# pujariaditya/WaveVerify

Measured on AMD Instinct MI355X. Metric: clips/sec embed+detect, 1s@16kHz bs=256, higher is better.
Workload: dtype f32; 1 GPU; embed_detect: 256 clips x 1 s @ 16 kHz per GPU (BASELINE.json configs[1]), seeded random weights; batch_per_gpu=256, global_batch=256, clip_samples=16000, parallelism=dp1 (independent clip shards, no data-path collective)

## Files before the change

### waveverify_amd/csrc/wv_k1.hip

```cpp
#include <algorithm>
#include <atomic>
#include <cstdlib>
#include <string>
#include <type_traits>

#include "wv_dev.h"

namespace wv {

typedef const __attribute__((address_space(1))) void* gptr_t;
typedef __attribute__((address_space(3))) void* lptr_t;

__device__ __attribute__((aligned(16))) float g_zero16[4] = {0.f, 0.f, 0.f, 0.f};

__device__ __forceinline__ float dpp_next(float v) {
    return __builtin_bit_cast(float, __builtin_amdgcn_update_dpp(0, __builtin_bit_cast(int, v), 0x130, 0xf, 0xf, true));
}

template <int NT_, int BKC_, int BM_ = 128>
struct K1 {
    static constexpr int NT = NT_, BN = 32 * NT_, BKC = BKC_, KQ = BKC_ / 4, BM = BM_, WM = BM_ / 32, NTHREADS = 64 * WM;
    static constexpr int A4 = KQ * BM;
    static constexpr int B4 = BKC * BN / 4;
    static constexpr int STAGE4 = A4 + B4;
    static constexpr int A_PIECES = A4 / 64, B_PIECES = B4 / 64;
    static constexpr int A_PER = (A_PIECES + WM - 1) / WM, B_PER_DMA = (B_PIECES + WM - 1) / WM;
    static constexpr int CG = BN / 4;
    static constexpr int HLD = BN + 4;
    static constexpr int NBT = (BKC / 2) * CG;
    static constexpr int B_PER = (NBT + NTHREADS - 1) / NTHREADS;
    static_assert(A4 % 64 == 0 && B4 % 64 == 0 && NTHREADS % CG == 0 && 64 % CG == 0, "staging maps");
};

template <int NT> struct NVec;
template <> struct NVec<4> { typedef f32x4 type; };
template <> struct NVec<2> { typedef f32x2 type; };

constexpr int OOB_VOFF = 0x40000000;

template <class C>
struct DmaRows {
    const float* src; size_t ld; int K; int rbase;
    __device__ __forceinline__ void init(const float* Xb, int K_, int Tin, int ti0, int wave, int lane) {
        const int col = ti0 + 4 * (lane % C::CG);
        rbase = lane / C::CG;
        const bool inr = col >= 0 && col + 3 < Tin;
        src = inr ? Xb + col : g_zero16;
        ld = inr ? (size_t)Tin : 0;
        K = K_;
        (void)wave;
    }
    __device__ __forceinline__ void init_flat(const float* X, int K_, int Tin, int B, int Tv, int pad, long long g0, int lane) {
        const long long g = g0 + 4 * (lane % C::CG);
        const int b = (int)(g / Tv), t = (int)(g - (long long)b * Tv) - pad;
        rbase = lane / C::CG;
        const bool inr = b < B && t >= 0;
        src = inr ? X + (size_t)b * K_ * Tin + t : g_zero16;
        ld = inr ? (size_t)Tin : 0;
        K = K_;
    }
    __device__ __forceinline__ void issue(int c, f32x4* Bst, int wave) const {
#pragma unroll
        for (int i = 0; i < C::B_PER_DMA; ++i) {
            const int pi = wave + i * C::WM;
            if (C::B_PIECES % C::WM == 0 || pi < C::B_PIECES) {
                const int k = min(c * C::BKC + pi * (64 / C::CG) + rbase, K - 1);
                __builtin_amdgcn_global_load_lds((gptr_t)(src + (size_t)k * ld), (lptr_t)(Bst + pi * 64), 16, 0, 0);
            }
        }
    }
};

template <class C>
struct DmaA {
    __amdgpu_buffer_rsrc_t rsrc;
    int voff[C::A_PER];
    int chunk_bytes;
    __device__ __forceinline__ void init(const f32x4* wq, int Mp, int m0, int nchunks, int wave, int lane) {
        rsrc = __builtin_amdgcn_make_buffer_rsrc(const_cast<f32x4*>(wq + m0), 0, (nchunks * C::KQ * Mp - m0) * 16, 0x00020000);
        chunk_bytes = C::KQ * Mp * 16;
#pragma unroll
        for (int i = 0; i < C::A_PER; ++i) {
            const int idx = (wave + i * C::WM) * 64 + lane;
            voff[i] = ((idx / C::BM) * Mp + idx % C::BM) * 16;
        }
    }
    __device__ __forceinline__ void issue(int c, f32x4* Ast, int wave) const {
        const int soff = c * chunk_bytes;
#pragma unroll
        for (int i = 0; i < C::A_PER; ++i) {
            const int pi = wave + i * C::WM;
            if (C::A_PIECES % C::WM == 0 || pi < C::A_PIECES) {
                const int vo = voff[i];
                __builtin_amdgcn_raw_ptr_buffer_load_lds(rsrc, (lptr_t)(Ast + pi * 64), 16, vo, soff, 0, 0);
            }
        }
    }
};

template <class C, int EPI, int RES>
struct K1Epi {
    static constexpr int NT = C::NT, HLD = C::HLD;
    static constexpr int NTAP = EPI == 0 ? 5 : (EPI == 2 ? 4 : (EPI == 4 ? 8 : 16));
    static constexpr int WLD = EPI == 0 ? 8 : NTAP + 4;
    static constexpr int TABLE_FLOATS = C::BM * WLD;
    static constexpr bool HASR = RES == 1 || RES == 2 || RES == 5;
    static constexpr bool RAWH = RES == 4 || RES == 5;
    static constexpr int RP = HASR ? 4 : 0;
    typedef typename NVec<NT>::type ovec;
    int M, m0, b, to0, lane, wave, half, q, o, to;
    bool act_lane, vec;
    const float* Rb; float* Yb; float* Ab; float* Wl;
    const float* Rb2; float* Hb; float* Sb;
    int voff0, nrec;
    float fgam, fbet;

    __device__ __forceinline__ int row_of(int r) const { return 32 * wave + (r & 3) + 8 * (r >> 2) + 4 * half; }
    __device__ __forceinline__ ovec load_res(const PwDwArgs& p, int r) const {
        ovec v;
#pragma unroll
        for (int e = 0; e < NT; ++e) v[e] = 0.f;
        const int gm = m0 + row_of(r);
        if (act_lane && gm < M) {
            const float* rp = Rb + (size_t)gm * p.Tout + to;
            if (vec) v = *reinterpret_cast<const ovec*>(rp);
            else {
#pragma unroll
                for (int e = 0; e < NT; ++e)
                    if (o + e < p.tto && to + e < p.Tout) v[e] = rp[e];
            }
        }
        return v;
    }
    __device__ __forceinline__ void store(const PwDwArgs& p, int gm, const float (&y)[NT]) const {
        const size_t yo = (size_t)gm * p.Tout + to;
        if (Yb) {
            if (vec) { ovec v; _Pragma("unroll") for (int e = 0; e < NT; ++e) v[e] = y[e]; *reinterpret_cast<ovec*>(Yb + yo) = v; }
            else {
#pragma unroll
                for (int e = 0; e < NT; ++e)
                    if (o + e < p.tto && to + e < p.Tout) Yb[yo + e] = y[e];
            }
        }
        if (Ab) {
            float a[NT];
#pragma unroll
            for (int e = 0; e < NT; ++e) a[e] = elu1(y[e] * p.act_scale);
            if (vec) { ovec v; _Pragma("unroll") for (int e = 0; e < NT; ++e) v[e] = a[e]; *reinterpret_cast<ovec*>(Ab + yo) = v; }
            else {
#pragma unroll
                for (int e = 0; e < NT; ++e)
                    if (o + e < p.tto && to + e < p.Tout) Ab[yo + e] = a[e];
            }
        }
    }
    __device__ __forceinline__ void begin(const PwDwArgs& p, float* table, int m0_, int b_, int to0_, long long gflat = 0) {
        M = p.pw.M; m0 = m0_; b = b_; to0 = to0_;
        const int tid = threadIdx.x;
        lane = tid & 63;
        wave = __builtin_amdgcn_readfirstlane(tid >> 6);
        half = lane >> 5; q = lane & 31;
        Wl = table;
        const size_t bo = (size_t)b * M * p.Tout;
        Yb = p.Y ? p.Y + bo : nullptr;
        Ab = p.Yact ? p.Yact + bo : nullptr;
        Rb = (HASR && p.resid) ? p.resid + bo : nullptr;
        Rb2 = (RES == 2 && p.resid2) ? p.resid2 + bo : nullptr;
        Hb = (RAWH && p.Yraw) ? p.Yraw + bo : nullptr;
        Sb = (RES == 5 && p.Ysum) ? p.Ysum + bo : nullptr;
        o = NT * q; to = to0 + o;
        act_lane = o < p.tto && to < p.Tout;
        vec = act_lane && to + NT - 1 < p.Tout && o + NT - 1 < p.tto && (p.Tout % NT) == 0;
        nrec = M * p.Tout * 4;
        voff0 = act_lane ? ((m0 + 32 * wave + 4 * half) * p.Tout + to) * 4 : 0x7f000000;
        if (EPI == 0 && p.flat) {
            const long long gc = gflat + p.pad + o;
            const int bo2 = (int)(gc / p.Tv), t = (int)(gc - (long long)bo2 * p.Tv) - p.pad;
            const bool ok = o < p.tto && bo2 < p.B && t >= 0;
            Yb = p.Y; Ab = p.Yact; Rb = HASR ? p.resid : nullptr; Rb2 = RES == 2 ? p.resid2 : nullptr; Hb = RAWH ? p.Yraw : nullptr; Sb = RES == 5 ? p.Ysum : nullptr;
            nrec = (int)((long long)p.B * M * p.Tout * 4);
            voff0 = ok ? (int)((((long long)bo2 * M + m0 + 32 * wave + 4 * half) * p.Tout + t) * 4) : (int)0x80000000u;
        }
        if (EPI == 8 && p.flat) {
            const int TvO = p.Tv >> 3;
            const long long go = gflat / 8 + (q >> 1);
            const int bo2 = (int)(go / TvO), n = (int)(go - (long long)bo2 * TvO);
            const bool ok = (q & 1) == 0 && (q >> 1) < p.tto && bo2 < p.B && n < p.Tout;
            Yb = p.Y; Ab = p.Yact;
            nrec = (int)((long long)p.B * M * p.Tout * 4);
            voff0 = ok ? (int)((((long long)bo2 * M + m0 + 32 * wave + 4 * half) * p.Tout + n) * 4) : (int)0x80000000u;
            fgam = 1.f; fbet = 0.f;
            if (p.film) {
                const float* fl = p.film + (size_t)min(bo2, p.B - 1) * p.film_stride + 2 * (m0 / (M / p.bands));
                fgam = fl[0]; fbet = fl[1];
            }
        }
        const bool lane_film = EPI == 8 && p.flat;
        const int bw = p.film ? (M / p.bands) : 1;
        const float* filmb = (p.film && !lane_film) ? p.film + (size_t)b * p.film_stride : nullptr;
        for (int m = tid; m < C::BM; m += C::NTHREADS) {
            const int gm = m0 + m;
            float* row = Wl + m * WLD;
#pragma unroll
            for (int i = 0; i < NTAP; ++i) row[i] = (gm < M && i < p.ks) ? p.dw_w[(size_t)gm * p.ks + i] : 0.f;
            float gam = 1.f, bet = 0.f;
            if (filmb && gm < M) { const int band = gm / bw; gam = filmb[2 * band]; bet = filmb[2 * band + 1]; }
            row[NTAP] = (gm < M && p.dw_b) ? p.dw_b[gm] : 0.f;
            row[NTAP + 1] = gam; row[NTAP + 2] = bet;
            if (EPI != 0) row[WLD - 1] = 0.f;
        }
    }

    typedef unsigned uvec __attribute__((ext_vector_type(NT)));
    __device__ __forceinline__ ovec buf_load(__amdgpu_buffer_rsrc_t r, int off) const {
        if constexpr (NT == 4) return __builtin_bit_cast(ovec, __builtin_amdgcn_raw_buffer_load_b128(r, off, 0, 0));
        else return __builtin_bit_cast(ovec, __builtin_amdgcn_raw_buffer_load_b64(r, off, 0, 0));
    }
    __device__ __forceinline__ void buf_store(__amdgpu_buffer_rsrc_t r, int off, ovec v) const {
        if constexpr (NT == 4) __builtin_amdgcn_raw_buffer_store_b128(__builtin_bit_cast(uvec, v), r, off, 0, 0);
        else __builtin_amdgcn_raw_buffer_store_b64(__builtin_bit_cast(uvec, v), r, off, 0, 0);
    }

    __device__ __forceinline__ void finish(f32x16 (&acc)[NT], const PwDwArgs& p, float* strips) {
        if constexpr (EPI == 0) {
            constexpr int NSH = 4 / NT;
            const int clip_bytes = nrec;
            const __amdgpu_buffer_rsrc_t rY = uniform_rsrc(Yb ? Yb : p.Yact, Yb ? clip_bytes : 0);
            const __amdgpu_buffer_rsrc_t rA = uniform_rsrc(Ab ? Ab : p.Yact, Ab ? clip_bytes : 0);
            const __amdgpu_buffer_rsrc_t rR = uniform_rsrc(Rb ? Rb : p.X, Rb ? clip_bytes : 0);
            const int row_bytes = p.Tout * 4;
            const int voff = voff0;
            const float* Wrow = Wl + (32 * wave + 4 * half) * 8;
            ovec res4[HASR ? 4 : 1];
            ovec add4[RES == 2 ? 4 : 1];
            const __amdgpu_buffer_rsrc_t rR2 = uniform_rsrc(Rb2 ? Rb2 : p.X, Rb2 ? clip_bytes : 0);
            const __amdgpu_buffer_rsrc_t rH = uniform_rsrc(Hb ? Hb : p.Y, Hb ? clip_bytes : 0);
            const __amdgpu_buffer_rsrc_t rS = uniform_rsrc(Sb ? Sb : p.Y, Sb ? clip_bytes : 0);
            const float sres = (RES == 5 && p.scale_ptr) ? p.out_scale * p.scale_ptr[0] : p.out_scale;
            if constexpr (HASR) {
#pragma unroll
                for (int r = 0; r < 4; ++r) res4[r] = buf_load(rR, voff + ((r & 3) + 8 * (r >> 2)) * row_bytes);
            }
            if constexpr (RES == 2) {
#pragma unroll
                for (int r = 0; r < 4; ++r) add4[r] = buf_load(rR2, voff + ((r & 3) + 8 * (r >> 2)) * row_bytes);
            }
            f32x4 w0n = *reinterpret_cast<const f32x4*>(Wrow), w1n = *reinterpret_cast<const f32x4*>(Wrow + 4);
#pragma unroll
            for (int r = 0; r < 16; ++r) {
                const int cr = (r & 3) + 8 * (r >> 2);
                const f32x4 w0 = w0n, w1 = w1n;
                if (r + 1 < 16) {
                    const int cn = ((r + 1) & 3) + 8 * ((r + 1) >> 2);
                    w0n = *reinterpret_cast<const f32x4*>(Wrow + cn * 8);
                    w1n = *reinterpret_cast<const f32x4*>(Wrow + cn * 8 + 4);
                }
                float hh[NT + 4], cur[NT];
#pragma unroll
                for (int e = 0; e < NT; ++e) { cur[e] = acc[e][r]; hh[e] = cur[e]; }
#pragma unroll
                for (int s2 = 1; s2 <= NSH; ++s2) {
#pragma unroll
                    for (int e = 0; e < NT; ++e) { cur[e] = dpp_next(cur[e]); hh[s2 * NT + e] = cur[e]; }
                }
                const int off = voff + cr * row_bytes;
                ovec y;
#pragma unroll
                for (int e = 0; e < NT; ++e) {
                    float v = fmaf(w0.x, hh[e], w1.y);
                    v = fmaf(w0.y, hh[e + 1], v); v = fmaf(w0.z, hh[e + 2], v);
                    v = fmaf(w0.w, hh[e + 3], v); v = fmaf(w1.x, hh[e + 4], v);
                    y[e] = v;
                }
                if constexpr (HASR) {
                    const ovec rr = res4[r & 3];
                    ovec rsum;
                    (void)rsum;
                    if (r + 4 < 16) res4[r & 3] = buf_load(rR, voff + (((r + 4) & 3) + 8 * ((r + 4) >> 2)) * row_bytes);
#pragma unroll
                    for (int e = 0; e < NT; ++e) {
                        if constexpr (RES == 2) {
                            const float z = p.out_scale * rr[e];
                            y[e] = y[e] * (z > 0.f ? 1.f : __expf(z)) * p.out_scale;
                        } else if constexpr (RES == 5) {
                            rsum[e] = fmaf(y[e], sres, rr[e]);
                        } else y[e] = fmaf(y[e], p.out_scale, rr[e]);
                    }
                    if constexpr (RES == 5) buf_store(rS, off, rsum);
                }
                if constexpr (RES == 2) {
                    const ovec ad = add4[r & 3];
                    if (r + 4 < 16) add4[r & 3] = buf_load(rR2, voff + (((r + 4) & 3) + 8 * ((r + 4) >> 2)) * row_bytes);
#pragma unroll
                    for (int e = 0; e < NT; ++e) y[e] += ad[e];
                }
                if constexpr (RAWH) {
                    ovec hraw;
#pragma unroll
                    for (int e = 0; e < NT; ++e) hraw[e] = hh[e + 4];
                    buf_store(rH, off, hraw);
                }
                if (Yb) buf_store(rY, off, y);
                if (Ab) {
                    ovec a;
#pragma unroll
                    for (int e = 0; e < NT; ++e) a[e] = elu1(y[e] * p.act_scale);
                    buf_store(rA, off, a);
                }
                __builtin_amdgcn_sched_barrier(0);
            }
        } else if constexpr (EPI == 5) {
            float* Hw = strips + wave * (4 * HLD);
#pragma unroll
            for (int r = 0; r < 16; ++r) {
                float* strip = Hw + (r & 1) * 2 * HLD;
                ovec hv;
#pragma unroll
                for (int e = 0; e < NT; ++e) hv[e] = acc[e][r];
                *reinterpret_cast<ovec*>(strip + half * HLD + NT * q) = hv;
                const int row = row_of(r), gm = m0 + row;
                const float* wt = Wl + row * WLD;
                const f32x4 ta = *reinterpret_cast<const f32x4*>(wt), tb = *reinterpret_cast<const f32x4*>(wt + 4);
                const f32x4 tc = *reinterpret_cast<const f32x4*>(wt + 8), td = *reinterpret_cast<const f32x4*>(wt + 16);
                if (gm < M && q < p.tto && to0 + q < p.Tout) {
                    const float* hp = strip + half * HLD + p.off + q * 5;
                    float y = td.x;
                    y = fmaf(ta.x, hp[0], y); y = fmaf(ta.y, hp[1], y); y = fmaf(ta.z, hp[2], y); y = fmaf(ta.w, hp[3], y);
                    y = fmaf(tb.x, hp[4], y); y = fmaf(tb.y, hp[5], y); y = fmaf(tb.z, hp[6], y); y = fmaf(tb.w, hp[7], y);
                    y = fmaf(tc.x, hp[8], y); y = fmaf(tc.y, hp[9], y);
                    y = fmaf(y, td.y, td.z);
                    const size_t ro = (size_t)gm * p.Tout + to0 + q;
                    if (Yb) Yb[ro] = y;
                    if (Ab) Ab[ro] = elu1(y * p.act_scale);
                }
            }
        } else if constexpr (EPI >= 2) {
            static_assert(NT == 4 && RES == 0, "strided DPP epilogue: 128-column windows, no residual");
            constexpr int R = EPI;
            const bool flat = R == 8 && p.flat;
            const int clip_bytes = flat ? nrec : M * p.Tout * 4;
            const __amdgpu_buffer_rsrc_t rY = uniform_rsrc(Yb ? Yb : p.Yact, Yb ? clip_bytes : 0);
            const __amdgpu_buffer_rsrc_t rA = uniform_rsrc(Ab ? Ab : p.Yact, Ab ? clip_bytes : 0);
            const int row_bytes = p.Tout * 4;
            const int o0 = R == 2 ? 2 * q : (R == 4 ? q : q >> 1);
            const bool lane_ok = (R != 8 || (q & 1) == 0) && o0 + (R == 2 ? 1 : 0) < p.tto && to0 + o0 + (R == 2 ? 1 : 0) < p.Tout;
            const int voff = flat ? voff0 : (lane_ok ? ((m0 + 32 * wave + 4 * half) * p.Tout + to0 + o0) * 4 : 0x7f000000);
            const float* Wrow = Wl + (32 * wave + 4 * half) * WLD;
#pragma unroll
            for (int r = 0; r < 16; ++r) {
                const int cr = (r & 3) + 8 * (r >> 2);
                constexpr int NL = R == 8 ? 4 : 2;
                float hh[4 * NL], cur[4];
#pragma unroll
                for (int e = 0; e < 4; ++e) { cur[e] = acc[e][r]; hh[e] = cur[e]; }
#pragma unroll
                for (int l = 1; l < NL; ++l) {
#pragma unroll
                    for (int e = 0; e < 4; ++e) { cur[e] = dpp_next(cur[e]); hh[4 * l + e] = cur[e]; }
                }
                const float* wt = Wrow + cr * WLD;
                float w[2 * R];
#pragma unroll
                for (int i = 0; i < 2 * R; i += 4) {
                    const f32x4 v = *reinterpret_cast<const f32x4*>(wt + i);
                    w[i] = v.x; w[i + 1] = v.y; w[i + 2] = v.z; w[i + 3] = v.w;
                }
                const f32x4 bgb = *reinterpret_cast<const f32x4*>(wt + NTAP);
                const int off = voff + cr * row_bytes;
                constexpr int NO = R == 2 ? 2 : 1;
                float y[NO];
#pragma unroll
                for (int j = 0; j < NO; ++j) {
                    const int base = R == 2 ? 2 + 2 * j : 0;
                    float v = bgb.x;
#pragma unroll
                    for (int i = 0; i < 2 * R; ++i) v = fmaf(w[i], hh[base + i], v);
                    y[j] = fmaf(v, bgb.y, bgb.z);
                    if (R == 8 && flat) y[j] = fmaf(y[j], fgam, fbet);
                }
                if constexpr (R == 2) {
                    typedef unsigned u2 __attribute__((ext_vector_type(2)));
                    if (Yb) __builtin_amdgcn_raw_buffer_store_b64(u2{__builtin_bit_cast(unsigned, y[0]), __builtin_bit_cast(unsigned, y[1])}, rY, off, 0, 0);
                    if (Ab) __builtin_amdgcn_raw_buffer_store_b64(u2{__builtin_bit_cast(unsigned, elu1(y[0] * p.act_scale)),
                                                                        __builtin_bit_cast(unsigned, elu1(y[1] * p.act_scale))}, rA, off, 0, 0);
                } else {
                    if (Yb) __builtin_amdgcn_raw_buffer_store_b32(__builtin_bit_cast(unsigned, y[0]), rY, off, 0, 0);
                    if (Ab) __builtin_amdgcn_raw_buffer_store_b32(__builtin_bit_cast(unsigned, elu1(y[0] * p.act_scale)), rA, off, 0, 0);
                }
                __builtin_amdgcn_sched_barrier(0);
            }
        } else {
            float* Hw = strips + wave * (4 * HLD);
            const int ks = p.ks;
            const int no = (p.tto + 31) / 32;
#pragma unroll
            for (int r = 0; r < 16; ++r) {
                float* strip = Hw + (r & 1) * 2 * HLD;
                ovec hv;
#pragma unroll
                for (int e = 0; e < NT; ++e) hv[e] = acc[e][r];
                *reinterpret_cast<ovec*>(strip + half * HLD + NT * q) = hv;
                const int row = row_of(r), gm = m0 + row;
                if (gm >= M) continue;
                const float* wt = Wl + row * WLD;
                const float bias = wt[16], gam = wt[17], bet = wt[18];
                const float* hrow = strip + half * HLD + p.off;
                const size_t ro = (size_t)gm * p.Tout + to0;
                for (int e = 0; e < no; ++e) {
                    const int oo = q * no + e;
                    if (oo >= p.tto || to0 + oo >= p.Tout) break;
                    const float* hp = hrow + oo * p.stride;
                    float y = bias;
                    for (int i = 0; i < ks; ++i) y = fmaf(wt[i], hp[i * p.dil], y);
                    y = fmaf(y, gam, bet);
                    if (RES == 1 && Rb) y = fmaf(y, p.out_scale, Rb[ro + oo]);
                    if (Yb) Yb[ro + oo] = y;
                    if (Ab) Ab[ro + oo] = elu1(y * p.act_scale);
                }
            }
        }
    }
};

template <int LDR> struct LdrSel { typedef RowPairLoader type; };
template <> struct LdrSel<2> { typedef ConvTrPair<4> type; };
template <> struct LdrSel<3> { typedef ConvTrPair<2> type; };
template <> struct LdrSel<4> { typedef ConvTrPair<1> type; };
template <> struct LdrSel<5> { typedef ConvTrPair<0> type; };
template <> struct LdrSel<6> { typedef ConvTrLds<4> type; };
template <> struct LdrSel<7> { typedef ConvTrLds<2> type; };
template <class C> constexpr int k1_lwp(int ldr) { return ldr == 7 ? (C::BN / 2 + 6 + 3) / 4 * 4 : (C::BN / 4 + 6 + 3) / 4 * 4; }

template <class C, int EPI, int LDR, int RES, int NS>
__global__ __launch_bounds__(C::NTHREADS, LDR >= 2 ? (C::B_PER > 1 ? 2 : 3) : 4) void k1_kernel(PwDwArgs p) {
    extern __shared__ __attribute__((aligned(16))) float smem[];
    constexpr bool REG = LDR != 0;
    typedef K1Epi<C, EPI, RES> Epi;
    typedef typename LdrSel<LDR>::type LB;
    typedef typename NVec<C::NT>::type bvec;
    constexpr bool FLAT_OK = EPI == 0 || EPI == 8;
    TileId tile = decode_tile(p);
    if (FLAT_OK && p.flat) {
        const unsigned L = blockIdx.x, j = L >> 3;
        tile.m_tile = j % p.num_m; tile.t_tile = (j / p.num_m) * 8 + (L & 7); tile.b = 0;
        tile.valid = tile.t_tile < p.num_t;
    }
    if (!tile.valid) return;
    const long long gflat = (long long)tile.t_tile * p.tto * p.stride;
    f32x4* S4 = reinterpret_cast<f32x4*>(smem);
    float* table = smem + NS * C::STAGE4 * 4;
    static_assert(NS == 2 || (NS == 3 && LDR == 0), "three stages: DMA path only");
    const int tid = threadIdx.x, lane = tid & 63;
    const int wave = __builtin_amdgcn_readfirstlane(tid >> 6);
    const int h = lane >> 5, i31 = lane & 31;
    const int cg = tid % C::CG;
    const int K = p.pw.K, Mp = p.pw.Mp;
    const int nchunks = (K + C::BKC - 1) / C::BKC;
    const f32x4* wq = reinterpret_cast<const f32x4*>(p.pw.wq);
    const int m0 = tile.m_tile * C::BM, b = tile.b;
    const int to0 = tile.t_tile * p.tto;
    const int ti0 = to0 * p.stride - p.pad - p.off;
    const float* Xb = p.X + (size_t)b * K * p.Tin;

    constexpr int LWP = LDR >= 6 ? k1_lwp<C>(LDR) : 4;
    Epi epi;
    epi.begin(p, table, m0, b, to0, gflat);
    DmaRows<C> db{};
    DmaA<C> da;
    da.init(wq, Mp, m0, nchunks, wave, lane);
    LB lb{};
    float raw[REG ? C::B_PER : 1][REG ? LB::NRAW : 1];
    if constexpr (LDR == 0) {
        if (FLAT_OK && p.flat) db.init_flat(p.X, K, p.Tin, p.B, p.Tv, p.pad, gflat, lane);
        else db.init(Xb, K, p.Tin, ti0, wave, lane);
    }
    else {
        const float* Xt = Xb;
        int c0 = ti0, ncols = p.Tin, tout = p.Tout;
        if (EPI == 0 && p.flat) {
            const long long g = gflat + 4 * cg;
            const int bb = (int)(g / p.Tv), t = (int)(g - (long long)bb * p.Tv) - p.pad;
            const bool inb = bb < p.B;
            Xt = p.X + (size_t)(inb ? bb : 0) * K * p.Tin;
            c0 = t - 4 * cg; ncols = inb ? p.Tin : 0; tout = inb ? p.Tout : 0;
        }
        if constexpr (LDR == 1) lb = LB{Xt, K, p.Tin, ncols, c0, p.pre_scale, p.pre_elu, nullptr, 0, false, false};
        else if constexpr (LDR >= 6) {
            const int lfirst = max(c0, 0) / p.ratio;
            lb = LB{p.ct_w, K, p.ratio, c0, LWP, ((lfirst - 1) & ~3), C::BKC - 1, nullptr, 0, 0};
        }
        else lb = LB{Xt, p.ct_w, p.ct_wt, K, p.pw.Kp, p.Tin, tout, c0, p.ratio, p.pre_scale, p.pre_elu, 0, 0, {}, {}};
    }
    float* Rbuf = table + Epi::TABLE_FLOATS;
    auto issue_rows = [&](int c, int buf) {
        if constexpr (LDR >= 6) {
            constexpr int PPR = LWP / 4, NPIECE = C::BKC * PPR, NINST = (NPIECE + 63) / 64, PER = (NINST + C::WM - 1) / C::WM;
#pragma unroll
            for (int i = 0; i < PER; ++i) {
                const int inst = wave + i * C::WM;
                const int q = inst * 64 + lane;
                const int row = q / PPR, f = lb.ls + 4 * (q - row * PPR);
                const bool inr = f >= 0 && f < p.Tin;
                const float* src = inr ? Xb + (size_t)(c * C::BKC + min(row, C::BKC - 1)) * p.Tin + f : g_zero16;
                if (inst < NINST && q < NPIECE)
                    __builtin_amdgcn_global_load_lds((gptr_t)src, (lptr_t)(Rbuf + (size_t)buf * C::BKC * LWP + inst * 256), 16, 0, 0);
            }
        }
    };

    auto issue = [&](int c, int st) {
        f32x4* S = S4 + st * C::STAGE4;
        da.issue(c, S, wave);
        if constexpr (!REG) db.issue(c, S + C::A4, wave);
    };
    auto fetch = [&](int c) {
        if constexpr (LDR >= 6) { if (c + 1 < nchunks) issue_rows(c + 1, (c + 1) & 1); }
        if constexpr (REG) {
#pragma unroll
            for (int r = 0; r < C::B_PER; ++r) {
                const int idx = tid + r * C::NTHREADS;
                if (C::NBT % C::NTHREADS == 0 || idx < C::NBT) lb.fetch2(c * C::BKC + 2 * (idx / C::CG), raw[r]);
            }
        }
    };
    auto commit = [&](int c, int st) {
        if constexpr (LDR >= 6) lb.Rcur = Rbuf + (size_t)(c & 1) * C::BKC * LWP;
        if constexpr (REG) {
            f32x4* Bq = S4 + st * C::STAGE4 + C::A4;
#pragma unroll
            for (int r = 0; r < C::B_PER; ++r) {
                const int idx = tid + r * C::NTHREADS;
                if (!(C::NBT % C::NTHREADS == 0 || idx < C::NBT)) continue;
                const int kp = idx / C::CG;
                float o[8];
                lb.finish2(c * C::BKC + 2 * kp, raw[r], o);
                Bq[(2 * kp) * C::CG + cg] = f32x4{o[0], o[1], o[2], o[3]};
                Bq[(2 * kp + 1) * C::CG + cg] = f32x4{o[4], o[5], o[6], o[7]};
            }
        }
    };
    constexpr int PIECES_MIN = C::A_PIECES / C::WM + C::B_PIECES / C::WM;
    f32x16 acc[C::NT];
#pragma unroll
    for (int e = 0; e < C::NT; ++e)
#pragma unroll
        for (int r = 0; r < 16; ++r) acc[e][r] = 0.f;
    issue(0, 0);
    if constexpr (NS == 2) {
        if constexpr (LDR >= 6) {
            issue_rows(0, 0);
            __syncthreads();
        }
        if constexpr (REG) { lb.init(cg); fetch(0); commit(0, 0); }
        __syncthreads();
    } else {
        if (nchunks > 1) { issue(1, 1); asm volatile("s_waitcnt vmcnt(%0)" :: "n"(PIECES_MIN) : "memory"); }
        else asm volatile("s_waitcnt vmcnt(0)" ::: "memory");
        asm volatile("s_waitcnt lgkmcnt(0)" ::: "memory");
        __builtin_amdgcn_s_barrier();
    }
    int st = 0;
    for (int c = 0; c < nchunks; ++c) {
        const f32x4* S = S4 + st * C::STAGE4;
        const int stn = st + 1 == NS ? 0 : st + 1;
        if constexpr (NS == 2) {
            if (c + 1 < nchunks) { issue(c + 1, stn); fetch(c + 1); }
        } else {
            if (c + 2 < nchunks) issue(c + 2, stn + 1 == NS ? 0 : stn + 1);
        }
        const float* Bf = reinterpret_cast<const float*>(S + C::A4) + C::NT * i31;
#pragma unroll
        for (int g = 0; g < C::BKC / 16; ++g) {
            const f32x4 a0 = S[(4 * g + h) * C::BM + 32 * wave + i31];
            const f32x4 a1 = S[(4 * g + h + 2) * C::BM + 32 * wave + i31];
#define WV_K1_STEP(AV, ROW)                                                                        \
    { const bvec bv = *reinterpret_cast<const bvec*>(Bf + (ROW) * C::BN);                          \
      _Pragma("unroll") for (int e = 0; e < C::NT; ++e)                                            \
          acc[e] = __builtin_amdgcn_mfma_f32_32x32x2f32(AV, bv[e], acc[e], 0, 0, 0); }
            WV_K1_STEP(a0.x, 16 * g + 4 * h + 0) WV_K1_STEP(a0.y, 16 * g + 4 * h + 1)
            WV_K1_STEP(a0.z, 16 * g + 4 * h + 2) WV_K1_STEP(a0.w, 16 * g + 4 * h + 3)
            WV_K1_STEP(a1.x, 16 * g + 8 + 4 * h + 0) WV_K1_STEP(a1.y, 16 * g + 8 + 4 * h + 1)
            WV_K1_STEP(a1.z, 16 * g + 8 + 4 * h + 2) WV_K1_STEP(a1.w, 16 * g + 8 + 4 * h + 3)
#undef WV_K1_STEP
        }
        if constexpr (NS == 2) {
            if (c + 1 < nchunks) commit(c + 1, stn);
            __syncthreads();
        } else {
            if (c + 2 < nchunks) asm volatile("s_waitcnt vmcnt(%0)" :: "n"(PIECES_MIN) : "memory");
            else asm volatile("s_waitcnt vmcnt(0)" ::: "memory");
            __builtin_amdgcn_s_barrier();
        }
        st = stn;
    }
    epi.finish(acc, p, smem);
}

static bool aligned16(const void* p) { return (reinterpret_cast<uintptr_t>(p) & 15) == 0; }

bool k1_supported(const PwDwArgs& a) {
    if (!a.pw.wq || a.pw.Mp % 128) return false;
    if (a.pw.M < 33) return false;
    if (((a.ct_w ? a.Tout : a.Tin) & 3) || !aligned16(a.X) || a.pw.K < 1) return false;
    if ((long long)a.pw.K * a.Tin * 4 >= OOB_VOFF || (long long)a.pw.M * a.Tout * 4 >= OOB_VOFF) return false;
    if (a.Y && !aligned16(a.Y)) return false;
    if (a.Yact && !aligned16(a.Yact)) return false;
    if (a.resid && !aligned16(a.resid)) return false;
    if ((a.resid2 && !aligned16(a.resid2)) || (a.Yraw && !aligned16(a.Yraw)) || (a.Ysum && !aligned16(a.Ysum))) return false;
    if (a.ks < 1 || a.ks > 16 || (a.ks - 1) * a.dil + 1 + 3 > 64) return false;
    if (a.ct_w && a.ratio == 1) return false;
    return true;
}

template <class C, int EPI, int LDR, int RES, int NS = 2>
static hipError_t k1_run(PwDwArgs a, hipStream_t s, const char* base) {
    const size_t smem = NS * (size_t)C::STAGE4 * 16 + (size_t)K1Epi<C, EPI, RES>::TABLE_FLOATS * sizeof(float) +
                        (LDR >= 6 ? (size_t)2 * C::BKC * k1_lwp<C>(LDR) * sizeof(float) : 0);
    static_assert(C::WM * 4 * C::HLD <= 2 * C::STAGE4 * 4, "strips alias the stages");
    a.num_m = (a.pw.M + C::BM - 1) / C::BM;
    a.num_t = (a.Tout + a.tto - 1) / a.tto;
    a.stagger = 0; a.first_gen = 0;
    long long n_act = (long long)a.num_t * a.B;
    if (a.flat) {
        if (!(C::NT == 4 && (EPI == 0 || (EPI == 8 && LDR == 0)))) return hipErrorInvalidValue;
        n_act = EPI == 8 ? ((long long)a.B * (a.Tv / 8) + a.tto - 1) / a.tto : ((long long)a.B * a.Tv - a.pad + a.tto - 1) / a.tto;
        if (n_act > 0x7fffffffLL) return hipErrorInvalidValue;
        a.num_t = (int)n_act;
    }
    const long long nblk = ((n_act + 7) / 8) * 8 * a.num_m;
    if (nblk > 0x7fffffffLL) return hipErrorInvalidValue;
    std::string name;
    if (prof::enabled())
        name = std::string(base) + "<" + std::to_string(C::BM) + "," + std::to_string(C::BN) + (LDR == 0 ? (NS == 3 ? ",dma3" : ",dma") : (LDR >= 6 ? ",win" : ",reg")) + (a.flat ? ",flat>" : ">");
    const double M = a.pw.M, K = a.pw.K, Bd = a.B;
    const double outs = (a.Y ? 1.0 : 0.0) + (a.Yact ? 1.0 : 0.0) + (a.resid ? 1.0 : 0.0);
    const double flops = a.ct_w ? 2.0 * Bd * a.Tout * K * (M + 2.0) : 2.0 * Bd * M * (K * a.Tin + (double)a.ks * a.Tout);
    prof::Scope ps(s, name.c_str(), flops, 4.0 * Bd * (K * a.Tin + M * a.Tout * outs));
    hipLaunchKernelGGL((k1_kernel<C, EPI, LDR, RES, NS>), dim3((unsigned)nblk), dim3(C::NTHREADS), smem, s, a);
    return hipGetLastError();
}

bool pw_dw_geometry(PwDwArgs& a, int BN);

template <class C, int EPI, int RES>
static hipError_t k1_pick_ldr(const PwDwArgs& a, hipStream_t s) {
    if (a.ct_w) {
        if constexpr (EPI == 0 && RES == 0) {
#ifndef K1_NO_LDS_UPSAMPLE
            if (!a.flat && a.pre_scale == 1.f && !a.pre_elu && a.pw.K % C::BKC == 0 && a.Tin % 4 == 0 && a.Tout == a.Tin * a.ratio && C::BM <= 128) {
                if (a.ratio % 4 == 0) return k1_run<C, 0, 6, false>(a, s, "convtr_pw_lds");
                if (a.ratio == 2) return k1_run<C, 0, 7, false>(a, s, "convtr_pw_lds");
            }
#endif
            if (a.ratio % 4 == 0) return k1_run<C, 0, 2, false>(a, s, "convtr_pw");
            if (a.ratio == 2) return k1_run<C, 0, 3, false>(a, s, "convtr_pw");
            return k1_run<C, 0, 5, false>(a, s, "convtr_pw");
        }
        return hipErrorInvalidValue;
    }
    const char* base = a.spec_add ? "spec_add" : (EPI == 0 ? (RES == 2 ? "pw_dw_k5_dact" : RES == 4 ? "pw_dw_k5_h" : RES == 5 ? "pw_dw_k5_hres" : RES ? "pw_dw_k5" : "pw_dw_k5_nr") : (EPI == 1 ? "pw_dw" : "pw_dw_s"));
    if (a.pre_elu || a.pre_scale != 1.f) return k1_run<C, EPI, 1, RES>(a, s, base);
    if constexpr (C::NT == 4 && C::BM == 128) {
        if (EPI == 0 && a.pw.K >= 256) return k1_run<C, EPI, 0, RES, 3>(a, s, base);
    }
    return k1_run<C, EPI, 0, RES>(a, s, base);
}

template <class C>
static hipError_t k1_pick_epi(const PwDwArgs& a, hipStream_t s, bool k5) {
    const bool res = a.resid != nullptr;
    if (a.res_mode == 2) {
        if (!k5 || !res) return hipErrorNotSupported;
        return k1_pick_ldr<C, 0, 2>(a, s);
    }
    if (a.Yraw) {
        if (!k5 || a.ct_w || (res != (a.Ysum != nullptr))) return hipErrorNotSupported;
        return res ? k1_pick_ldr<C, 0, 5>(a, s) : k1_pick_ldr<C, 0, 4>(a, s);
    }
    if (k5) return res ? k1_pick_ldr<C, 0, true>(a, s) : k1_pick_ldr<C, 0, false>(a, s);
    if constexpr (C::NT == 4) {
        if (!res && !a.ct_w && a.dil == 1 && a.ks == 2 * a.stride && a.pad == a.stride &&
            a.off == (a.stride == 2 ? 2 : 0)) {
            if (a.stride == 2) return k1_pick_ldr<C, 2, false>(a, s);
            if (a.stride == 4) return k1_pick_ldr<C, 4, false>(a, s);
            if (a.stride == 8) return k1_pick_ldr<C, 8, false>(a, s);
        }
        if (!res && !a.ct_w && a.dil == 1 && a.ks == 10 && a.stride == 5 && a.tto <= 32) return k1_pick_ldr<C, 5, false>(a, s);
    }
    return res ? k1_pick_ldr<C, 1, true>(a, s) : k1_pick_ldr<C, 1, false>(a, s);
}

hipError_t launch_k1(const PwDwArgs& a0, hipStream_t s) {
    PwDwArgs a = a0;
    const bool k5 = a.ks == 5 && a.stride == 1 && a.dil == 1 && a.pad == 4 && !a.film;
    const int need = (a.ks - 1) * a.dil + 1;
    bool narrow = (a.ct_w ? a.Tout : a.Tin) + a.pad + 3 <= 64;
    if (!narrow) {
        PwDwArgs g128 = a, g64 = a;
        if (pw_dw_geometry(g128, 128) && pw_dw_geometry(g64, 64)) {
            const long long c128 = (long long)((a.Tout + g128.tto - 1) / g128.tto) * 128;
            const long long c64 = (long long)((a.Tout + g64.tto - 1) / g64.tto) * 64;
            if (c64 * 100 < c128 * 95) narrow = true;
        }
    }
    (void)need;
    a.flat = 0;
    if (k5 && a.B > 1 && (a.Tout & 3) == 0) {
        int bm = 128, best = (a.pw.M + 127) / 128 * 128;
        for (int cand : {96, 64}) { const int pd = (a.pw.M + cand - 1) / cand * cand; if (pd < best) { best = pd; bm = cand; } }
        const long long Tv = a.Tout + 4;
        const long long flat_cols = ((long long)a.B * Tv - 4 + 123) / 124 * 128;
        PwDwArgs g = a;
        const int bn = narrow ? 64 : 128;
        long long clip_cols = -1;
        if (pw_dw_geometry(g, bn)) clip_cols = (long long)a.B * ((a.Tout + g.tto - 1) / g.tto) * bn;
        if (a.pw.M % bm == 0 && (long long)a.B * a.pw.M * a.Tout * 4 < 0x7fffffffLL && clip_cols > 0 &&
            flat_cols * 100 < clip_cols * 98) {
            a.flat = 1; a.Tv = (int)Tv; narrow = false;
        }
    }
    if (!pw_dw_geometry(a, narrow ? 64 : 128)) return hipErrorNotSupported;
    if (!narrow && !a.flat && !a.resid && !a.ct_w && a.ks == 16 && a.stride == 8 && a.dil == 1 && a.pad == 8 && a.off == 0 && a.B > 1 &&
        a.Tin % 8 == 0 && a.Tout * 8 == a.Tin && a.pw.M % 128 == 0 && (!a.film || (a.pw.M / a.bands) % 128 == 0) && !a.pre_elu && a.pre_scale == 1.f &&
        (long long)a.B * a.pw.M * a.Tout * 4 < 0x7fffffffLL && (long long)a.B * a.pw.K * a.Tin * 4 < 0x7fffffffLL) {
        const long long flat_tiles = ((long long)a.B * ((a.Tin + 8) / 8) + a.tto - 1) / a.tto;
        const long long clip_tiles = (long long)a.B * ((a.Tout + a.tto - 1) / a.tto);
        if (flat_tiles * 100 < clip_tiles * 98) { a.flat = 1; a.Tv = a.Tin + 8; }
    }
    if ((a.tto * a.stride) % 4 != 0 || (a.pad + a.off) % 4 != 0) return hipErrorNotSupported;
    int bm = 128, best = (a.pw.M + 127) / 128 * 128;
    for (int cand : {96, 64}) {
        const int padded = (a.pw.M + cand - 1) / cand * cand;
        if (padded < best) { best = padded; bm = cand; }
    }
    if (narrow) {
        if (bm == 128) return k1_pick_epi<K1<2, 32, 128>>(a, s, k5);
        if (bm == 96) return k1_pick_epi<K1<2, 32, 96>>(a, s, k5);
        return k1_pick_epi<K1<2, 32, 64>>(a, s, k5);
    }
    if (a.ct_w && k5 && !narrow && !a.resid && !a.Yraw && a.res_mode != 2 && a.pw.M % 256 == 0) return k1_pick_ldr<K1<4, 16, 256>, 0, false>(a, s);
    if (bm == 128) return k1_pick_epi<K1<4, 16, 128>>(a, s, k5);
    if (bm == 96) return k1_pick_epi<K1<4, 16, 96>>(a, s, k5);
    return k1_pick_epi<K1<4, 16, 64>>(a, s, k5);
}


template <class C, bool FUSE>
__global__ __launch_bounds__(C::NTHREADS, (FUSE && C::BM == 64) ? 2 : ((FUSE || C::B_PER > 1) ? 3 : 4)) void stft_k1_kernel(StftArgs p, SpecAddArgs q) {
    constexpr bool PRE_RES = FUSE && C::BM == 64;
    extern __shared__ __attribute__((aligned(16))) float smem[];
    typedef typename NVec<C::NT>::type bvec;
    typedef unsigned uvec __attribute__((ext_vector_type(C::NT)));
    const unsigned L = blockIdx.x, j = L >> 3;
    const int m_tile = j % p.num_m;
    const unsigned n_idx = (j / p.num_m) * 8 + (L & 7);
    if (n_idx >= (unsigned)p.num_t * p.B) return;
    const int t_tile = n_idx % p.num_t, b = n_idx / p.num_t;
    f32x4* S4 = reinterpret_cast<f32x4*>(smem);
    const int tid = threadIdx.x, lane = tid & 63;
    const int wave = __builtin_amdgcn_readfirstlane(tid >> 6);
    const int h = lane >> 5, i31 = lane & 31, cg = tid % C::CG;
    const int K = p.n_fft, m0 = m_tile * C::BM, t0 = t_tile * C::BN;
    const int nchunks = (K + C::BKC - 1) / C::BKC;
    const float* wb = p.wav + (size_t)b * p.T;
    DmaA<C> da;
    da.init(reinterpret_cast<const f32x4*>(p.basis_q), p.Mp, m0, nchunks, wave, lane);

    int sbase[4]; bool fv[4];
#pragma unroll
    for (int e = 0; e < 4; ++e) {
        const int t = t0 + 4 * cg + e;
        fv[e] = t < p.Tf;
        sbase[e] = t * p.hop - (p.n_fft - 1);
    }
    const bool interior = (K % C::BKC) == 0 && t0 + C::BN <= p.Tf && (long long)t0 * p.hop - (p.n_fft - 1) >= 0 &&
                          (long long)(t0 + C::BN - 1) * p.hop < p.T;
    float raw[C::B_PER][8];
    const bool side_on = m_tile == 0;
    float d0[4] = {0.f, 0.f, 0.f, 0.f}, d1[4] = {0.f, 0.f, 0.f, 0.f};
    auto fetch = [&](int c, auto FAST) {
#pragma unroll
        for (int r = 0; r < C::B_PER; ++r) {
            const int idx = tid + r * C::NTHREADS;
            if (!(C::NBT % C::NTHREADS == 0 || idx < C::NBT)) continue;
            const int k0 = c * C::BKC + 2 * (idx / C::CG);
            if constexpr (decltype(FAST)::value) {
#pragma unroll
                for (int e = 0; e < 4; ++e) {
                    const f32x2u v = *reinterpret_cast<const f32x2u*>(wb + (sbase[e] + k0));
                    raw[r][e] = v.x; raw[r][4 + e] = v.y;
                }
            } else {
#pragma unroll
                for (int i = 0; i < 2; ++i)
#pragma unroll
                    for (int e = 0; e < 4; ++e) raw[r][4 * i + e] = wb[min(max(sbase[e] + k0 + i, 0), p.T - 1)];
            }
        }
    };
    auto commit = [&](int c, int st, auto FAST) {
        f32x4* Bq = S4 + st * C::STAGE4 + C::A4;
#pragma unroll
        for (int r = 0; r < C::B_PER; ++r) {
            const int idx = tid + r * C::NTHREADS;
            if (!(C::NBT % C::NTHREADS == 0 || idx < C::NBT)) continue;
            const int kp = idx / C::CG, k0 = c * C::BKC + 2 * kp;
            float o[8];
#pragma unroll
            for (int i = 0; i < 2; ++i)
#pragma unroll
                for (int e = 0; e < 4; ++e) {
                    if constexpr (decltype(FAST)::value) o[4 * i + e] = raw[r][4 * i + e];
                    else {
                        const int sidx = sbase[e] + k0 + i;
                        o[4 * i + e] = (fv[e] && k0 + i < K && sidx >= 0 && sidx < p.T) ? raw[r][4 * i + e] : 0.f;
                    }
                }
            Bq[(2 * kp) * C::CG + cg] = f32x4{o[0], o[1], o[2], o[3]};
            Bq[(2 * kp + 1) * C::CG + cg] = f32x4{o[4], o[5], o[6], o[7]};
            if (side_on) {
#pragma unroll
                for (int i = 0; i < 2; ++i) {
                    const int k = min(k0 + i, K - 1);
                    const float s0 = p.side[k], s1 = p.side[K + k];
#pragma unroll
                    for (int e = 0; e < 4; ++e) { d0[e] = fmaf(s0, o[4 * i + e], d0[e]); d1[e] = fmaf(s1, o[4 * i + e], d1[e]); }
                }
            }
        }
    };
    f32x16 acc[C::NT];
#pragma unroll
    for (int e = 0; e < C::NT; ++e)
#pragma unroll
        for (int r = 0; r < 16; ++r) acc[e][r] = 0.f;
    auto gemm = [&](auto FAST) {
        da.issue(0, S4, wave);
        fetch(0, FAST); commit(0, 0, FAST);
        __syncthreads();
        for (int c = 0; c < nchunks; ++c) {
            const int st = c & 1;
            const f32x4* S = S4 + st * C::STAGE4;
            if (c + 1 < nchunks) { da.issue(c + 1, S4 + (st ^ 1) * C::STAGE4, wave); fetch(c + 1, FAST); }
            const float* Bf = reinterpret_cast<const float*>(S + C::A4) + C::NT * i31;
#pragma unroll
            for (int g = 0; g < C::BKC / 16; ++g) {
                const f32x4 a0 = S[(4 * g + h) * C::BM + 32 * wave + i31];
                const f32x4 a1 = S[(4 * g + h + 2) * C::BM + 32 * wave + i31];
#define WV_ST_STEP(AV, ROW)                                                                        \
    { const bvec bv = *reinterpret_cast<const bvec*>(Bf + (ROW) * C::BN);                          \
      _Pragma("unroll") for (int e = 0; e < C::NT; ++e)                                            \
          acc[e] = __builtin_amdgcn_mfma_f32_32x32x2f32(AV, bv[e], acc[e], 0, 0, 0); }
                WV_ST_STEP(a0.x, 16 * g + 4 * h + 0) WV_ST_STEP(a0.y, 16 * g + 4 * h + 1)
                WV_ST_STEP(a0.z, 16 * g + 4 * h + 2) WV_ST_STEP(a0.w, 16 * g + 4 * h + 3)
                WV_ST_STEP(a1.x, 16 * g + 8 + 4 * h + 0) WV_ST_STEP(a1.y, 16 * g + 8 + 4 * h + 1)
                WV_ST_STEP(a1.z, 16 * g + 8 + 4 * h + 2) WV_ST_STEP(a1.w, 16 * g + 8 + 4 * h + 3)
#undef WV_ST_STEP
            }
            if (c + 1 < nchunks) commit(c + 1, st ^ 1, FAST);
            __syncthreads();
        }
    };
    if (interior) gemm(std::true_type{});
    else gemm(std::false_type{});
    float* sd = smem;
    if (side_on) {
        const int slot = tid / C::CG;
#pragma unroll
        for (int e = 0; e < 4; ++e) {
            sd[(slot * C::BN + 4 * cg + e) * 2] = d0[e];
            sd[(slot * C::BN + 4 * cg + e) * 2 + 1] = d1[e];
        }
        __syncthreads();
    }
    constexpr int NSLOT = C::NTHREADS / C::CG;
    const int clip_bytes = p.F * p.Tf * 4;
    const __amdgpu_buffer_rsrc_t rP = uniform_rsrc(FUSE ? p.wav : p.P + (size_t)b * p.F * p.Tf, FUSE ? 0 : clip_bytes);
    const int tq = t0 + C::NT * i31;
    const bool lane_ok = tq < p.Tf;
    auto logmag = [&](float re, float im) { return stft_logmag(re, im, p.c1, p.c0); };
    constexpr int F16 = FUSE ? (C::BM / 2 + 1 + 15) / 16 * 16 : 0, NC2 = F16 / 16;
    float* Pl = smem + NSLOT * C::BN * 2;
    f32x4 a2[FUSE ? NC2 : 1][2];
    if constexpr (FUSE) {
        const __amdgpu_buffer_rsrc_t rW = uniform_rsrc(q.pw.wq, NC2 * 4 * q.pw.Mp * 16);
        const int avoff = (h * q.pw.Mp + 32 * wave + i31) * 16;
#pragma unroll
        for (int c = 0; c < NC2; ++c) {
            a2[c][0] = __builtin_bit_cast(f32x4, __builtin_amdgcn_raw_buffer_load_b128(rW, avoff, c * 4 * q.pw.Mp * 16, 0));
            a2[c][1] = __builtin_bit_cast(f32x4, __builtin_amdgcn_raw_buffer_load_b128(rW, avoff, (c * 4 + 2) * q.pw.Mp * 16, 0));
        }
        for (int i = tid; i < (F16 - (C::BM / 2 + 1)) * C::BN; i += C::NTHREADS) Pl[(C::BM / 2 + 1) * C::BN + i] = 0.f;
    }
#pragma unroll
    for (int r = 0; r < 16; r += 2) {
        const int row = m0 + 32 * wave + (r & 3) + 8 * (r >> 2) + 4 * h;
// ... 159 lines not shown
```

### waveverify_amd/csrc/wv_kernels.h

```cpp
#pragma once
#include <hip/hip_runtime.h>
#include <stdint.h>

#include <cstring>
#include <vector>

namespace wv {

constexpr int BK = 16;
constexpr int M_ALIGN = 128;

inline int round_up(int x, int a) { return (x + a - 1) / a * a; }

struct PwWeight {
    const float* wt = nullptr;
    int K = 0, M = 0, Kp = 0, Mp = 0;
    const float* wq = nullptr;
};
struct PwDwArgs {
    const float* X;
    PwWeight pw;
    const float* dw_w;
    const float* dw_b;
    const float* film;
    const float* resid;
    const float* resid2;
    float* Yraw;
    float* Ysum;
    const float* scale_ptr;
    int res_mode;
    float* Y;
    int B, Tin, Tout, ks, stride, dil, pad;
    float pre_scale;
    int pre_elu;
    float out_scale;
    int bands, film_stride;
    float* Yact;
    float act_scale;
    int num_m, num_t;
    int stagger, first_gen;
    int tto, off;
    int spec_add;
    int flat, Tv;
    const float* ct_w;
    int ratio;
    const float* ct_wt;
};
hipError_t launch_pw_dw(const PwDwArgs& a, hipStream_t s);
bool k1_supported(const PwDwArgs& a);
hipError_t launch_k1(const PwDwArgs& a, hipStream_t s);
bool pw_dw_geometry(PwDwArgs& a, int BN);
struct RbArgs {
    const float* X;
    float pre_scale;
    PwWeight pw1, pw2;
    const float* tab1;
    const float* tab2;
    float* Y;
    float* Yact;
    float out_scale, act_scale;
    int B, C, T;
    int num_t, ntiles;
    const float* out_scale_ptr = nullptr;
    float *sv_h0 = nullptr, *sv_u = nullptr, *sv_h1 = nullptr, *sv_v = nullptr;
};
bool rb_supported(const RbArgs& a);
hipError_t launch_resblock(const RbArgs& a, hipStream_t s);
inline std::vector<float> pack_rb_table(const float* dw_w, const float* dw_b, int C) {
    std::vector<float> t((size_t)C * 8, 0.f);
    for (int m = 0; m < C; ++m) {
        for (int i = 0; i < 5; ++i) t[(size_t)m * 8 + i] = dw_w[(size_t)m * 5 + i];
        t[(size_t)m * 8 + 5] = dw_b ? dw_b[m] : 0.f;
        t[(size_t)m * 8 + 6] = 1.f;
    }
    return t;
}
inline std::vector<float> pack_ct_wt(const float* w, int K, int Kp, int ratio) {
    std::vector<float> t((size_t)2 * ratio * Kp, 0.f);
    for (int k = 0; k < K; ++k)
        for (int i = 0; i < 2 * ratio; ++i) t[(size_t)i * Kp + k] = w[(size_t)k * 2 * ratio + i];
    return t;
}

struct H16Weight { const void* wq = nullptr; int K = 0, M = 0, Kp = 0, Mp = 0, nchunks = 0; };
inline uint16_t f32_to_f16_bits(float f) {
    uint32_t x; std::memcpy(&x, &f, 4);
    const uint32_t sign = (x >> 16) & 0x8000u;
    x &= 0x7fffffffu;
    if (x >= 0x7f800000u) return (uint16_t)(sign | 0x7c00u | (x > 0x7f800000u ? 0x200u : 0u));
    if (x >= 0x477ff000u) return (uint16_t)(sign | 0x7c00u);
    if (x < 0x38800000u) {
        if (x < 0x33000000u) return (uint16_t)sign;
        const int e = (int)(x >> 23);
        uint32_t m = (x & 0x7fffffu) | 0x800000u;
        const int shift = 126 - e;
        const uint32_t half = m >> shift, rem = m & ((1u << shift) - 1), mid = 1u << (shift - 1);
        return (uint16_t)(sign | (half + ((rem > mid || (rem == mid && (half & 1))) ? 1u : 0u)));
    }
    const uint32_t mant = x & 0x7fffffu, e = (x >> 23) - 112;
    uint32_t hv = (e << 10) | (mant >> 13);
    const uint32_t rem = mant & 0x1fffu;
    if (rem > 0x1000u || (rem == 0x1000u && (hv & 1))) ++hv;
    return (uint16_t)(sign | hv);
}
inline std::vector<uint16_t> pack_h16(const float* pw, const float* dw, int M, int K, int ks, H16Weight* out, bool dw_by_k = false) {
    H16Weight w; w.K = K; w.M = M; w.Kp = round_up(K, 16); w.Mp = round_up(M, 32);
    const int nkc = w.Kp / 16;
    w.nchunks = round_up(ks * nkc, 8);
    std::vector<uint16_t> q((size_t)w.nchunks * w.Mp * 16, 0);
    for (int i = 0; i < ks; ++i)
        for (int m = 0; m < M; ++m) {
            const float t = (dw && !dw_by_k) ? dw[(size_t)m * ks + i] : 1.f;
            for (int k = 0; k < K; ++k) {
                const float tk = (dw && dw_by_k) ? dw[(size_t)k * ks + i] : t;
                q[(((size_t)((k / 16) * ks + i) * w.Mp + m) * 2 + ((k >> 3) & 1)) * 8 + (k & 7)] = f32_to_f16_bits(pw[(size_t)m * K + k] * tk);
            }
        }
    *out = w;
    return q;
}
inline std::vector<uint16_t> pack_head16(const float* wc, int D, int nb, int hop, H16Weight* out) {
    const int rows = nb * hop;
    std::vector<float> wt((size_t)rows * D);
    for (int d = 0; d < D; ++d)
        for (int r = 0; r < rows; ++r) wt[(size_t)r * D + d] = wc[(size_t)d * rows + r];
    return pack_h16(wt.data(), nullptr, rows, D, 1, out);
}
struct RhArgs {
    const void* X; float pre_scale; H16Weight w1, w2; const float* tab1; const float* tab2;
    void* Y; void* Yact; float out_scale, act_scale; int B, C, T; int num_t, ntiles;
};
constexpr double RH_LOG2E = 1.4426950408889634;
inline std::vector<uint16_t> pack_rh_pw(const float* pw, int C, H16Weight* out) {
    std::vector<float> t((size_t)C * C);
    for (size_t i = 0; i < t.size(); ++i) t[i] = (float)((double)pw[i] / RH_LOG2E);
    return pack_h16(t.data(), nullptr, C, C, 1, out);
}
inline std::vector<float> pack_rh_table(const float* dw_w, const float* dw_b, int C, double scale) {
    std::vector<float> t((size_t)(C / 2) * 12, 0.f);
    for (int m = 0; m < C; ++m) {
        float* row = t.data() + (size_t)(m / 2) * 12 + (m & 1);
        for (int i = 0; i < 5; ++i) row[2 * i] = (float)((double)dw_w[(size_t)m * 5 + i] * scale);
        row[10] = dw_b ? (float)((double)dw_b[m] * scale) : 0.f;
    }
    return t;
}
bool rh_supported(const RhArgs& a);
hipError_t launch_resblock16(const RhArgs& a, hipStream_t s);
struct Conv16Args {
    const void* X; H16Weight w; const float* bias; const void* resid; void* Y; void* Yact; float* Yf32;
    float out_scale, act_scale; int B, M, Tin, Tout, ks, stride, pad;
    const float* film = nullptr; int bands = 1, film_stride = 0;
    int up = 0, up_mb = 0;
};
inline int up16_block(int Mo, int r) {
    for (int mb = (256 / r) / 8 * 8; mb >= 8; mb -= 8)
        if (Mo % mb == 0) return mb;
    return 0;
}
inline std::vector<uint16_t> pack_up16(const float* pw, const float* ct, int Mo, int K, int r, int mb, H16Weight* out) {
    H16Weight w; w.K = K; w.M = Mo * r; w.Kp = round_up(K, 16); w.Mp = round_up(w.M, 32);
    const int nkc = w.Kp / 16;
    w.nchunks = round_up(2 * nkc, 8);
    std::vector<uint16_t> q((size_t)w.nchunks * w.Mp * 16, 0);
    for (int i = 0; i < 2; ++i)
        for (int p = 0; p < r; ++p)
            for (int m = 0; m < Mo; ++m) {
                const size_t row = (size_t)(m / mb) * r * mb + (size_t)p * mb + m % mb;
                for (int k = 0; k < K; ++k)
                    q[(((size_t)((k / 16) * 2 + i) * w.Mp + row) * 2 + ((k >> 3) & 1)) * 8 + (k & 7)] =
                        f32_to_f16_bits(pw[(size_t)m * K + k] * ct[(size_t)k * 2 * r + (i == 0 ? p + r : p)]);
            }
    *out = w;
    return q;
}
hipError_t launch_conv16(const Conv16Args& a, hipStream_t s);
struct Spec16Args {
    const float* wav; H16Weight cosw, sinw, cosl, sinl, pw; const void* resid; void* Y; void* Yact;
    const float* side;
    float* Yf32;
    float out_scale, act_scale, c1, c0; int B, T, Tf, n_fft, hop;
};
hipError_t launch_spec16(const Spec16Args& a, hipStream_t s);
inline float f16_bits_to_f32(uint16_t hb) {
    const uint32_t sign = (uint32_t)(hb & 0x8000u) << 16, e = (hb >> 10) & 31u, m = hb & 0x3ffu;
    uint32_t x;
    if (e == 0) {
        if (m == 0) x = sign;
        else { int sh = 0; uint32_t mm = m; while (!(mm & 0x400u)) { mm <<= 1; ++sh; } x = sign | ((uint32_t)(113 - sh) << 23) | ((mm & 0x3ffu) << 13); }
    } else if (e == 31) x = sign | 0x7f800000u | (m << 13);
    else x = sign | ((e + 112) << 23) | (m << 13);
    float f; std::memcpy(&f, &x, 4);
    return f;
}
inline void pack_stft16(const float* basis, int n_fft, std::vector<uint16_t> (&q)[4], H16Weight (&w)[4]) {
    const int F = n_fft / 2 + 1, R = n_fft / 2;
    std::vector<float> m[4];
    for (auto& v : m) v.resize((size_t)R * n_fft);
    for (int f = 0; f < R; ++f)
        for (int n = 0; n < n_fft; ++n) {
            const float c = basis[(size_t)f * n_fft + n];
            const float s = f == 0 ? basis[(size_t)(F - 1) * n_fft + n] : basis[(size_t)(F + f) * n_fft + n];
// ... 128 lines not shown
```

### waveverify_amd/csrc/wv_kernels.hip

```cpp
#include "wv_kernels.h"
#include "wv_dev.h"

namespace wv {


template <int BM_, int BN_, int WM_, int WN_>
struct Tile {
    static constexpr int BM = BM_, BN = BN_, WM = WM_, WN = WN_;
    static constexpr int NTHREADS = 64 * WM * WN;
    static constexpr int MT = BM / (32 * WM);
    static constexpr int NT = BN / (32 * WN);
    static constexpr int A_VEC = BK * BM / 4;
    static constexpr int A_PER = (A_VEC + NTHREADS - 1) / NTHREADS;
    static constexpr int B_TPR = BN / 4;
    static constexpr int BKSTEP = NTHREADS / B_TPR;
    static constexpr int B_PER = (BK + BKSTEP - 1) / BKSTEP;
    static constexpr int STAGE = BK * (BM + BN);
    static_assert(MT >= 1 && NT >= 1, "tile too small for the wave grid");
    static_assert(BM % 4 == 0 && NTHREADS % B_TPR == 0 && BKSTEP >= 1, "staging map");
};

template <class T>
__device__ __forceinline__ void zero_acc(f32x16 (&acc)[T::MT][T::NT]) {
#pragma unroll
// ... 103 lines not shown
    const float* base; int K, ld, ncols, c0; float scale; int elu;
    const float* p; int c; bool full, vec;
    __device__ __forceinline__ void init(int col4) {
        c = c0 + col4;
        full = c >= 0 && c + 3 < ncols;
        vec = full && ((ld & 3) == 0) && ((c & 3) == 0) && ((reinterpret_cast<uintptr_t>(base) & 15) == 0);
        p = base + c;
    }
    __device__ __forceinline__ void fetch(int k, float (&raw)[4]) const {
        if (k < K && vec) {
            const float4 v = *reinterpret_cast<const float4*>(p + (size_t)k * ld);
            raw[0] = v.x; raw[1] = v.y; raw[2] = v.z; raw[3] = v.w;
        } else {
#pragma unroll
            for (int i = 0; i < 4; ++i)
                raw[i] = (k < K && c + i >= 0 && c + i < ncols) ? p[(size_t)k * ld + i] : 0.f;
        }
    }
    __device__ __forceinline__ void finish(int, const float (&raw)[4], float (&o)[4]) const {
#pragma unroll
        for (int i = 0; i < 4; ++i) o[i] = act(raw[i], scale, elu);
    }
};

template <class T>
struct QT {
    static constexpr int KQ = BK / 4;
    static constexpr int NB = KQ * T::BN;
    static constexpr int CG = T::BN / 4;
    static constexpr int NBT = (BK / 2) * CG;
    static constexpr int B_PER = (NBT + T::NTHREADS - 1) / T::NTHREADS;
    static_assert(T::NTHREADS % CG == 0, "a thread keeps its column group");
};

template <class T, class LB>
__device__ __forceinline__ void gemm_mainloop_q(f32x16 (&acc)[1][T::NT], const f32x4* __restrict__ wq,
                                                int Mp, int m0, LB& lb, int nchunks, f32x4* smem) {
    using Q = QT<T>;
    static_assert(T::WN == 1 && T::MT == 1, "row-strip tile");
    const int tid = threadIdx.x, lane = tid & 63, wave = tid >> 6;
    const int cg = tid % Q::CG;
    const int h = lane >> 5, i31 = lane & 31;
    const f32x4* wa = wq + m0 + 32 * wave + i31;
    f32x4 an0, an1;
    float rb[Q::B_PER][LB::NRAW];
    lb.init(cg);

    auto fetch = [&](int c) {
        an0 = wa[(size_t)(c * Q::KQ + h) * Mp];
        an1 = wa[(size_t)(c * Q::KQ + h + 2) * Mp];
#pragma unroll
        for (int r = 0; r < Q::B_PER; ++r) {
            const int idx = tid + r * T::NTHREADS;
            if (Q::NBT % T::NTHREADS == 0 || idx < Q::NBT) lb.fetch2(c * BK + (idx / Q::CG) * 2, rb[r]);
        }
    };
    auto commit = [&](int c, f32x4* buf) {
        float* Bf = reinterpret_cast<float*>(buf);
#pragma unroll
        for (int r = 0; r < Q::B_PER; ++r) {
            const int idx = tid + r * T::NTHREADS;
            if (!(Q::NBT % T::NTHREADS == 0 || idx < Q::NBT)) continue;
            const int kp = idx / Q::CG;
            const int kq = kp >> 1, kh = kp & 1;
            float o[8];
            lb.finish2(c * BK + 2 * kp, rb[r], o);
#pragma unroll
            for (int j = 0; j < 4; ++j) {
                const int slot = q_slot(4 * cg + j);
                f32x2 v{o[j], o[4 + j]};
                *reinterpret_cast<f32x2*>(Bf + ((size_t)(kq * T::BN + slot) * 4 + 2 * kh)) = v;
            }
        }
    };
    int bslot[T::NT];
#pragma unroll
    for (int j = 0; j < T::NT; ++j) bslot[j] = q_slot(32 * j + i31);
    fetch(0);
    commit(0, smem);
    f32x4 a0 = an0, a1 = an1;
    __syncthreads();
    for (int c = 0; c < nchunks; ++c) {
        const f32x4* Bs = smem + (c & 1) * Q::NB;
        if (c + 1 < nchunks) fetch(c + 1);
        {
            f32x4 b0[T::NT], b1[T::NT];
#pragma unroll
            for (int j = 0; j < T::NT; ++j) {
                b0[j] = Bs[h * T::BN + bslot[j]];
                b1[j] = Bs[(h + 2) * T::BN + bslot[j]];
            }
#define WV_QSTEP(AV, BQ, COMP)                                                                     \
    _Pragma("unroll") for (int j = 0; j < T::NT; ++j)                                              \
        acc[0][j] = __builtin_amdgcn_mfma_f32_32x32x2f32(AV, BQ[j].COMP, acc[0][j], 0, 0, 0);
            WV_QSTEP(a0.x, b0, x) WV_QSTEP(a0.y, b0, y) WV_QSTEP(a0.z, b0, z) WV_QSTEP(a0.w, b0, w)
            WV_QSTEP(a1.x, b1, x) WV_QSTEP(a1.y, b1, y) WV_QSTEP(a1.z, b1, z) WV_QSTEP(a1.w, b1, w)
#undef WV_QSTEP
        }
        if (c + 1 < nchunks) commit(c + 1, smem + ((c + 1) & 1) * Q::NB);
        a0 = an0; a1 = an1;
        __syncthreads();
    }
}

template <class T, int KS, int RP_ = 8>
struct PwDwEpi {
    static constexpr int HLD = T::BN + 4;
    static constexpr int RP = RP_;
    static constexpr int WLD = KS ? 8 : 20;
    static constexpr int FLOATS = T::BM * WLD;
    static constexpr int STRIP_FLOATS = T::WM * 4 * HLD;
    int M, m0, b, to0, lane, wave, half, q, o, to;
    bool act_lane, vec;
    const float* Rb; float* Yb; float* Wl; float* Hw;
    float4 res[RP ? RP : 1];

    __device__ __forceinline__ int row_of(int r) const { return 32 * wave + (r & 3) + 8 * (r >> 2) + 4 * half; }
    __device__ __forceinline__ float4 load_res(const PwDwArgs& p, int r) const {
        float4 v = make_float4(0.f, 0.f, 0.f, 0.f);
        const int gm = m0 + row_of(r);
        if (Rb && act_lane && gm < M) {
            const float* rp = Rb + (size_t)gm * p.Tout + to;
            if (vec) v = *reinterpret_cast<const float4*>(rp);
            else {
                v.x = rp[0];
                if (to + 1 < p.Tout) v.y = rp[1];
                if (to + 2 < p.Tout) v.z = rp[2];
                if (to + 3 < p.Tout) v.w = rp[3];
            }
        }
        return v;
    }
    __device__ __forceinline__ void begin(const PwDwArgs& p, float* epi_smem, float* strip_smem, int m0_, int b_, int to0_) {
        M = p.pw.M; m0 = m0_; b = b_; to0 = to0_;
        const int tid = threadIdx.x;
        lane = tid & 63;
        wave = __builtin_amdgcn_readfirstlane(tid >> 6);
        half = lane >> 5; q = lane & 31;
        Wl = epi_smem;
        Hw = strip_smem + wave * (4 * HLD);
        Yb = p.Y + (size_t)b * M * p.Tout;
        Rb = p.resid ? p.resid + (size_t)b * M * p.Tout : nullptr;
        o = 4 * q; to = to0 + o;
        act_lane = o < p.tto && to < p.Tout;
        vec = act_lane && to + 3 < p.Tout && o + 3 < p.tto && (p.Tout & 3) == 0;
        if (KS) {
            const int bw = p.film ? (M / p.bands) : 1;
            const float* filmb = p.film ? p.film + (size_t)b * p.film_stride : nullptr;
            for (int m = tid; m < T::BM; m += T::NTHREADS) {
                const int gm = m0 + m;
                float v[8] = {0, 0, 0, 0, 0, 0, 1.f, 0};
                if (gm < M) {
#pragma unroll
                    for (int i = 0; i < KS; ++i) v[i] = p.dw_w[(size_t)gm * KS + i];
                    v[5] = p.dw_b ? p.dw_b[gm] : 0.f;
                    if (filmb) { const int band = gm / bw; v[6] = filmb[2 * band]; v[7] = filmb[2 * band + 1]; }
                }
                *reinterpret_cast<float4*>(Wl + m * 8) = make_float4(v[0], v[1], v[2], v[3]);
                *reinterpret_cast<float4*>(Wl + m * 8 + 4) = make_float4(v[4], v[5], v[6], v[7]);
            }
            if constexpr (RP > 0) {
#pragma unroll
                for (int r = 0; r < RP; ++r) res[r] = load_res(p, r);
            }
        } else {
            const int bw = p.film ? (M / p.bands) : 1;
            const float* filmb = p.film ? p.film + (size_t)b * p.film_stride : nullptr;
            for (int m = tid; m < T::BM; m += T::NTHREADS) {
                const int gm = m0 + m;
                float* row = Wl + m * WLD;
                for (int i = 0; i < 16; ++i) row[i] = (gm < M && i < p.ks) ? p.dw_w[(size_t)gm * p.ks + i] : 0.f;
                row[16] = (gm < M && p.dw_b) ? p.dw_b[gm] : 0.f;
                float gam = 1.f, bet = 0.f;
                if (filmb && gm < M) { const int band = gm / bw; gam = filmb[2 * band]; bet = filmb[2 * band + 1]; }
                row[17] = gam; row[18] = bet; row[19] = 0.f;
            }
        }
    }

    __device__ __forceinline__ void finish(f32x16 (&acc)[1][T::NT], const PwDwArgs& p) {
        if (KS) {
#pragma unroll
            for (int r = 0; r < 16; ++r) {
                float* strip = Hw + (r & 1) * 2 * HLD;
#pragma unroll
                for (int j = 0; j < T::NT; ++j) strip[half * HLD + 32 * j + q] = acc[0][j][r];
                const int row = row_of(r), gm = m0 + row;
                float4 rr = make_float4(0.f, 0.f, 0.f, 0.f);
                if constexpr (RP > 0) {
                    rr = res[r % RP];
                    if (r + RP < 16) res[r % RP] = load_res(p, r + RP);
                }
                if (act_lane && gm < M) {
                    const float4 h0 = *reinterpret_cast<const float4*>(strip + half * HLD + o);
                    const float4 h1 = *reinterpret_cast<const float4*>(strip + half * HLD + o + 4);
                    const float4 w0 = *reinterpret_cast<const float4*>(Wl + row * 8);
                    const float4 w1 = *reinterpret_cast<const float4*>(Wl + row * 8 + 4);
                    const float h[8] = {h0.x, h0.y, h0.z, h0.w, h1.x, h1.y, h1.z, h1.w};
                    const float rv[4] = {rr.x, rr.y, rr.z, rr.w};
                    float y[4];
#pragma unroll
                    for (int e = 0; e < 4; ++e) {
                        float v = w1.y;
                        v = fmaf(w0.x, h[e], v); v = fmaf(w0.y, h[e + 1], v); v = fmaf(w0.z, h[e + 2], v);
                        v = fmaf(w0.w, h[e + 3], v); v = fmaf(w1.x, h[e + 4], v);
                        v = fmaf(v, w1.z, w1.w);
                        if (RP > 0 && Rb) v = fmaf(v, p.out_scale, rv[e]);
                        y[e] = v;
                    }
                    const size_t yo = (size_t)gm * p.Tout + to;
                    if (p.Y) {
                        float* yp = Yb + yo;
                        if (vec) *reinterpret_cast<float4*>(yp) = make_float4(y[0], y[1], y[2], y[3]);
                        else {
#pragma unroll
                            for (int e = 0; e < 4; ++e)
                                if (o + e < p.tto && to + e < p.Tout) yp[e] = y[e];
                        }
                    }
                    if (p.Yact) {
                        float* ya = p.Yact + (size_t)b * M * p.Tout + yo;
#pragma unroll
                        for (int e = 0; e < 4; ++e) y[e] = elu1(y[e] * p.act_scale);
                        if (vec) *reinterpret_cast<float4*>(ya) = make_float4(y[0], y[1], y[2], y[3]);
                        else {
#pragma unroll
                            for (int e = 0; e < 4; ++e)
                                if (o + e < p.tto && to + e < p.Tout) ya[e] = y[e];
                        }
                    }
                }
            }
        } else {
            const int ks = p.ks;
            const int no = (p.tto + 31) / 32;
            const bool pair2 = no == 2 && p.stride == 2 && ks == 4 && p.dil == 1 && (p.off & 1) == 0 &&
                               (p.Tout & 1) == 0 && (to0 & 1) == 0;
#pragma unroll
            for (int r = 0; r < 16; ++r) {
                float* strip = Hw + (r & 1) * 2 * HLD;
#pragma unroll
                for (int j = 0; j < T::NT; ++j) strip[half * HLD + 32 * j + q] = acc[0][j][r];
                const int row = row_of(r), gm = m0 + row;
                if (gm >= M) continue;
                const float* wt = Wl + row * WLD;
                const float bias = wt[16], gam = wt[17], bet = wt[18];
                const float* hrow = strip + half * HLD + p.off;
                float* yrow = Yb + (size_t)gm * p.Tout + to0;
                float* arow = p.Yact ? p.Yact + ((size_t)b * M + gm) * p.Tout + to0 : nullptr;
                const float* rrow = Rb ? Rb + (size_t)gm * p.Tout + to0 : nullptr;
                if (pair2) {
                    const int o0 = 2 * q;
                    if (o0 + 1 < p.tto && to0 + o0 + 1 < p.Tout) {
                        const f32x2 ha = *reinterpret_cast<const f32x2*>(hrow + 2 * o0);
                        const f32x2 hb = *reinterpret_cast<const f32x2*>(hrow + 2 * o0 + 2);
                        const f32x2 hc = *reinterpret_cast<const f32x2*>(hrow + 2 * o0 + 4);
                        float y0 = fmaf(wt[3], hb.y, fmaf(wt[2], hb.x, fmaf(wt[1], ha.y, fmaf(wt[0], ha.x, bias))));
                        float y1 = fmaf(wt[3], hc.y, fmaf(wt[2], hc.x, fmaf(wt[1], hb.y, fmaf(wt[0], hb.x, bias))));
                        y0 = fmaf(y0, gam, bet); y1 = fmaf(y1, gam, bet);
                        if (rrow) { y0 = fmaf(y0, p.out_scale, rrow[o0]); y1 = fmaf(y1, p.out_scale, rrow[o0 + 1]); }
                        if (p.Y) *reinterpret_cast<f32x2*>(yrow + o0) = f32x2{y0, y1};
                        if (arow) *reinterpret_cast<f32x2*>(arow + o0) = f32x2{elu1(y0 * p.act_scale), elu1(y1 * p.act_scale)};
                        continue;
                    }
                }
                for (int e = 0; e < no; ++e) {
                    const int oo = q * no + e;
                    if (oo >= p.tto || to0 + oo >= p.Tout) break;
                    const float* h = hrow + oo * p.stride;
                    float y = bias;
                    for (int i = 0; i < ks; ++i) y = fmaf(wt[i], h[i * p.dil], y);
                    y = fmaf(y, gam, bet);
                    if (rrow) y = fmaf(y, p.out_scale, rrow[oo]);
                    if (p.Y) yrow[oo] = y;
                    if (arow) arow[oo] = elu1(y * p.act_scale);
                }
            }
        }
    }
};

template <class T, int KS, int RM = -1, bool RES = true>
__global__ __launch_bounds__(T::NTHREADS, (T::NTHREADS >= 192 && T::BN == 128) ? 3 : 2) void pw_dw_kernel(PwDwArgs p) {
    static_assert(T::WN == 1 && T::MT == 1, "row-strip tile");
    extern __shared__ __attribute__((aligned(16))) float smem[];
    constexpr int HLD = T::BN + 4;
    const TileId tile = decode_tile(p);
    if (!tile.valid) return;
    const int m0 = tile.m_tile * T::BM;
    const int b = tile.b;
    const int K = p.pw.K;
    const int to0 = tile.t_tile * p.tto;
    const int ti0 = to0 * p.stride - p.pad - p.off;

    if (p.stagger > 0) {
        const unsigned lin = blockIdx.x;
        if (lin < (unsigned)p.first_gen) {
            const int slot = lin / 256;
            for (int i = 0; i < slot * p.stagger; ++i) __builtin_amdgcn_s_sleep(127);
        }
    }
    PwDwEpi<T, KS, (RM < 0 && RES) ? ((T::BN == 64 || T::BM <= 96) ? 4 : 8) : 0> epi;
    constexpr int STAGES_F = 2 * QT<T>::NB * 4;
    epi.begin(p, smem + STAGES_F, smem, m0, b, to0);
    static_assert(PwDwEpi<T, KS>::STRIP_FLOATS <= STAGES_F, "strips alias the stages");
    f32x16 acc[1][T::NT];
    zero_acc<T>(acc);
// ... 490 lines not shown
}
Scope::Scope(hipStream_t st, const char* kernel, double flops, double bytes) : s(st) {
    if (!g_on.load(std::memory_order_relaxed)) return;
    hipStreamCaptureStatus cs = hipStreamCaptureStatusNone;
    if (hipStreamIsCapturing(st, &cs) != hipSuccess || cs != hipStreamCaptureStatusNone) return;
    std::lock_guard<std::mutex> lk(g_mu);
    if (g_recs.size() >= MAX_RECS) drain_locked();
    std::string key = std::string(kernel) + "|" + g_role;
    auto it = g_index.find(key);
    int k;
    if (it == g_index.end()) { k = (int)g_agg.size(); g_index[key] = k; Agg a; a.name = key; g_agg.push_back(a); }
    else k = it->second;
    g_agg[k].launches += 1; g_agg[k].flops += flops; g_agg[k].bytes += bytes;
    ev_a = get_event(); ev_b = get_event(); key_ = k;
    (void)hipEventRecord((hipEvent_t)ev_a, s);
    armed = true;
}
Scope::~Scope() {
    if (!armed) return;
    (void)hipEventRecord((hipEvent_t)ev_b, s);
    std::lock_guard<std::mutex> lk(g_mu);
    g_recs.push_back(Rec{(hipEvent_t)ev_a, (hipEvent_t)ev_b, key_});
}
}

template <class T>
static std::string tile_name(const char* base) {
    return std::string(base) + "<" + std::to_string(T::BM) + "," + std::to_string(T::BN) + "," +
           std::to_string(T::WM) + "," + std::to_string(T::WN) + ">";
}

template <class T>
static constexpr size_t stage_bytes() { return 2 * (size_t)T::STAGE * sizeof(float); }

static int cur_dev() { int d = 0; (void)hipGetDevice(&d); return d & 31; }
template <class K>
static hipError_t set_smem(K kernel, size_t bytes, std::atomic<unsigned>& done) {
    if (bytes <= 64 * 1024) return hipSuccess;
    const unsigned bit = 1u << cur_dev();
    if (done.load(std::memory_order_relaxed) & bit) return hipSuccess;
    hipError_t e = hipFuncSetAttribute(reinterpret_cast<const void*>(kernel),
                                       hipFuncAttributeMaxDynamicSharedMemorySize, (int)bytes);
    if (e == hipSuccess) done.fetch_or(bit, std::memory_order_relaxed);
    return e;
}

static int gcd_(int a, int b) { while (b) { int t = a % b; a = b; b = t; } return a; }

bool pw_dw_geometry(PwDwArgs& a, int BN) {
    const int span = (a.ks - 1) * a.dil + 1;
    a.off = (4 - (a.pad % 4)) % 4;
    int tto = (BN - a.off - span) / a.stride + 1;
    const int q = 4 / gcd_(a.stride, 4);
    tto -= tto % q;
    if (tto < 1) {
        a.off = 0;
        tto = (BN - span) / a.stride + 1;
    }
    a.tto = tto;
    return tto >= 1;
}

template <class T, int KS>
static hipError_t run_pw_dw_ks(PwDwArgs a, hipStream_t s) {
    if (!pw_dw_geometry(a, T::BN)) return hipErrorInvalidValue;
    const size_t eb = (size_t)PwDwEpi<T, KS>::FLOATS * sizeof(float);
    const size_t smem = 2 * (size_t)QT<T>::NB * 16 + eb;
    static std::atomic<unsigned> attr_f32{0};
    {
        hipError_t e = set_smem(pw_dw_kernel<T, KS>, smem, attr_f32);
        if (e != hipSuccess) return e;
    }
    static std::atomic<int> per_cu_dev[32];
    int per_cu = per_cu_dev[cur_dev()].load(std::memory_order_relaxed);
    if (per_cu < 1) {
        int n = 0;
        if (hipOccupancyMaxActiveBlocksPerMultiprocessor(&n, pw_dw_kernel<T, KS>, T::NTHREADS, smem) != hipSuccess || n < 1)
            n = 1;
        per_cu = n;
        per_cu_dev[cur_dev()].store(n, std::memory_order_relaxed);
    }
    a.stagger = 2;
    a.first_gen = 256 * per_cu;
    a.num_m = (a.pw.M + T::BM - 1) / T::BM;
    a.num_t = (a.Tout + a.tto - 1) / a.tto;
    const long long n_act = (long long)a.num_t * a.B;
    const long long nblk = ((n_act + 7) / 8) * 8 * a.num_m;
    if (nblk > 0x7fffffffLL) return hipErrorInvalidValue;
    dim3 grid((unsigned)nblk);
    if (nblk < 4LL * a.first_gen) a.stagger = 0;
    static const std::string name = tile_name<T>(KS ? "pw_dw_k5" : "pw_dw");
    const double M = a.pw.M, K = a.pw.K, Bd = a.B;
    if constexpr (KS == 5) if (a.ct_w) {
        static const std::string cname = tile_name<T>("convtr_pw");
        prof::Scope pc(s, cname.c_str(), 2.0 * Bd * a.Tout * K * (M + 2.0), 4.0 * Bd * (K * a.Tin + M * a.Tout));
        static std::atomic<unsigned> attr_ct4{0}, attr_ct2{0}, attr_ct1{0}, attr_ct0{0};
        {
            hipError_t e = set_smem(pw_dw_kernel<T, 5, 4>, smem, attr_ct4);
            if (e == hipSuccess) e = set_smem(pw_dw_kernel<T, 5, 2>, smem, attr_ct2);
            if (e == hipSuccess) e = set_smem(pw_dw_kernel<T, 5, 1>, smem, attr_ct1);
            if (e == hipSuccess) e = set_smem(pw_dw_kernel<T, 5, 0>, smem, attr_ct0);
            if (e != hipSuccess) return e;
        }
        if (a.ratio % 4 == 0) hipLaunchKernelGGL((pw_dw_kernel<T, 5, 4>), grid, dim3(T::NTHREADS), smem, s, a);
        else if (a.ratio == 2) hipLaunchKernelGGL((pw_dw_kernel<T, 5, 2>), grid, dim3(T::NTHREADS), smem, s, a);
        else if (a.ratio == 1) hipLaunchKernelGGL((pw_dw_kernel<T, 5, 1>), grid, dim3(T::NTHREADS), smem, s, a);
        else hipLaunchKernelGGL((pw_dw_kernel<T, 5, 0>), grid, dim3(T::NTHREADS), smem, s, a);
        return hipGetLastError();
    }
    if constexpr (KS == 5) if (a.spec_add && a.resid) {
        static const std::string sname = tile_name<T>("spec_add");
        prof::Scope pa(s, sname.c_str(), 2.0 * Bd * M * K * a.Tin, 4.0 * Bd * (K * a.Tin + 2.0 * M * a.Tout));
        static std::atomic<unsigned> attr_sa{0};
        {
            hipError_t e = set_smem(pw_dw_kernel<T, 5, -2>, smem, attr_sa);
            if (e != hipSuccess) return e;
        }
        hipLaunchKernelGGL((pw_dw_kernel<T, 5, -2>), grid, dim3(T::NTHREADS), smem, s, a);
        return hipGetLastError();
    }
    static const std::string name_nr = tile_name<T>("pw_dw_k5_nr");
    const bool nores = KS == 5 && !a.resid;
    prof::Scope ps(s, nores ? name_nr.c_str() : name.c_str(), 2.0 * Bd * M * (K * a.Tin + (double)a.ks * a.Tout),
                   4.0 * Bd * (K * a.Tin + M * a.Tout * (a.resid ? 2.0 : 1.0)));
    if constexpr (KS == 5) if (nores) {
        static std::atomic<unsigned> attr_nr{0};
        {
            hipError_t e = set_smem(pw_dw_kernel<T, 5, -1, false>, smem, attr_nr);
            if (e != hipSuccess) return e;
        }
        hipLaunchKernelGGL((pw_dw_kernel<T, 5, -1, false>), grid, dim3(T::NTHREADS), smem, s, a);
        return hipGetLastError();
    }
    hipLaunchKernelGGL((pw_dw_kernel<T, KS>), grid, dim3(T::NTHREADS), smem, s, a);
    return hipGetLastError();
}

template <class T>
static hipError_t run_pw_dw(const PwDwArgs& a, hipStream_t s) {
    if (a.ks == 5 && a.stride == 1 && a.dil == 1 && a.pad == 4) return run_pw_dw_ks<T, 5>(a, s);
    return run_pw_dw_ks<T, 0>(a, s);
}

static int pick_bm(int M) {
    if (M <= 32) return 32;
    if (M <= 64) return 64;
    if (M <= 96) return 96;
    if (M % 128 == 0) return 128;
    if (M == 192) return 64;
    if (M % 96 == 0) return 96;
    return 128;
}

hipError_t launch_pw_dw(const PwDwArgs& a, hipStream_t s) {
    if (a.ct_w && (!a.ct_wt || (reinterpret_cast<uintptr_t>(a.ct_wt) & 7) || a.ratio < 1 || a.Tout != a.Tin * a.ratio || a.ks != 5 || a.stride != 1 || a.dil != 1 || a.pad != 4 ||
                   (reinterpret_cast<uintptr_t>(a.ct_w) & 15)))
        return hipErrorInvalidValue;
    if (a.ks < 1 || a.ks > 16 || a.stride < 1 || a.dil < 1 || a.pad < 0 || a.pw.Mp % M_ALIGN || a.pw.Kp % BK || !a.pw.wq)
        return hipErrorInvalidValue;
    if (k1_supported(a)) {
        const hipError_t e = launch_k1(a, s);
        if (e != hipErrorNotSupported) return e;
    }
    if (a.res_mode || a.Yraw || a.Ysum) return hipErrorNotSupported;
    const int need = (a.ks - 1) * a.dil + 1;
    bool narrow = a.Tin + a.pad + 3 <= 64 && need + 3 <= 64;
    if (!narrow && need + 3 <= 64) {
        PwDwArgs g128 = a, g64 = a;
        if (pw_dw_geometry(g128, 128) && pw_dw_geometry(g64, 64)) {
            const long long c128 = (long long)((a.Tout + g128.tto - 1) / g128.tto) * 128;
            const long long c64 = (long long)((a.Tout + g64.tto - 1) / g64.tto) * 64;
            if (c64 * 100 < c128 * 95) narrow = true;
        }
    }
    const int bm = pick_bm(a.pw.M);
    if (narrow) {
        switch (bm) {
            case 32: return run_pw_dw<Tile<32, 64, 1, 1>>(a, s);
            case 64: return run_pw_dw<Tile<64, 64, 2, 1>>(a, s);
            case 96: return run_pw_dw<Tile<96, 64, 3, 1>>(a, s);
            default: return run_pw_dw<Tile<128, 64, 4, 1>>(a, s);
        }
    }
    switch (bm) {
        case 32: return run_pw_dw<Tile<32, 128, 1, 1>>(a, s);
        case 64: return run_pw_dw<Tile<64, 128, 2, 1>>(a, s);
        case 96: return run_pw_dw<Tile<96, 128, 3, 1>>(a, s);
        default: return run_pw_dw<Tile<128, 128, 4, 1>>(a, s);
    }
}

template <class T, int MODE>
static hipError_t run_dw_pw_mode(const DwPwArgs& a, hipStream_t s) {
    size_t smem = stage_bytes<T>();
    const size_t hb = ((size_t)T::BM * (T::BN + 4) + T::BN) * sizeof(float);
    if (hb > smem) smem = hb;
    static std::atomic<unsigned> attr_done{0};
    {
        hipError_t e = set_smem(dw_pw_kernel<T, MODE>, smem, attr_done);
        if (e != hipSuccess) return e;
    }
    if (a.l2norm && a.pw.M > T::BM) return hipErrorInvalidValue;
    dim3 grid((a.pw.M + T::BM - 1) / T::BM, (a.Tout + T::BN - 1) / T::BN, a.B);
    static const std::string name = tile_name<T>(MODE == 0 ? "pw" : "dwconv_pw");
    const double M = a.pw.M, K = a.pw.K, Bd = a.B;
    const double stencil = a.mode == 1 ? 2.0 * a.ks : 0.0;
    prof::Scope ps(s, name.c_str(), Bd * a.Tout * (2.0 * M * K + stencil * K),
                   4.0 * Bd * (K * a.Tin + M * a.Tout * (a.accumulate ? 2.0 : 1.0)));
    hipLaunchKernelGGL((dw_pw_kernel<T, MODE>), grid, dim3(NT_), smem, s, a);
    return hipGetLastError();
}

template <class T>
static hipError_t run_dw_pw(const DwPwArgs& a, hipStream_t s) {
    if (a.mode == 0) return run_dw_pw_mode<T, 0>(a, s);
    return run_dw_pw_mode<T, 1>(a, s);
}

hipError_t launch_dw_pw(const DwPwArgs& a, hipStream_t s) {
    if (a.pw.Mp % M_ALIGN || a.pw.Kp % BK || a.mode < 0 || a.mode > 1 || a.Tout != a.Tin) return hipErrorInvalidValue;
    int bm = pick_bm(a.pw.M);
    if (a.l2norm) bm = a.pw.M <= 64 ? 64 : 128;
    if (a.Tout <= 64) {
        if (bm <= 64) return run_dw_pw<Tile<64, 64, 2, 2>>(a, s);
        return run_dw_pw<Tile<128, 64, 2, 2>>(a, s);
    }
    switch (bm) {
        case 32: return run_dw_pw<Tile<32, 128, 1, 4>>(a, s);
        case 64: return run_dw_pw<Tile<64, 128, 1, 4>>(a, s);
        case 96: return run_dw_pw<Tile<96, 128, 1, 4>>(a, s);
        default: return run_dw_pw<Tile<128, 128, 1, 4>>(a, s);
    }
}

template <class T>
static hipError_t run_stft(const StftArgs& a, hipStream_t s) {
    dim3 grid((a.n_fft + T::BM - 1) / T::BM, (a.Tf + T::BN - 1) / T::BN, a.B);
    static const std::string name = tile_name<T>("stft_logmag");
    prof::Scope ps(s, name.c_str(), 2.0 * a.B * (2.0 * a.F) * a.n_fft * a.Tf,
                   4.0 * a.B * ((double)a.T + (double)a.F * a.Tf));
    hipLaunchKernelGGL(stft_logmag_kernel<T>, grid, dim3(NT_), stage_bytes<T>(), s, a);
    return hipGetLastError();
}

hipError_t launch_stft_logmag(const StftArgs& a_in, hipStream_t s) {
    StftArgs a = a_in;
    a.c1 = 0.5f * 0.69314718055994531f * a.inv_std;
    a.c0 = -a.mean * a.inv_std;
    if (a.Mp % M_ALIGN || a.Mp < a.n_fft || a.n_fft < 4 || (a.n_fft & 1) || a.F != a.n_fft / 2 + 1 || !a.side)
        return hipErrorInvalidValue;
    {
        const hipError_t e = launch_stft_k1(a, s);
        if (e != hipErrorNotSupported) return e;
    }
    if (a.Tf <= 64) return run_stft<Tile<128, 64, 2, 2>>(a, s);
    if (a.n_fft <= 64) return run_stft<Tile<64, 128, 1, 4>>(a, s);
    if (round_up(a.n_fft, 96) < round_up(a.n_fft, 128)) return run_stft<Tile<96, 128, 1, 4>>(a, s);
    return run_stft<Tile<128, 128, 1, 4>>(a, s);
}

hipError_t launch_conv_pre(const float* x, const float* w, const float* bias, float* Y, float* Yact, float act_scale,
                           int B, int C, int T, int ks, float in_scale, hipStream_t s) {
    if (ks < 1 || ks > MAX_KS) return hipErrorInvalidValue;
    dim3 grid((T + 4 * NT_ - 1) / (4 * NT_), B);
    prof::Scope ps(s, "conv_pre", 2.0 * B * C * ks * (double)T, 4.0 * B * (double)T * (1.0 + C * (Yact ? 2.0 : 1.0)));
    hipLaunchKernelGGL(conv_pre_kernel, grid, dim3(NT_), 0, s, x, w, bias, Y, Yact, act_scale, C, T, ks, in_scale);
    return hipGetLastError();
}

hipError_t launch_tail(const float* H, const float* w, const float* bias, const float* x,
                       float* out, int B, int C, int Tin, int T, int ks, float pre_scale,
                       float out_scale, hipStream_t s) {
    if (ks < 1 || ks > 32 || T > Tin) return hipErrorInvalidValue;
    if (ks == 5 && (Tin & 3) == 0 && (reinterpret_cast<uintptr_t>(H) & 15) == 0) {
        prof::Scope ps(s, "tail", 2.0 * B * C * ks * (double)T, 4.0 * B * ((double)C * Tin + 2.0 * T));
        hipLaunchKernelGGL(tail5_vec_kernel, dim3((T + 1007) / 1008, B), dim3(NT_), 0, s, H, w, bias, x, out, C, Tin, T, pre_scale, out_scale);
        return hipGetLastError();
    }
    const int per_block = 4 * (64 - (ks - 1));
    dim3 grid((T + per_block - 1) / per_block, B);
    prof::Scope ps(s, "tail", 2.0 * B * C * ks * (double)T, 4.0 * B * ((double)C * Tin + 2.0 * T));
    hipLaunchKernelGGL(tail_kernel, grid, dim3(NT_), 0, s, H, w, bias, x, out, C, Tin, T, ks,
                       pre_scale, out_scale);
    return hipGetLastError();
}

hipError_t launch_head(const HeadArgs& a, hipStream_t s) {
    using T = Tile<64, 64, 2, 2>;
    dim3 grid(a.nb, a.B);
    static const std::string name = tile_name<T>("head");
    prof::Scope ps(s, name.c_str(), 2.0 * a.B * a.D * (double)a.nb * a.hop * a.Fr,
                   4.0 * a.B * ((double)a.D * a.Fr + (a.logits ? (double)a.nb * a.T : 0.0)));
    if (a.keep_lo || a.keep_hi || a.psum) {
        if (!a.keep_lo || !a.keep_hi || a.mean_prob) return hipErrorInvalidValue;
        hipLaunchKernelGGL((head_kernel<T, true>), grid, dim3(NT_), stage_bytes<T>(), s, a);
    } else {
        hipLaunchKernelGGL((head_kernel<T, false>), grid, dim3(NT_), stage_bytes<T>(), s, a);
    }
    return hipGetLastError();
}

hipError_t launch_film(const FilmArgs& a, hipStream_t s) {
    if (a.E > NT_ || a.E < 1) return hipErrorInvalidValue;
    prof::Scope ps(s, "film", 2.0 * a.B * a.E * (a.msg_dim + a.n_layers * a.E + a.n_out), 4.0 * a.B * (a.msg_dim + a.n_out));
    hipLaunchKernelGGL(film_kernel, dim3(a.B), dim3(NT_), 0, s, a);
    return hipGetLastError();
}

}
```

### waveverify_amd/csrc/wv_model.hip

```cpp
#include <hip/hip_runtime.h>

#include <cmath>
#include <cstdio>
#include <cstdlib>
#include <cstring>
#include <string>
#include <unordered_map>
#include <vector>

#include "wv_host.h"
#include "wv_kernels.h"

namespace {

thread_local std::string g_err;
using wv::fail;

struct Param {
    std::string name;
    std::vector<int64_t> shape;
    bool wn = false;
    bool optional = false;
    std::vector<float> data;
    bool set = false;
    int64_t numel() const { int64_t n = 1; for (auto d : shape) n *= d; return n; }
};

using wv::PwWeight;

struct ResBlock {
    PwWeight pw1, pw2;
    const float *dw1_w, *dw1_b, *dw2_w, *dw2_b;
    const float *tab1 = nullptr, *tab2 = nullptr;
    float pre_scale, out_scale;
    int ks, dil1, dil2;
};
struct SpecLayer {
    const float* basis_t; const float* basis_q; const float* side; int n_fft, hop, F, Mp; float mean, inv_std;
    PwWeight pw; float scale;
    const float* id_taps;
};
struct DownLayer { PwWeight pw; const float *dw_w, *dw_b; int ratio; float pre_scale; };
struct UpLayer {
    const float* ct_w; int ratio; PwWeight pw; const float* pw_b; float pre_scale;
    const float* id_taps;
    const float* ct_wt;
    std::vector<ResBlock> res;
};

}

int wv::fail(int code, std::string msg) { g_err = std::move(msg); return code; }

struct wv_model {
    wv_config cfg{};
    std::vector<Param> params;
    std::unordered_map<std::string, int> index;
    std::unordered_map<std::string, std::vector<float>> stft_override;
    bool finalized = false;
    std::vector<void*> dev;

    const float *pre_w = nullptr, *pre_b = nullptr;
    std::vector<std::vector<ResBlock>> enc_blocks;
    std::vector<SpecLayer> specs;
    std::vector<DownLayer> downs;
    const float* post_dw_w = nullptr; PwWeight post_pw; const float* post_b = nullptr;
    bool has_film = false;
    const float *f_w0 = nullptr, *f_b0 = nullptr, *f_wl = nullptr, *f_bl = nullptr,
                *f_wf = nullptr, *f_bf = nullptr;
    PwWeight dec_pw0; const float *dec_dw0_w = nullptr, *dec_dw0_b = nullptr;
    std::vector<UpLayer> ups;
    const float *last_w = nullptr, *last_b = nullptr;
    float dec_post = 1.f;
    const float *head_wc = nullptr, *head_bc = nullptr;
    int head_nb = 0;
    struct H16Block { wv::H16Weight w1, w2; const float *tab1 = nullptr, *tab2 = nullptr; };
    struct H16Stage { std::vector<H16Block> blocks; wv::H16Weight spec, down, cosw, sinw, cosl, sinl, post, head; };
    struct H16Up { wv::H16Weight up; int mb = 0; std::vector<H16Block> blocks; };
    std::vector<H16Stage> h16;
    wv::H16Weight h16_dec_head;
    std::vector<H16Up> h16_ups;

    ~wv_model() { for (void* p : dev) (void)hipFree(p); }
};

namespace {

int hop_of(const wv_config& c) { int h = 1; for (int i = 0; i < c.n_strides; ++i) h *= c.strides[i]; return h; }
int ratio_enc(const wv_config& c, int s) { return c.strides[c.n_strides - 1 - s]; }

void add(wv_model* m, const std::string& name, std::vector<int64_t> shape, bool wn, bool optional = false) {
    Param p; p.name = name; p.shape = std::move(shape); p.wn = wn; p.optional = optional;
    m->index[name] = (int)m->params.size();
    m->params.push_back(std::move(p));
}

void add_resblock(wv_model* m, const std::string& pre, int dim, int k, bool zero_init) {
    if (zero_init) add(m, pre + ".res_scale_param", {1}, false);
    const int idx[2][2] = {{1, 2}, {4, 5}};
    for (auto& pd : idx) {
        add(m, pre + ".block." + std::to_string(pd[0]) + ".conv.conv.weight", {dim, dim, 1}, true);
        add(m, pre + ".block." + std::to_string(pd[1]) + ".conv.conv.bias", {dim}, false);
        add(m, pre + ".block." + std::to_string(pd[1]) + ".conv.conv.weight", {dim, 1, k}, true);
    }
}

void build_param_table(wv_model* m) {
    const wv_config& c = m->cfg;
    const int C0 = c.channels_enc, S = c.n_strides;
    const bool zi = c.zero_init != 0;
    add(m, "encoder.conv_pre.1.conv.conv.bias", {C0}, false);
    add(m, "encoder.conv_pre.1.conv.conv.weight", {C0, 1, c.kernel_size}, true);
    int mult = 1;
    for (int s = 0; s < S; ++s) {
        for (int j = 0; j < c.n_residual_enc; ++j)
            add_resblock(m, "encoder.blocks." + std::to_string(s) + "." + std::to_string(j),
                         mult * C0, c.residual_kernel_size, zi);
        mult *= 2;
    }
    mult = 1;
    for (int s = 0; s < S; ++s) {
        const std::string pre = "encoder.spec_blocks." + std::to_string(s);
        if (zi) add(m, pre + ".scale_param", {1}, false);
        add(m, pre + ".layer.conv.conv.weight", {mult * C0, mult * c.n_fft_base / 2 + 1, 1}, true);
        mult *= 2;
    }
    mult = 1;
    for (int s = 0; s < S; ++s) {
        const int C = mult * C0, r = ratio_enc(c, s);
        const std::string pre = "encoder.downsample." + std::to_string(s);
        add(m, pre + ".2.conv.conv.weight", {2 * C, C, 1}, true);
        add(m, pre + ".3.conv.conv.bias", {2 * C}, false);
        add(m, pre + ".3.conv.conv.weight", {2 * C, 1, 2 * r}, true);
        mult *= 2;
    }
    const int Ctop = mult * C0;
    if (zi) add(m, "encoder.spec_post.scale_param", {1}, false);
    add(m, "encoder.spec_post.layer.conv.conv.weight", {Ctop, mult * c.n_fft_base / 2 + 1, 1}, true);
    add(m, "encoder.conv_post.1.conv.conv.weight", {Ctop, 1, c.last_kernel_size}, true);
    add(m, "encoder.conv_post.2.conv.conv.bias", {c.dimension}, false);
    add(m, "encoder.conv_post.2.conv.conv.weight", {c.dimension, Ctop, 1}, true);
    const bool opt = c.kind != WV_KIND_GENERATOR;
    const int E = c.embedding_dim;
    add(m, "encoder.msg_embedding.0.weight", {E, c.msg_dimension}, false, opt);
    add(m, "encoder.msg_embedding.0.bias", {E}, false, opt);
    for (int l = 0; l < c.embedding_layers; ++l) {
        const std::string pre = "encoder.msg_embedding." + std::to_string(1 + 2 * l);
        add(m, pre + ".weight", {E, E}, false, opt);
        add(m, pre + ".bias", {E}, false, opt);
    }
    for (int s = 0; s < S; ++s)
        for (int b = 0; b < c.freq_bands; ++b)
            for (const char* nm : {"gamma", "beta"}) {
                const std::string pre = "encoder.film_layers." + std::to_string(s) + "." +
                                        std::to_string(b) + "." + nm + "_layer";
                add(m, pre + ".weight", {1, E}, false, opt);
                add(m, pre + ".bias", {1}, false, opt);
            }
    if (c.kind == WV_KIND_GENERATOR) {
        const int Cd = c.channels_dec;
        int dm = 1 << S;
        add(m, "decoder.model.0.conv.conv.weight", {dm * Cd, c.dimension, 1}, true);
        add(m, "decoder.model.1.conv.conv.bias", {dm * Cd}, false);
        add(m, "decoder.model.1.conv.conv.weight", {dm * Cd, 1, c.kernel_size}, true);
        int n = 2;
        for (int i = 0; i < S; ++i) {
            const int C = dm * Cd, r = c.strides[i];
            add(m, "decoder.model." + std::to_string(n + 2) + ".convtr.convtr.weight", {C, 1, 2 * r}, true);
            add(m, "decoder.model." + std::to_string(n + 3) + ".conv.conv.bias", {C / 2}, false);
            add(m, "decoder.model." + std::to_string(n + 3) + ".conv.conv.weight", {C / 2, C, 1}, true);
            for (int j = 0; j < c.n_residual_dec; ++j)
                add_resblock(m, "decoder.model." + std::to_string(n + 4 + j), C / 2,
                             c.residual_kernel_size, zi);
            n += 4 + c.n_residual_dec;
            dm /= 2;
        }
        add(m, "decoder.model." + std::to_string(n + 2) + ".conv.conv.bias", {1}, false);
        add(m, "decoder.model." + std::to_string(n + 2) + ".conv.conv.weight", {1, Cd, c.last_kernel_size}, true);
    } else {
        const int nb = c.kind == WV_KIND_DETECTOR ? c.nbits : 1;
        add(m, "reverse_convolution.weight", {c.dimension, c.output_dim, hop_of(c)}, false);
        add(m, "reverse_convolution.bias", {c.output_dim}, false);
        add(m, "last_layer.weight", {nb, c.output_dim, 1}, false);
        add(m, "last_layer.bias", {nb}, false);
    }
}

struct Uploader {
    wv_model* m;
    int err = WV_OK;
    const float* up(const std::vector<float>& h) {
        if (err != WV_OK) return nullptr;
        void* d = nullptr;
        const size_t bytes = std::max<size_t>(h.size(), 1) * sizeof(float);
        if (hipMalloc(&d, bytes) != hipSuccess) { err = fail(WV_EHIP, "hipMalloc failed while packing weights"); return nullptr; }
        m->dev.push_back(d);
        if (!h.empty() && hipMemcpy(d, h.data(), h.size() * sizeof(float), hipMemcpyHostToDevice) != hipSuccess) {
            err = fail(WV_EHIP, "hipMemcpy failed while packing weights");
            return nullptr;
        }
        return static_cast<const float*>(d);
    }
    wv::H16Weight h16(const std::vector<float>& pw, const float* dw, int M, int K, int ks) {
        wv::H16Weight w;
        const std::vector<uint16_t> q = wv::pack_h16(pw.data(), dw, M, K, ks, &w);
        return h16_up(q, w);
    }
    wv_model::H16Block h16_block(const std::string& pre, int C) {
        wv_model::H16Block b;
        wv::H16Weight w;
        { const std::vector<uint16_t> q = wv::pack_rh_pw(host(pre + ".block.1.conv.conv.weight").data(), C, &w); b.w1 = h16_up(q, w); }
        { const std::vector<uint16_t> q = wv::pack_rh_pw(host(pre + ".block.4.conv.conv.weight").data(), C, &w); b.w2 = h16_up(q, w); }
        b.tab1 = up(wv::pack_rh_table(host(pre + ".block.2.conv.conv.weight").data(), host(pre + ".block.2.conv.conv.bias").data(), C, wv::RH_LOG2E));
        b.tab2 = up(wv::pack_rh_table(host(pre + ".block.5.conv.conv.weight").data(), host(pre + ".block.5.conv.conv.bias").data(), C, 1.0));
        return b;
    }
    wv::H16Weight h16_up(const std::vector<uint16_t>& q, wv::H16Weight w) {
        if (err != WV_OK) return w;
        void* d = nullptr;
        if (hipMalloc(&d, q.size() * sizeof(uint16_t)) != hipSuccess) { err = fail(WV_EHIP, "hipMalloc failed while packing f16 weights"); return w; }
        m->dev.push_back(d);
        if (hipMemcpy(d, q.data(), q.size() * sizeof(uint16_t), hipMemcpyHostToDevice) != hipSuccess) {
            err = fail(WV_EHIP, "hipMemcpy failed while packing f16 weights");
            return w;
        }
        w.wq = d;
        return w;
    }
    const std::vector<float>& host(const std::string& name) {
        static const std::vector<float> empty;
        auto it = m->index.find(name);
        if (it == m->index.end()) { err = fail(WV_ENOKEY, "internal: unknown key " + name); return empty; }
        return m->params[it->second].data;
    }
    const float* plain(const std::string& name) { return up(host(name)); }
    float scalar_or(const std::string& name, float dflt) {
        auto it = m->index.find(name);
        return it == m->index.end() ? dflt : m->params[it->second].data[0];
    }
    PwWeight pw_from(const std::vector<float>& w, int M, int K) {
        PwWeight p; p.M = M; p.K = K; p.Kp = wv::round_up(K, wv::BK); p.Mp = wv::round_up(M, wv::M_ALIGN);
        std::vector<float> t((size_t)p.Kp * p.Mp, 0.f);
        for (int mm = 0; mm < M; ++mm)
            for (int k = 0; k < K; ++k) t[(size_t)k * p.Mp + mm] = w[(size_t)mm * K + k];
        p.wt = up(t);
        std::vector<float> q((size_t)wv::round_up(K, 32) * p.Mp, 0.f);
        for (int mm = 0; mm < M; ++mm)
            for (int k = 0; k < K; ++k) q[((size_t)(k / 4) * p.Mp + mm) * 4 + (k & 3)] = w[(size_t)mm * K + k];
        p.wq = up(q);
        return p;
    }
    PwWeight pw(const std::string& name) {
        auto it = m->index.find(name);
        const Param& P = m->params[it->second];
        return pw_from(P.data, (int)P.shape[0], (int)P.shape[1]);
    }
};

std::vector<float> make_basis(int n_fft) {
    const int F = n_fft / 2 + 1;
    std::vector<float> w((size_t)2 * F * n_fft);
    const float c = (float)(-2.0 * M_PI / n_fft);
    const float wc = (float)(2.0 * M_PI / n_fft);
    for (int k = 0; k < F; ++k) {
        volatile float ck = c * (float)k;
        for (int n = 0; n < n_fft; ++n) {
            volatile float ang = ck * (float)n;
            volatile float wa = (float)n * wc;
            const float win = 0.5f - 0.5f * (float)std::cos((double)wa);
            w[(size_t)k * n_fft + n] = (float)std::cos((double)ang) * win;
            w[(size_t)(F + k) * n_fft + n] = (float)std::sin((double)ang) * win;
        }
    }
    return w;
}

const float* pack_basis(Uploader& U, const std::vector<float>& basis, int n_fft, int* Mp_out, const float** side_out,
                        const float** q_out) {
    std::vector<float> bt, side;
    wv::pack_stft_basis(basis.data(), n_fft, bt, side, Mp_out);
    *side_out = U.up(side);
    *q_out = U.up(wv::pack_stft_q(bt, n_fft, *Mp_out));
    return U.up(bt);
}

ResBlock pack_resblock(Uploader& U, const std::string& pre, int idx, float rs, int ks, int dil1) {
    ResBlock r{};
    r.pw1 = U.pw(pre + ".block.1.conv.conv.weight");
    r.dw1_w = U.plain(pre + ".block.2.conv.conv.weight");
    r.dw1_b = U.plain(pre + ".block.2.conv.conv.bias");
    r.pw2 = U.pw(pre + ".block.4.conv.conv.weight");
    r.dw2_w = U.plain(pre + ".block.5.conv.conv.weight");
    r.dw2_b = U.plain(pre + ".block.5.conv.conv.bias");
    r.pre_scale = (float)std::pow(1.0 + idx * (double)rs * rs, -0.5);
    r.out_scale = rs * U.scalar_or(pre + ".res_scale_param", 1.f);
    r.ks = ks; r.dil1 = dil1; r.dil2 = 1;
    if (ks == 5 && U.err == WV_OK) {
        const int C = r.pw1.M;
        r.tab1 = U.up(wv::pack_rb_table(U.host(pre + ".block.2.conv.conv.weight").data(), U.host(pre + ".block.2.conv.conv.bias").data(), C));
        r.tab2 = U.up(wv::pack_rb_table(U.host(pre + ".block.5.conv.conv.weight").data(), U.host(pre + ".block.5.conv.conv.bias").data(), C));
    }
    return r;
}

int ipow(int b, int e) { int r = 1; while (e-- > 0) r *= b; return r; }
int round_up_int(int x, int a) { return (x + a - 1) / a * a; }

int pack_model(wv_model* m) {
    const wv_config& c = m->cfg;
    Uploader U{m};
    std::vector<float> head_wc_host;
    const int S = c.n_strides, C0 = c.channels_enc;
    const float rs = c.res_scale_enc;
    m->pre_w = U.plain("encoder.conv_pre.1.conv.conv.weight");
    m->pre_b = U.plain("encoder.conv_pre.1.conv.conv.bias");
    int mult = 1, stride = 1;
    for (int s = 0; s <= S; ++s) {
        const bool post = s == S;
        const std::string pre = post ? "encoder.spec_post" : "encoder.spec_blocks." + std::to_string(s);
        if (!post) {
            std::vector<ResBlock> blocks;
            for (int j = 1; j <= c.n_residual_enc; ++j)
                blocks.push_back(pack_resblock(U, "encoder.blocks." + std::to_string(s) + "." + std::to_string(j - 1),
                                               j, rs, c.residual_kernel_size, ipow(c.dilation_base, j)));
            m->enc_blocks.push_back(std::move(blocks));
        }
        SpecLayer sp{};
        sp.n_fft = mult * c.n_fft_base; sp.hop = stride; sp.F = sp.n_fft / 2 + 1;
        auto ov = m->stft_override.find(pre + ".spec.weight");
        sp.basis_t = pack_basis(U, ov != m->stft_override.end() ? ov->second : make_basis(sp.n_fft),
                                sp.n_fft, &sp.Mp, &sp.side, &sp.basis_q);
        const int mi = post ? WV_MAX_STRIDES : s;
        sp.mean = post ? c.spec_means[WV_MAX_STRIDES] : c.spec_means[s];
        sp.inv_std = 1.f / (post ? c.spec_stds[WV_MAX_STRIDES] : c.spec_stds[s]);
        (void)mi;
        sp.pw = U.pw(pre + ".layer.conv.conv.weight");
        sp.scale = U.scalar_or(pre + ".scale_param", 1.f) * rs;
        {
            std::vector<float> taps((size_t)sp.pw.M * 5, 0.f);
            for (int mm = 0; mm < sp.pw.M; ++mm) taps[(size_t)mm * 5 + 4] = 1.f;
            sp.id_taps = U.up(taps);
        }
        m->specs.push_back(sp);
        if (!post) {
            DownLayer d{};
            const std::string dp = "encoder.downsample." + std::to_string(s);
            d.pw = U.pw(dp + ".2.conv.conv.weight");
            d.dw_w = U.plain(dp + ".3.conv.conv.weight");
            d.dw_b = U.plain(dp + ".3.conv.conv.bias");
            d.ratio = ratio_enc(c, s);
            d.pre_scale = (float)std::pow(1.0 + c.n_residual_enc * (double)rs * rs, -0.5);
            m->downs.push_back(d);
            stride *= d.ratio;
            mult *= 2;
        }
    }
    m->post_dw_w = U.plain("encoder.conv_post.1.conv.conv.weight");
    m->post_pw = U.pw("encoder.conv_post.2.conv.conv.weight");
    m->post_b = U.plain("encoder.conv_post.2.conv.conv.bias");
    (void)C0;

    m->has_film = m->params[m->index["encoder.msg_embedding.0.weight"]].set;
    if (m->has_film) {
        const int E = c.embedding_dim;
        m->f_w0 = U.plain("encoder.msg_embedding.0.weight");
        m->f_b0 = U.plain("encoder.msg_embedding.0.bias");
        std::vector<float> wl, bl, wf, bf;
        for (int l = 0; l < c.embedding_layers; ++l) {
            const std::string pre = "encoder.msg_embedding." + std::to_string(1 + 2 * l);
            const auto& w = U.host(pre + ".weight"); const auto& b = U.host(pre + ".bias");
            wl.insert(wl.end(), w.begin(), w.end()); bl.insert(bl.end(), b.begin(), b.end());
        }
        for (int s = 0; s < S; ++s)
            for (int b = 0; b < c.freq_bands; ++b)
                for (const char* nm : {"gamma", "beta"}) {
                    const std::string pre = "encoder.film_layers." + std::to_string(s) + "." +
                                            std::to_string(b) + "." + nm + "_layer";
                    const auto& w = U.host(pre + ".weight"); const auto& bb = U.host(pre + ".bias");
                    wf.insert(wf.end(), w.begin(), w.end()); bf.push_back(bb[0]);
                }
        m->f_wl = U.up(wl); m->f_bl = U.up(bl); m->f_wf = U.up(wf); m->f_bf = U.up(bf);
        (void)E;
    }

    if (c.kind == WV_KIND_GENERATOR) {
        const float rd = c.res_scale_dec;
        m->dec_pw0 = U.pw("decoder.model.0.conv.conv.weight");
        m->dec_dw0_w = U.plain("decoder.model.1.conv.conv.weight");
        m->dec_dw0_b = U.plain("decoder.model.1.conv.conv.bias");
        m->dec_post = (float)std::pow(1.0 + c.n_residual_dec * (double)rd * rd, -0.5);
        int n = 2;
        for (int i = 0; i < S; ++i) {
            UpLayer u{};
            u.ratio = c.strides[i];
            u.ct_w = U.plain("decoder.model." + std::to_string(n + 2) + ".convtr.convtr.weight");
            u.pw = U.pw("decoder.model." + std::to_string(n + 3) + ".conv.conv.weight");
            u.pw_b = U.plain("decoder.model." + std::to_string(n + 3) + ".conv.conv.bias");
            {
                std::vector<float> taps((size_t)u.pw.M * 5, 0.f);
                for (int mm = 0; mm < u.pw.M; ++mm) taps[(size_t)mm * 5 + 4] = 1.f;
                u.id_taps = U.up(taps);
                const std::vector<float>& cw = U.host("decoder.model." + std::to_string(n + 2) + ".convtr.convtr.weight");
                u.ct_wt = U.up(wv::pack_ct_wt(cw.data(), u.pw.K, u.pw.Kp, u.ratio));
            }
            u.pre_scale = i > 0 ? m->dec_post : 1.f;
            for (int j = 0; j < c.n_residual_dec; ++j)
                u.res.push_back(pack_resblock(U, "decoder.model." + std::to_string(n + 4 + j), j, rd,
                                              c.residual_kernel_size, ipow(c.dilation_base, j)));
            m->ups.push_back(std::move(u));
            n += 4 + c.n_residual_dec;
        }
        m->last_w = U.plain("decoder.model." + std::to_string(n + 2) + ".conv.conv.weight");
        m->last_b = U.plain("decoder.model." + std::to_string(n + 2) + ".conv.conv.bias");
    } else {
        const int D = c.dimension, O = c.output_dim, hop = hop_of(c);
        const int nb = c.kind == WV_KIND_DETECTOR ? c.nbits : 1;
        const auto& w1 = U.host("reverse_convolution.weight");
        const auto& b1 = U.host("reverse_convolution.bias");
        const auto& w2 = U.host("last_layer.weight");
        const auto& b2 = U.host("last_layer.bias");
        std::vector<float> wc((size_t)D * nb * hop), bc(nb);
        for (int d = 0; d < D; ++d)
            for (int nn = 0; nn < nb; ++nn)
                for (int j = 0; j < hop; ++j) {
                    double acc = 0;
                    for (int o = 0; o < O; ++o) acc += (double)w2[(size_t)nn * O + o] * w1[((size_t)d * O + o) * hop + j];
                    wc[((size_t)d * nb + nn) * hop + j] = (float)acc;
                }
        for (int nn = 0; nn < nb; ++nn) {
            double acc = b2[nn];
            for (int o = 0; o < O; ++o) acc += (double)w2[(size_t)nn * O + o] * b1[o];
            bc[nn] = (float)acc;
        }
        m->head_wc = U.up(wc); m->head_bc = U.up(bc); m->head_nb = nb;
        head_wc_host = wc;
    }
    auto rh_c = [](int C) { return C == 32 || C == 64 || C == 96 || C == 128 || C == 192 || C == 256 || C == 384 || C == 512 || C == 768; };
    bool h16_ok = c.residual_kernel_size == 5 && c.dilation_base == 1 && c.kernel_size <= 16 && c.last_kernel_size <= 16;
    for (int s = 0, C = C0; s < S && h16_ok; ++s, C *= 2) {
        h16_ok = rh_c(C) || m->enc_blocks[s].empty();
        if (C != m->specs[s].n_fft && round_up_int(m->specs[s].F, 16) > 2 * C) h16_ok = false;
        if (C % 8) h16_ok = false;
    }
    if (h16_ok) {
        int C = C0;
        for (int s = 0; s < S && U.err == WV_OK; ++s, C *= 2) {
            wv_model::H16Stage st;
            for (int j = 0; j < c.n_residual_enc; ++j)
                st.blocks.push_back(U.h16_block("encoder.blocks." + std::to_string(s) + "." + std::to_string(j), C));
            const int F = m->specs[s].F, r = ratio_enc(c, s);
            st.spec = U.h16(U.host("encoder.spec_blocks." + std::to_string(s) + ".layer.conv.conv.weight"), nullptr, C, F, 1);
            const std::string dp = "encoder.downsample." + std::to_string(s);
            st.down = U.h16(U.host(dp + ".2.conv.conv.weight"), U.host(dp + ".3.conv.conv.weight").data(), 2 * C, C, 2 * r);
            {
                const int n_fft = m->specs[s].n_fft;
                auto ov = m->stft_override.find("encoder.spec_blocks." + std::to_string(s) + ".spec.weight");
                const std::vector<float> basis = ov != m->stft_override.end() ? ov->second : make_basis(n_fft);
                std::vector<uint16_t> q4[4];
                wv::H16Weight w4[4];
                wv::pack_stft16(basis.data(), n_fft, q4, w4);
                st.cosw = U.h16_up(q4[0], w4[0]); st.sinw = U.h16_up(q4[1], w4[1]); st.cosl = U.h16_up(q4[2], w4[2]); st.sinl = U.h16_up(q4[3], w4[3]);
            }
            m->h16.push_back(std::move(st));
        }
        if (U.err == WV_OK && C % 16 == 0) {
            wv_model::H16Stage st;
            const int n_fft = m->specs[S].n_fft;
            st.spec = U.h16(U.host("encoder.spec_post.layer.conv.conv.weight"), nullptr, C, m->specs[S].F, 1);
            if ((C == n_fft && C == 1024 && m->specs[S].hop == 320) || (2 * C == n_fft && C == 128 && m->specs[S].hop == 32)) {
                auto ov = m->stft_override.find("encoder.spec_post.spec.weight");
                const std::vector<float> basis = ov != m->stft_override.end() ? ov->second : make_basis(n_fft);
                std::vector<uint16_t> q4[4];
                wv::H16Weight w4[4];
                wv::pack_stft16(basis.data(), n_fft, q4, w4);
                st.cosw = U.h16_up(q4[0], w4[0]); st.sinw = U.h16_up(q4[1], w4[1]); st.cosl = U.h16_up(q4[2], w4[2]); st.sinl = U.h16_up(q4[3], w4[3]);
            }
            {
                wv::H16Weight w;
                const std::vector<uint16_t> q = wv::pack_h16(U.host("encoder.conv_post.2.conv.conv.weight").data(), U.host("encoder.conv_post.1.conv.conv.weight").data(),
                                                             c.dimension, C, c.last_kernel_size, &w, true);
                st.post = U.h16_up(q, w);
                if (c.kind != WV_KIND_GENERATOR) {
                    wv::H16Weight wh;
                    const std::vector<uint16_t> qh = wv::pack_head16(head_wc_host.data(), c.dimension, m->head_nb, hop_of(c), &wh);
                    st.head = U.h16_up(qh, wh);
                }
            }
            m->h16.push_back(std::move(st));
        }
        bool dec_ok = c.kind == WV_KIND_GENERATOR && (int)m->h16.size() > S && c.dimension % 16 == 0 && (c.last_kernel_size == 3 || c.last_kernel_size == 5 || c.last_kernel_size == 7);
        for (size_t i = 0; i < m->ups.size() && dec_ok; ++i) dec_ok = (m->ups[i].res.empty() || rh_c(m->ups[i].pw.M)) && m->ups[i].pw.M % 16 == 0 && m->ups[i].pw.K % 16 == 0;
        if (dec_ok && U.err == WV_OK) {
            m->h16_dec_head = U.h16(U.host("decoder.model.0.conv.conv.weight"), U.host("decoder.model.1.conv.conv.weight").data(), m->dec_pw0.M, c.dimension, c.kernel_size);
            int n = 2;
            for (size_t i = 0; i < m->ups.size() && U.err == WV_OK; ++i) {
                wv_model::H16Up hu;
                const UpLayer& u = m->ups[i];
                wv::H16Weight w;
                hu.mb = wv::up16_block(u.pw.M, u.ratio) ? wv::up16_block(u.pw.M, u.ratio) : u.pw.M;
                const std::vector<uint16_t> q = wv::pack_up16(U.host("decoder.model." + std::to_string(n + 3) + ".conv.conv.weight").data(),
                                                              U.host("decoder.model." + std::to_string(n + 2) + ".convtr.convtr.weight").data(), u.pw.M, u.pw.K, u.ratio, hu.mb, &w);
                hu.up = U.h16_up(q, w);
                for (int j = 0; j < c.n_residual_dec; ++j) hu.blocks.push_back(U.h16_block("decoder.model." + std::to_string(n + 4 + j), u.pw.M));
                m->h16_ups.push_back(std::move(hu));
                n += 4 + c.n_residual_dec;
            }
        }
    }
    return U.err;
}

size_t align_up(size_t x) { return (x + 255) & ~(size_t)255; }

struct WsLayout {
    size_t act = 0;
    size_t spec = 0;
    size_t film = 0, latent = 0;
    size_t off_r0 = 0, off_r1 = 0, off_a0 = 0, off_a1 = 0, off_u = 0, off_p = 0, off_film = 0, off_lat = 0, total = 0;
};

WsLayout layout(const wv_model* m, int B, int T) {
    const wv_config& c = m->cfg;
    WsLayout L;
    size_t Tl = (size_t)T, C = (size_t)c.channels_enc, mx = C * Tl, sp = 0;
    int mult = 1;
    size_t stride = 1;
    for (int s = 0; s <= c.n_strides; ++s) {
        const size_t F = (size_t)mult * c.n_fft_base / 2 + 1;
        const size_t Tf = ((size_t)T + stride - 1) / stride;
        sp = std::max(sp, F * Tf);
        if (s < c.n_strides) {
            const int r = ratio_enc(c, s);
            Tl = (Tl + r - 1) / r; C *= 2; mx = std::max(mx, C * Tl);
            stride *= r; mult *= 2;
        }
    }
    const size_t Fr = Tl;
    if (c.kind == WV_KIND_GENERATOR) {
        size_t Cd = (size_t)c.channels_dec << c.n_strides, Td = Fr;
        mx = std::max(mx, Cd * Td);
        for (int i = 0; i < c.n_strides; ++i) { Td *= c.strides[i]; Cd /= 2; mx = std::max(mx, Cd * Td); }
    }
    L.act = (size_t)B * mx; L.spec = (size_t)B * sp;
    L.film = (size_t)B * c.n_strides * c.freq_bands * 2;
    L.latent = (size_t)B * c.dimension * Fr;
    size_t o = 0;
    L.off_r0 = o; o += align_up(L.act * 4);
    L.off_r1 = o; o += align_up(L.act * 4);
    L.off_a0 = o; o += align_up(L.act * 4);
    L.off_a1 = o; o += align_up(L.act * 4);
    L.off_u = o; o += align_up(L.act * 4);
    L.off_p = o; o += align_up(L.spec * 4);
    L.off_film = o; o += align_up(L.film * 4);
    L.off_lat = o; o += align_up(L.latent * 4);
    L.total = o;
    return L;
}

inline bool fused_block(const wv_config& c, int C, int T) {
    return (C == 64 || C == 96 || C == 128 || C == 192) && c.residual_kernel_size == 5 && c.dilation_base == 1 && (T & 3) == 0 &&
           (long long)C * T * 4 < 0x7f000000LL;
}
inline bool wants_act_copy(const wv_config& c, int C, int T) { return C >= 129 && !fused_block(c, C, T); }

struct Stream {
    float* r[2]; float* a[2]; float* u;
    float* raw = nullptr; float* act = nullptr;
    float* other_raw() const { return raw == r[0] ? r[1] : r[0]; }
    float* other_act() const { return act == a[0] ? a[1] : a[0]; }
};

int run_resblock(const ResBlock& r, Stream& st, bool want_raw, float next_scale, int B, int T, hipStream_t s,
                 const char* role) {
    wv::prof::set_role(role);
    if (st.raw && r.tab1 && r.dil1 == 1 && r.dil2 == 1) {
        wv::RbArgs f{};
        f.X = st.raw; f.pre_scale = r.pre_scale; f.pw1 = r.pw1; f.pw2 = r.pw2; f.tab1 = r.tab1; f.tab2 = r.tab2;
        f.Y = want_raw ? st.other_raw() : nullptr;
        f.Yact = next_scale > 0.f ? st.other_act() : nullptr;
        f.out_scale = r.out_scale; f.act_scale = next_scale; f.B = B; f.C = r.pw1.M; f.T = T;
        const hipError_t e = wv::launch_resblock(f, s);
        if (e == hipSuccess) { st.raw = f.Y; st.act = f.Yact; return WV_OK; }
        if (e != hipErrorNotSupported) return fail(WV_EHIP, std::string("launch_resblock: ") + hipGetErrorString(e));
    }
    wv::PwDwArgs a{};
    if (st.act) { a.X = st.act; a.pre_scale = 1.f; a.pre_elu = 0; }
    else { a.X = st.raw; a.pre_scale = r.pre_scale; a.pre_elu = 1; }
    a.pw = r.pw1; a.dw_w = r.dw1_w; a.dw_b = r.dw1_b; a.Y = nullptr; a.Yact = st.u; a.act_scale = 1.f;
    a.B = B; a.Tin = T; a.Tout = T; a.ks = r.ks; a.stride = 1; a.dil = r.dil1; a.pad = (r.ks - 1) * r.dil1;
    a.out_scale = 1.f; a.bands = 1;
    WV_HIP_TRY(wv::launch_pw_dw(a, s));
    wv::PwDwArgs b{};
    float* yr = want_raw ? st.other_raw() : nullptr;
    float* ya = next_scale > 0.f ? st.other_act() : nullptr;
    b.X = st.u; b.pw = r.pw2; b.dw_w = r.dw2_w; b.dw_b = r.dw2_b; b.resid = st.raw; b.Y = yr; b.Yact = ya;
    b.act_scale = next_scale;
    b.B = B; b.Tin = T; b.Tout = T; b.ks = r.ks; b.stride = 1; b.dil = r.dil2; b.pad = (r.ks - 1) * r.dil2;
    b.pre_scale = 1.f; b.pre_elu = 0; b.out_scale = r.out_scale; b.bands = 1;
    WV_HIP_TRY(wv::launch_pw_dw(b, s));
    st.raw = yr; st.act = ya;
    return WV_OK;
}

int run_film(wv_model* m, const float* msg, int msg_rows, float* film, int B, hipStream_t st) {
    const wv_config& c = m->cfg;
    if (!m->has_film) return fail(WV_ESTATE, "this model was finalized without message-MLP / FiLM tensors");
    if (msg_rows != B && msg_rows != 1) return fail(WV_EINVAL, "msg_rows must be B or 1");
    wv::prof::set_role("enc.film");
    wv::FilmArgs f{};
    f.msg = msg; f.msg_rows = msg_rows; f.msg_dim = c.msg_dimension; f.E = c.embedding_dim;
    f.n_layers = c.embedding_layers; f.n_out = c.n_strides * c.freq_bands * 2;
    f.w0 = m->f_w0; f.b0 = m->f_b0; f.wl = m->f_wl; f.bl = m->f_bl; f.wf = m->f_wf; f.bf = m->f_bf;
    f.film = film; f.B = B;
    WV_HIP_TRY(wv::launch_film(f, st));
    return WV_OK;
}

Stream make_stream(char* ws, const WsLayout& L) {
    Stream st{};
    st.r[0] = (float*)(ws + L.off_r0); st.r[1] = (float*)(ws + L.off_r1);
    st.a[0] = (float*)(ws + L.off_a0); st.a[1] = (float*)(ws + L.off_a1);
    st.u = (float*)(ws + L.off_u);
    return st;
}

int run_encoder(wv_model* m, const float* x, const float* msg, int msg_rows, float* latent, int B,
                int T, char* ws, const WsLayout& L, hipStream_t st, int* Fr_out, int first_stage = 0, bool post_spec_done = false) {
    const wv_config& c = m->cfg;
    Stream sm = make_stream(ws, L);
    float* P = (float*)(ws + L.off_p);
    float* film = nullptr;
    if (msg) {
        film = (float*)(ws + L.off_film);
        int rc = run_film(m, msg, msg_rows, film, B, st);
        if (rc) return rc;
    }
    int Tl = T, C = c.channels_enc;
    sm.raw = sm.r[0];
    if (first_stage > 0) {
        sm.act = nullptr;
        for (int s = 0; s < first_stage; ++s) { Tl = (Tl + ratio_enc(c, s) - 1) / ratio_enc(c, s); C *= 2; }
    } else {
        wv::prof::set_role("enc.conv_pre");
        sm.act = (m->enc_blocks[0].empty() || !wants_act_copy(c, c.channels_enc, T)) ? nullptr : sm.a[0];
        WV_HIP_TRY(wv::launch_conv_pre(x, m->pre_w, m->pre_b, sm.raw, sm.act, sm.act ? m->enc_blocks[0][0].pre_scale : 0.f,
                                   B, c.channels_enc, T, c.kernel_size, 1.f / c.wav_std, st));
    }
    const int film_stride = c.n_strides * c.freq_bands * 2;
    for (int s = first_stage; s <= c.n_strides; ++s) {
        const bool post = s == c.n_strides;
        if (!post) {
            const std::vector<ResBlock>& blocks = m->enc_blocks[s];
            for (size_t j = 0; j < blocks.size(); ++j) {
                const bool last = j + 1 == blocks.size();
                int rc = run_resblock(blocks[j], sm, true, (last || !wants_act_copy(c, C, Tl)) ? 0.f : blocks[j + 1].pre_scale, B, Tl, st,
                                      "enc.resblock");
                if (rc) return rc;
            }
        }
        if (post && post_spec_done) break;
        wv::prof::set_role("enc.spec");
        const SpecLayer& sp = m->specs[s];
        wv::StftArgs sa{};
        sa.wav = x; sa.basis_t = sp.basis_t; sa.basis_q = sp.basis_q; sa.side = sp.side; sa.P = P; sa.B = B; sa.T = T;
        sa.Tf = (T + sp.hop - 1) / sp.hop; sa.n_fft = sp.n_fft; sa.hop = sp.hop; sa.F = sp.F; sa.Mp = sp.Mp;
        sa.mean = sp.mean; sa.inv_std = sp.inv_std;
        if (sa.Tf != Tl) return fail(WV_EINVAL, "internal: STFT frame count != feature length");
        bool fused_spec = false;
        {
            wv::SpecAddArgs q{};
            q.pw = sp.pw; q.resid = sm.raw; q.out_scale = sp.scale;
            q.Y = post ? sm.raw : nullptr;
            q.Yact = post ? nullptr : sm.other_act(); q.act_scale = post ? 0.f : m->downs[s].pre_scale;
            const hipError_t e = wv::launch_stft_spec(sa, q, st);
            if (e == hipSuccess) {
                if (!post) { sm.act = q.Yact; sm.raw = nullptr; }
                fused_spec = true;
            } else if (e != hipErrorNotSupported) return fail(WV_EHIP, std::string("launch_stft_spec: ") + hipGetErrorString(e));
        }
        if (!fused_spec) {
        WV_HIP_TRY(wv::launch_stft_logmag(sa, st));
        const float down_scale = post ? 0.f : m->downs[s].pre_scale;
        if (sp.pw.M < 33 || (Tl & 3)) {
            wv::DwPwArgs k2{};
            k2.X = P; k2.pw = sp.pw; k2.Y = sm.raw; k2.B = B; k2.Tin = Tl; k2.Tout = Tl; k2.mode = 0;
            k2.pre_scale = 1.f; k2.pre_elu = 0; k2.accumulate = 1; k2.out_scale = sp.scale;
            k2.Yact = post ? nullptr : sm.other_act(); k2.act_scale = down_scale;
            WV_HIP_TRY(wv::launch_dw_pw(k2, st));
            sm.act = k2.Yact;
        } else {
            wv::PwDwArgs acc{};
            acc.X = P; acc.pw = sp.pw; acc.dw_w = sp.id_taps; acc.dw_b = nullptr; acc.resid = sm.raw;
            acc.Y = post ? sm.raw : nullptr;
            acc.Yact = post ? nullptr : sm.other_act(); acc.act_scale = down_scale;
            acc.B = B; acc.Tin = Tl; acc.Tout = Tl; acc.ks = 5; acc.stride = 1; acc.dil = 1; acc.pad = 4;
            acc.pre_scale = 1.f; acc.pre_elu = 0; acc.out_scale = sp.scale; acc.bands = 1;
            acc.spec_add = 1;
            WV_HIP_TRY(wv::launch_pw_dw(acc, st));
            if (!post) { sm.act = acc.Yact; sm.raw = nullptr; }
        }
        }
        if (post) break;
        const DownLayer& d = m->downs[s];
        wv::prof::set_role(film ? "enc.down_film" : "enc.down");
        wv::PwDwArgs a{};
        if (sm.act) { a.X = sm.act; a.pre_scale = 1.f; a.pre_elu = 0; }
        else { a.X = sm.raw; a.pre_scale = d.pre_scale; a.pre_elu = 1; }
        const bool next_has_blocks = s + 1 < c.n_strides && !m->enc_blocks[s + 1].empty() && wants_act_copy(c, 2 * C, (Tl + d.ratio - 1) / d.ratio);
        float* yr = sm.raw ? sm.other_raw() : sm.r[0];
        float* ya = next_has_blocks ? (sm.act ? sm.other_act() : sm.a[0]) : nullptr;
        a.pw = d.pw; a.dw_w = d.dw_w; a.dw_b = d.dw_b; a.Y = yr; a.Yact = ya;
        a.act_scale = next_has_blocks ? m->enc_blocks[s + 1][0].pre_scale : 0.f;
        a.B = B; a.Tin = Tl; a.Tout = (Tl + d.ratio - 1) / d.ratio;
        a.ks = 2 * d.ratio; a.stride = d.ratio; a.dil = 1; a.pad = d.ratio;
        a.out_scale = 1.f;
        a.bands = c.freq_bands; a.film_stride = film_stride;
        a.film = film ? film + (size_t)s * c.freq_bands * 2 : nullptr;
        if (film && (2 * C) % c.freq_bands) return fail(WV_EINVAL, "channels not divisible by freq_bands");
        WV_HIP_TRY(wv::launch_pw_dw(a, st));
        sm.raw = yr; sm.act = ya;
        Tl = a.Tout; C *= 2;
    }
    wv::prof::set_role("enc.conv_post");
    wv::DwPwArgs cp{};
    cp.X = sm.raw; cp.dw_w = m->post_dw_w; cp.pw = m->post_pw; cp.bias = m->post_b; cp.Y = latent;
    cp.B = B; cp.Tin = Tl; cp.Tout = Tl; cp.mode = 1; cp.ks = c.last_kernel_size;
    cp.pre_scale = 1.f; cp.pre_elu = 1; cp.l2norm = 1;
    if (c.dimension > 128) return fail(WV_EINVAL, "dimension > 128 not supported by the fused L2-norm epilogue");
    WV_HIP_TRY(wv::launch_dw_pw(cp, st));
    *Fr_out = Tl;
    return WV_OK;
}

int check_common(const wv_model* m, int B, int T, const void* ws, size_t ws_bytes, WsLayout* L) {
    if (!m) return fail(WV_EINVAL, "null model");
    if (!m->finalized) return fail(WV_ESTATE, "wv_model_finalize has not been called");
    if (B < 1 || T < 1) return fail(WV_EINVAL, "B and T must be >= 1");
    *L = layout(m, B, T);
    if (!ws || ws_bytes < L->total)
        return fail(WV_ENOMEM, "workspace too small: need " + std::to_string(L->total) + " bytes");
    return WV_OK;
}

}

extern "C" {

const char* wv_last_error(void) { return g_err.c_str(); }
#ifndef WV_SRC_HASH
#define WV_SRC_HASH "unhashed"
#endif
const char* wv_version(void) { return "waveverify_hip 0.3 (gfx950, f32 MFMA) src " WV_SRC_HASH; }

int wv_config_default(int kind, wv_config* c) {
    if (!c || kind < 0 || kind > 2) return fail(WV_EINVAL, "bad kind / null cfg");
    std::memset(c, 0, sizeof(*c));
    c->kind = kind;
    c->dimension = 128; c->msg_dimension = 16; c->channels_enc = 64; c->channels_dec = 96;
    c->n_fft_base = 64; c->n_residual_enc = 2; c->n_residual_dec = 3;
    c->n_strides = 4; const int st[4] = {8, 5, 4, 2};
    for (int i = 0; i < 4; ++i) c->strides[i] = st[i];
    c->kernel_size = 5; c->last_kernel_size = 5; c->residual_kernel_size = 5; c->dilation_base = 1;
    c->zero_init = 1; c->nbits = 16; c->output_dim = 32; c->embedding_dim = 64;
    c->embedding_layers = 2; c->freq_bands = 4;
    c->res_scale_enc = c->res_scale_dec = 0.5773502691896258f; c->wav_std = 0.1122080159f;
    const float mu[5] = {-4.554f, -4.315f, -4.021f, -3.726f, -3.477f};
    const float sd[5] = {2.830f, 2.837f, 2.817f, 2.796f, 2.871f};
    for (int i = 0; i < 5; ++i) { c->spec_means[i] = mu[i]; c->spec_stds[i] = sd[i]; }
    c->spec_means[WV_MAX_STRIDES] = mu[4]; c->spec_stds[WV_MAX_STRIDES] = sd[4];
    if (kind == WV_KIND_LOCATOR) {
        c->dimension = 64; c->channels_enc = 32; c->n_residual_enc = 1;
        c->n_strides = 2; c->strides[0] = 8; c->strides[1] = 4; c->strides[2] = c->strides[3] = 0;
    }
    return WV_OK;
}

int wv_model_create(const wv_config* cfg, wv_model** out) {
    if (!cfg || !out) return fail(WV_EINVAL, "null argument");
    if (cfg->kind < 0 || cfg->kind > 2) return fail(WV_EINVAL, "bad kind");
    if (cfg->n_strides < 1 || cfg->n_strides > WV_MAX_STRIDES) return fail(WV_EINVAL, "bad n_strides");
    for (int i = 0; i < cfg->n_strides; ++i)
        if (cfg->strides[i] < 1 || 2 * cfg->strides[i] > 16) return fail(WV_EINVAL, "stride out of range (1..8)");
    if (cfg->channels_enc < 1 || cfg->dimension < 1 || cfg->n_fft_base < 2 || (cfg->n_fft_base & 1))
        return fail(WV_EINVAL, "bad channel / fft sizes");
    if (cfg->embedding_dim > 256 || cfg->freq_bands < 1) return fail(WV_EINVAL, "bad embedding_dim / freq_bands");
    if (cfg->kernel_size > 16 || cfg->last_kernel_size > 16 || cfg->residual_kernel_size > 16)
        return fail(WV_EINVAL, "kernel sizes above 16 are not supported");
    auto* m = new wv_model();
    m->cfg = *cfg;
    build_param_table(m);
    *out = m;
    return WV_OK;
}

void wv_model_destroy(wv_model* m) { delete m; }

int wv_model_num_params(const wv_model* m) { return m ? (int)m->params.size() : 0; }

int wv_model_param_info(const wv_model* m, int i, char* name_out, int name_cap, int64_t* shape_out,
                        int* ndim_out, int* is_wn) {
    if (!m || i < 0 || i >= (int)m->params.size()) return fail(WV_EINVAL, "index out of range");
    const Param& p = m->params[i];
    if (name_out && name_cap > 0) { std::strncpy(name_out, p.name.c_str(), name_cap - 1); name_out[name_cap - 1] = 0; }
    if (shape_out) for (int d = 0; d < 4; ++d) shape_out[d] = d < (int)p.shape.size() ? p.shape[d] : 1;
    if (ndim_out) *ndim_out = (int)p.shape.size();
    if (is_wn) *is_wn = p.wn ? 1 : 0;
    return WV_OK;
}

int wv_model_set_param(wv_model* m, const char* name, const float* data, int64_t numel) {
    if (!m || !name || !data) return fail(WV_EINVAL, "null argument");
    if (m->finalized) return fail(WV_ESTATE, "model already finalized");
    auto it = m->index.find(name);
    if (it == m->index.end()) return fail(WV_ENOKEY, std::string("unknown parameter: ") + name);
    Param& p = m->params[it->second];
    if (numel != p.numel())
        return fail(WV_EINVAL, std::string("size mismatch for ") + name + ": got " + std::to_string(numel) +
                                   ", expected " + std::to_string(p.numel()));
    p.data.assign(data, data + numel);
    p.set = true;
    return WV_OK;
}

int wv_model_set_param_wn(wv_model* m, const char* name, const float* g, int64_t gn, const float* v, int64_t vn) {
    if (!m || !name || !g || !v) return fail(WV_EINVAL, "null argument");
    auto it = m->index.find(name);
    if (it == m->index.end()) return fail(WV_ENOKEY, std::string("unknown parameter: ") + name);
    Param& p = m->params[it->second];
    if (!p.wn) return fail(WV_EINVAL, std::string(name) + " is not weight-normed in the reference");
    if (vn != p.numel() || gn != p.shape[0]) return fail(WV_EINVAL, std::string("size mismatch for ") + name);
    const int64_t rows = p.shape[0], inner = vn / rows;
    std::vector<float> w((size_t)vn);
    for (int64_t r = 0; r < rows; ++r) {
        float ss = 0.f;
        for (int64_t i = 0; i < inner; ++i) ss += v[r * inner + i] * v[r * inner + i];
        const float sc = g[r] / std::sqrt(ss);
        for (int64_t i = 0; i < inner; ++i) w[(size_t)(r * inner + i)] = v[r * inner + i] * sc;
    }
    return wv_model_set_param(m, name, w.data(), vn);
}

int wv_model_set_stft_basis(wv_model* m, const char* name, const float* data, int64_t numel) {
    if (!m || !name || !data) return fail(WV_EINVAL, "null argument");
    if (m->finalized) return fail(WV_ESTATE, "model already finalized");
    const std::string n(name);
    int mult = 1; bool ok = false;
    for (int s = 0; s <= m->cfg.n_strides; ++s) {
        const std::string key = (s == m->cfg.n_strides ? std::string("encoder.spec_post")
                                                       : "encoder.spec_blocks." + std::to_string(s)) + ".spec.weight";
        const int n_fft = mult * m->cfg.n_fft_base;
        if (key == n) {
            if (numel != (int64_t)(n_fft + 2) * n_fft) return fail(WV_EINVAL, "size mismatch for " + n);
            ok = true;
        }
        mult *= 2;
    }
    if (!ok) return fail(WV_ENOKEY, "unknown STFT buffer: " + n);
    m->stft_override[n].assign(data, data + numel);
    return WV_OK;
}

int wv_model_finalize(wv_model* m) {
    if (!m) return fail(WV_EINVAL, "null model");
    if (m->finalized) return WV_OK;
    int n_film_set = 0, n_film = 0;
    for (const Param& p : m->params) {
        if (p.optional) { ++n_film; n_film_set += p.set; continue; }
        if (!p.set) return fail(WV_ENOKEY, "missing parameter: " + p.name);
    }
    if (n_film_set != 0 && n_film_set != n_film)
        return fail(WV_ENOKEY, "message-MLP / FiLM tensors must be given all or none");
    int rc = pack_model(m);
    if (rc) return rc;
    WV_HIP_TRY(hipDeviceSynchronize());
    m->finalized = true;
    for (Param& p : m->params) { p.data.clear(); p.data.shrink_to_fit(); }
    return WV_OK;
}

size_t wv_workspace_bytes(const wv_model* m, int B, int T) {
    if (!m || B < 1 || T < 1) return 0;
    return layout(m, B, T).total;
}

int wv_encoder_forward(wv_model* m, const float* x, const float* msg, int msg_rows, float* latent,
                       int B, int T, void* ws, size_t ws_bytes, void* stream) {
    WsLayout L;
    int rc = check_common(m, B, T, ws, ws_bytes, &L);
    if (rc) return rc;
    if (!x || !latent) return fail(WV_EINVAL, "null tensor");
    int Fr = 0;
    return run_encoder(m, x, msg, msg_rows, latent, B, T, (char*)ws, L, (hipStream_t)stream, &Fr);
}

int wv_generator_forward(wv_model* m, const float* x, const float* msg, int msg_rows, float* out,
                         int add_input, int B, int T, void* ws, size_t ws_bytes, void* stream) {
    WsLayout L;
    int rc = check_common(m, B, T, ws, ws_bytes, &L);
    if (rc) return rc;
    if (m->cfg.kind != WV_KIND_GENERATOR) return fail(WV_ESTATE, "not a generator model");
    if (!x || !msg || !out) return fail(WV_EINVAL, "null tensor");
    hipStream_t st = (hipStream_t)stream;
    const wv_config& c = m->cfg;
    char* w = (char*)ws;
    float* latent = (float*)(w + L.off_lat);
    int Fr = 0;
    rc = run_encoder(m, x, msg, msg_rows, latent, B, T, w, L, st, &Fr);
    if (rc) return rc;
    Stream sm = make_stream(w, L);
    wv::prof::set_role("dec.head");
    wv::PwDwArgs h{};
    h.X = latent; h.pw = m->dec_pw0; h.dw_w = m->dec_dw0_w; h.dw_b = m->dec_dw0_b;
    h.Y = nullptr; h.Yact = sm.a[0]; h.act_scale = m->ups.empty() ? 1.f : m->ups[0].pre_scale;
    h.B = B; h.Tin = Fr; h.Tout = Fr; h.ks = c.kernel_size; h.stride = 1; h.dil = 1; h.pad = c.kernel_size - 1;
    h.pre_scale = 1.f; h.pre_elu = 0; h.out_scale = 1.f; h.bands = 1;
    WV_HIP_TRY(wv::launch_pw_dw(h, st));
    sm.raw = nullptr; sm.act = sm.a[0];
    int Tl = Fr;
    for (size_t i = 0; i < m->ups.size(); ++i) {
        const UpLayer& u = m->ups[i];
        const bool last_up = i + 1 == m->ups.size();
        const float stage_next = last_up ? 0.f : m->ups[i + 1].pre_scale;
        wv::prof::set_role("dec.upsample");
        wv::PwDwArgs a{};
        a.X = sm.act; a.ct_w = u.ct_w; a.ct_wt = u.ct_wt; a.ratio = u.ratio; a.pw = u.pw; a.dw_w = u.id_taps; a.dw_b = u.pw_b;
        const bool has_blocks = !u.res.empty();
        a.Y = (has_blocks || last_up) ? sm.r[0] : nullptr;
        const bool blocks_act = has_blocks && wants_act_copy(c, u.pw.M, Tl * u.ratio);
        a.Yact = has_blocks ? (blocks_act ? sm.other_act() : nullptr) : (last_up ? nullptr : sm.other_act());
        a.act_scale = has_blocks ? u.res[0].pre_scale : stage_next;
        a.B = B; a.Tin = Tl; a.Tout = Tl * u.ratio; a.ks = 5; a.stride = 1; a.dil = 1; a.pad = 4;
        a.pre_scale = 1.f; a.pre_elu = 0; a.out_scale = 1.f; a.bands = 1;
        WV_HIP_TRY(wv::launch_pw_dw(a, st));
        sm.raw = a.Y; sm.act = a.Yact;
        Tl = a.Tout;
        for (size_t j = 0; j < u.res.size(); ++j) {
            const bool last = j + 1 == u.res.size();
            const float next = last ? stage_next : (wants_act_copy(c, u.pw.M, Tl) ? u.res[j + 1].pre_scale : 0.f);
            rc = run_resblock(u.res[j], sm, !last || last_up, next, B, Tl, st, "dec.resblock");
            if (rc) return rc;
        }
    }
    wv::prof::set_role("dec.tail");
    WV_HIP_TRY(wv::launch_tail(sm.raw, m->last_w, m->last_b, add_input ? x : nullptr, out, B, c.channels_dec,
                           Tl, T, c.last_kernel_size, m->dec_post, c.wav_std, st));
    return WV_OK;
}

enum { H16_TAIL_F32 = 0, H16_TAIL_LATENT = 1 };
static int run_encoder_stages_f16(wv_model* m, const float* x, const float* film, int B, int T, char* ws, const WsLayout& L, hipStream_t st, int tail,
                                  bool* post_done, bool* latent_done, int* Fr_out) {
    const wv_config& c = m->cfg;
    const int S = c.n_strides;
    void* R[2] = {ws + L.off_r0, ws + L.off_r1};
    void* A0 = ws + L.off_a0;
    float* P = (float*)(ws + L.off_p);
    void* P16 = ws + L.off_u;
    int cur = 0, Tl = T, C = c.channels_enc;
    const int film_stride = c.n_strides * c.freq_bands * 2;
    wv::prof::set_role("enc16.conv_pre");
    WV_HIP_TRY(wv::launch_conv_pre16(x, m->pre_w, m->pre_b, R[0], B, C, T, c.kernel_size, 1.f / c.wav_std, st));
    for (int s = 0; s < S; ++s) {
        const wv_model::H16Stage& hs = m->h16[s];
        wv::prof::set_role("enc16.resblock");
        for (size_t j = 0; j < m->enc_blocks[s].size(); ++j) {
            const ResBlock& r = m->enc_blocks[s][j];
            wv::RhArgs a{};
            a.X = R[cur]; a.pre_scale = r.pre_scale; a.w1 = hs.blocks[j].w1; a.w2 = hs.blocks[j].w2; a.tab1 = hs.blocks[j].tab1; a.tab2 = hs.blocks[j].tab2;
            a.Y = R[cur ^ 1]; a.Yact = nullptr; a.out_scale = r.out_scale; a.act_scale = 0.f; a.B = B; a.C = C; a.T = Tl;
            const hipError_t e = wv::launch_resblock16(a, st);
            if (e != hipSuccess) return fail(e == hipErrorNotSupported ? WV_ESTATE : WV_EHIP, std::string("launch_resblock16: ") + hipGetErrorString(e));
            cur ^= 1;
        }
        wv::prof::set_role("enc16.spec");
        const SpecLayer& sp = m->specs[s];
        wv::StftArgs sa{};
        sa.wav = x; sa.basis_t = sp.basis_t; sa.basis_q = sp.basis_q; sa.side = sp.side; sa.P = P; sa.B = B; sa.T = T;
        sa.Tf = (T + sp.hop - 1) / sp.hop; sa.n_fft = sp.n_fft; sa.hop = sp.hop; sa.F = sp.F; sa.Mp = sp.Mp;
        sa.mean = sp.mean; sa.inv_std = sp.inv_std;
        if (sa.Tf != Tl) return fail(WV_EINVAL, "internal: STFT frame count != feature length");
        const DownLayer& d = m->downs[s];
        wv::Spec16Args f{};
        f.wav = x; f.side = sp.side; f.cosw = hs.cosw; f.sinw = hs.sinw; f.cosl = hs.cosl; f.sinl = hs.sinl; f.pw = hs.spec; f.resid = R[cur]; f.Y = nullptr; f.Yact = A0;
        f.out_scale = sp.scale; f.act_scale = d.pre_scale; f.c1 = 0.5f * 0.6931471805599453f * sp.inv_std; f.c0 = -sp.mean * sp.inv_std;
        f.B = B; f.T = T; f.Tf = Tl; f.n_fft = sp.n_fft; f.hop = sp.hop;
        const hipError_t fe = (C == sp.n_fft || 2 * C == sp.n_fft) ? wv::launch_spec16(f, st) : hipErrorNotSupported;
        if (fe != hipSuccess && fe != hipErrorNotSupported) return fail(WV_EHIP, std::string("launch_spec16: ") + hipGetErrorString(fe));
        if (fe == hipErrorNotSupported) {
            if ((size_t)B * round_up_int(sp.F, 16) * Tl * 2 > L.act * 4) return fail(WV_ESTATE, "f16 mode: the spectrogram of this scale does not fit its staging buffer");
            WV_HIP_TRY(wv::launch_stft_logmag(sa, st));
            WV_HIP_TRY(wv::launch_f32_to_c8(P, P16, B, sp.F, Tl, 1.f, 0, st));
            wv::Conv16Args q{};
            q.X = P16; q.w = hs.spec; q.bias = nullptr; q.resid = R[cur]; q.Y = nullptr; q.Yact = A0; q.Yf32 = nullptr;
            q.out_scale = sp.scale; q.act_scale = d.pre_scale; q.B = B; q.M = C; q.Tin = Tl; q.Tout = Tl; q.ks = 1; q.stride = 1; q.pad = 0;
            WV_HIP_TRY(wv::launch_conv16(q, st));
        }
        wv::prof::set_role(film ? "enc16.down_film" : "enc16.down");
        const bool last = s + 1 == S, post16 = (int)m->h16.size() > S;
        wv::Conv16Args g{};
        g.X = A0; g.w = hs.down; g.bias = d.dw_b; g.resid = nullptr; g.Y = (last && !post16) ? nullptr : R[cur ^ 1]; g.Yact = nullptr;
        g.Yf32 = (last && !post16) ? (float*)R[0] : nullptr; g.out_scale = 1.f; g.act_scale = 0.f;
        g.B = B; g.M = 2 * C; g.Tin = Tl; g.Tout = (Tl + d.ratio - 1) / d.ratio; g.ks = 2 * d.ratio; g.stride = d.ratio; g.pad = d.ratio;
        if (film) {
            if ((2 * C) % c.freq_bands) return fail(WV_EINVAL, "channels not divisible by freq_bands");
            g.film = film + (size_t)s * c.freq_bands * 2; g.bands = c.freq_bands; g.film_stride = film_stride;
        }
        WV_HIP_TRY(wv::launch_conv16(g, st));
        cur ^= 1; Tl = g.Tout; C *= 2;
    }
    *post_done = false; *latent_done = false; *Fr_out = Tl;
    if ((int)m->h16.size() > S) {
        wv::prof::set_role("enc16.spec_post");
        const SpecLayer& sp = m->specs[S];
        const wv_model::H16Stage& hs = m->h16[S];
        if ((T + sp.hop - 1) / sp.hop != Tl) return fail(WV_EINVAL, "internal: STFT frame count != feature length");
        const bool latent = tail == H16_TAIL_LATENT && hs.post.wq && c.last_kernel_size <= 16;
        float* f32out = latent ? nullptr : (float*)R[cur ^ 1];
        bool done = false;
        if (hs.cosw.wq) {
            wv::Spec16Args f{};
            f.wav = x; f.side = sp.side; f.cosw = hs.cosw; f.sinw = hs.sinw; f.cosl = hs.cosl; f.sinl = hs.sinl; f.pw = hs.spec; f.resid = R[cur]; f.Y = nullptr;
            f.Yact = latent ? A0 : nullptr; f.Yf32 = f32out;
            f.out_scale = sp.scale; f.act_scale = latent ? 1.f : 0.f; f.c1 = 0.5f * 0.6931471805599453f * sp.inv_std; f.c0 = -sp.mean * sp.inv_std;
            f.B = B; f.T = T; f.Tf = Tl; f.n_fft = sp.n_fft; f.hop = sp.hop;
            const hipError_t fe = wv::launch_spec16(f, st);
            if (fe == hipSuccess) done = true;
            else if (fe != hipErrorNotSupported) return fail(WV_EHIP, std::string("launch_spec16 (post): ") + hipGetErrorString(fe));
        }
        if (!done && (size_t)B * round_up_int(sp.F, 16) * Tl * 2 <= L.act * 4 && (size_t)B * sp.F * Tl <= L.spec) {
            wv::StftArgs sa{};
            sa.wav = x; sa.basis_t = sp.basis_t; sa.basis_q = sp.basis_q; sa.side = sp.side; sa.P = P; sa.B = B; sa.T = T;
            sa.Tf = Tl; sa.n_fft = sp.n_fft; sa.hop = sp.hop; sa.F = sp.F; sa.Mp = sp.Mp; sa.mean = sp.mean; sa.inv_std = sp.inv_std;
            WV_HIP_TRY(wv::launch_stft_logmag(sa, st));
            WV_HIP_TRY(wv::launch_f32_to_c8(P, P16, B, sp.F, Tl, 1.f, 0, st));
            wv::Conv16Args q{};
            q.X = P16; q.w = hs.spec; q.bias = nullptr; q.resid = R[cur]; q.Y = nullptr; q.Yact = latent ? A0 : nullptr; q.Yf32 = f32out;
            q.out_scale = sp.scale; q.act_scale = latent ? 1.f : 0.f; q.B = B; q.M = C; q.Tin = Tl; q.Tout = Tl; q.ks = 1; q.stride = 1; q.pad = 0;
            WV_HIP_TRY(wv::launch_conv16(q, st));
            done = true;
        }
        if (done && latent) {
            wv::prof::set_role("enc16.conv_post");
            wv::Conv16Args g{};
            g.X = A0; g.w = hs.post; g.bias = m->post_b; g.resid = nullptr; g.Y = nullptr; g.Yact = nullptr; g.Yf32 = (float*)(ws + L.off_lat);
            g.out_scale = 1.f; g.act_scale = 0.f; g.B = B; g.M = c.dimension; g.Tin = Tl; g.Tout = Tl; g.ks = c.last_kernel_size; g.stride = 1;
            g.pad = c.last_kernel_size - 1;
            WV_HIP_TRY(wv::launch_conv16(g, st));
            *post_done = true; *latent_done = true;
            return WV_OK;
        }
        if (done) {
            if ((cur ^ 1) != 0) WV_HIP_TRY(hipMemcpyAsync(R[0], R[1], (size_t)B * C * Tl * sizeof(float), hipMemcpyDeviceToDevice, st));
            *post_done = true;
            return WV_OK;
        }
        WV_HIP_TRY(wv::launch_c8_to_f32(R[cur], (float*)R[cur ^ 1], B, C, Tl, st));
        if ((cur ^ 1) != 0) WV_HIP_TRY(hipMemcpyAsync(R[0], R[1], (size_t)B * C * Tl * sizeof(float), hipMemcpyDeviceToDevice, st));
    }
    return WV_OK;
}

static int run_head_model(wv_model* m, const float* x, float* logits, float* mean_prob, int B, int T,
                          void* ws, size_t ws_bytes, void* stream, bool f16 = false,
                          const int* keep_lo = nullptr, const int* keep_hi = nullptr, float* psum = nullptr) {
    WsLayout L;
    int rc = check_common(m, B, T, ws, ws_bytes, &L);
    if (rc) return rc;
    if (!x || (!logits && !mean_prob && !psum)) return fail(WV_EINVAL, "null tensor");
    hipStream_t st = (hipStream_t)stream;
    char* w = (char*)ws;
    float* latent = (float*)(w + L.off_lat);
    int Fr = 0;
    bool post_done = false;
    if (f16) {
        if (m->h16.empty()) return fail(WV_ESTATE, "this model has no f16 plan (ResnetBlock stages of 32 ... 768 channels, k = 5, dilation 1)");
        const wv_config& c = m->cfg;
        const int D = c.dimension, hop = hop_of(c);
        const bool head16 = !logits && (int)m->h16.size() > c.n_strides && m->h16.back().head.wq && D % 16 == 0 && D <= 128 && m->head_nb % 4 == 0 && m->head_nb <= 32 && hop % 32 == 0;
        bool latent_done = false;
        rc = run_encoder_stages_f16(m, x, nullptr, B, T, w, L, st, head16 ? H16_TAIL_LATENT : H16_TAIL_F32, &post_done, &latent_done, &Fr);
        if (rc) return rc;
        if (latent_done) {
            wv::prof::set_role("head16");
            const hipError_t e2 = wv::launch_head16(latent, m->h16.back().head, m->head_bc, mean_prob, B, D, m->head_nb, hop, Fr, T, st,
// ... 157 lines not shown
```

### waveverify_amd/csrc/wv_ops.hip

```cpp
#include <hip/hip_runtime.h>

#include <cmath>
#include <cstring>
#include <string>
#include <vector>

#include "wv_host.h"
#include "wv_kernels.h"

namespace {

using wv::al256;
using wv::fail;

struct Tmp {
    std::vector<void*> d;
    bool ok = true;
    const float* up(const float* h, size_t n) {
        if (!h || !ok) return nullptr;
        void* p = nullptr;
        if (hipMalloc(&p, std::max<size_t>(n, 1) * sizeof(float)) != hipSuccess) { ok = false; return nullptr; }
        d.push_back(p);
        if (n && hipMemcpy(p, h, n * sizeof(float), hipMemcpyHostToDevice) != hipSuccess) { ok = false; return nullptr; }
        return (const float*)p;
    }
    const float* upv(const std::vector<float>& v) { return up(v.data(), v.size()); }
    const void* upb(const void* h, size_t bytes) {
        if (!h || !ok) return nullptr;
        void* p = nullptr;
        if (hipMalloc(&p, std::max<size_t>(bytes, 16)) != hipSuccess) { ok = false; return nullptr; }
        d.push_back(p);
        if (bytes && hipMemcpy(p, h, bytes, hipMemcpyHostToDevice) != hipSuccess) { ok = false; return nullptr; }
        return p;
    }
    wv::H16Weight h16(const float* pw, const float* dw, int M, int K, int ks) {
        wv::H16Weight w;
        const std::vector<uint16_t> q = wv::pack_h16(pw, dw, M, K, ks, &w);
        w.wq = upb(q.data(), q.size() * sizeof(uint16_t));
        return w;
    }
    wv::PwWeight pw(const float* w, int M, int K) {
        wv::PwWeight p; p.M = M; p.K = K; p.Kp = wv::round_up(K, wv::BK); p.Mp = wv::round_up(M, wv::M_ALIGN);
        std::vector<float> t((size_t)p.Kp * p.Mp, 0.f);
        for (int m = 0; m < M; ++m)
            for (int k = 0; k < K; ++k) t[(size_t)k * p.Mp + m] = w[(size_t)m * K + k];
        p.wt = upv(t);
        std::vector<float> q((size_t)wv::round_up(K, 32) * p.Mp, 0.f);
        for (int mm = 0; mm < M; ++mm)
            for (int k = 0; k < K; ++k) q[((size_t)(k / 4) * p.Mp + mm) * 4 + (k & 3)] = w[(size_t)mm * K + k];
        p.wq = upv(q);
        return p;
    }
    ~Tmp() { (void)hipDeviceSynchronize(); for (void* p : d) (void)hipFree(p); }
};

int launched(hipError_t e) {
    if (e == hipErrorInvalidValue) return fail(WV_EINVAL, "the launcher refused the arguments (a shape or pointer outside the kernel's limits)");
    WV_HIP_TRY(e);
    return WV_OK;
}
int unsupported(const std::string& covers) { return fail(WV_EINVAL, "the call is outside what the fused kernel covers: " + covers); }
const char* const FUSED_GATES = "; activations 16-byte aligned, one clip's tensor within the kernel's 32-bit byte offsets";

int done(Tmp& t, hipError_t e, hipStream_t s) {
    if (!t.ok) return fail(WV_EHIP, "device allocation or upload of the weights failed");
    if (int rc = launched(e)) return rc;
    WV_HIP_TRY(hipStreamSynchronize(s));
    return WV_OK;
}

}

extern "C" {

int wv_op_pw_dw(const float* X, const float* w_pw, const float* w_dw, const float* dw_bias,
                const float* film, const float* resid, float* Y, int B, int K, int M, int Tin,
                int ks, int stride, int dilation, float pre_scale, int pre_elu, float out_scale,
                int bands, float* Yact, float act_scale, void* stream) {
    if (!X || !w_pw || !w_dw || (!Y && !Yact) || B < 1 || K < 1 || M < 1 || Tin < 1) return fail(WV_EINVAL, "null pointer (X, w_pw, w_dw, or both Y and Yact) or B, K, M, Tin < 1");
    Tmp t;
    wv::PwDwArgs a{};
    a.X = X; a.pw = t.pw(w_pw, M, K); a.dw_w = t.up(w_dw, (size_t)M * ks);
    a.dw_b = t.up(dw_bias, M); a.film = film; a.resid = resid; a.Y = Y; a.Yact = Yact; a.act_scale = act_scale;
    a.B = B; a.Tin = Tin; a.Tout = (Tin + stride - 1) / stride; a.ks = ks; a.stride = stride;
    a.dil = dilation; a.pad = (ks - 1) * dilation - (stride - 1);
    a.pre_scale = pre_scale; a.pre_elu = pre_elu; a.out_scale = out_scale;
    a.bands = bands > 0 ? bands : 1; a.film_stride = 2 * a.bands;
    if (a.pad < 0) return fail(WV_EINVAL, "negative left pad: (ks - 1) * dilation < stride - 1");
    return done(t, wv::launch_pw_dw(a, (hipStream_t)stream), (hipStream_t)stream);
}

int wv_op_resblock(const float* X, float pre_scale, const float* w_pw1, const float* w_dw1, const float* b1,
                   const float* w_pw2, const float* w_dw2, const float* b2, float* Y, float* Yact,
                   int B, int C, int T, float out_scale, float act_scale, void* stream) {
    if (!X || !w_pw1 || !w_dw1 || !w_pw2 || !w_dw2 || (!Y && !Yact) || B < 1 || C < 1 || T < 1) return fail(WV_EINVAL, "null pointer (X, a weight, or both Y and Yact) or B, C, T < 1");
    Tmp t;
    wv::RbArgs a{};
    a.X = X; a.pre_scale = pre_scale; a.pw1 = t.pw(w_pw1, C, C); a.pw2 = t.pw(w_pw2, C, C);
    a.tab1 = t.upv(wv::pack_rb_table(w_dw1, b1, C)); a.tab2 = t.upv(wv::pack_rb_table(w_dw2, b2, C));
    a.Y = Y; a.Yact = Yact; a.out_scale = out_scale; a.act_scale = act_scale; a.B = B; a.C = C; a.T = T;
    const hipError_t e = wv::launch_resblock(a, (hipStream_t)stream);
    if (e == hipErrorNotSupported) return unsupported(std::string("C in {64, 96, 128, 192}, T % 4 == 0") + FUSED_GATES);
    return done(t, e, (hipStream_t)stream);
}

int wv_h16_round_host(const float* in, uint16_t* out, int64_t n) {
    if (!in || !out || n < 0) return fail(WV_EINVAL, "null pointer or n < 0");
    for (int64_t i = 0; i < n; ++i) out[i] = wv::f32_to_f16_bits(in[i]);
    return WV_OK;
}
int wv_h16_from_f32(const float* X, void* Y16, int B, int C, int T, float scale, int elu, void* stream) {
    Tmp t;
    return done(t, wv::launch_f32_to_c8(X, Y16, B, C, T, scale, elu, (hipStream_t)stream), (hipStream_t)stream);
}
int wv_h16_to_f32(const void* X16, float* Y, int B, int C, int T, void* stream) {
    Tmp t;
    return done(t, wv::launch_c8_to_f32(X16, Y, B, C, T, (hipStream_t)stream), (hipStream_t)stream);
}
int wv_h16_conv_pre(const float* x, const float* w, const float* bias, void* Y16, int B, int C, int T, int ks, float in_scale, void* stream) {
    if (!x || !w || !Y16 || C < 1 || ks < 1) return fail(WV_EINVAL, "null pointer (x, w, Y16) or C, ks < 1");
    Tmp t;
    return done(t, wv::launch_conv_pre16(x, t.up(w, (size_t)C * ks), t.up(bias, C), Y16, B, C, T, ks, in_scale, (hipStream_t)stream), (hipStream_t)stream);
}
int wv_h16_resblock(const void* X16, float pre_scale, const float* w_pw1, const float* w_dw1, const float* b1, const float* w_pw2, const float* w_dw2,
                    const float* b2, void* Y16, void* Yact16, int B, int C, int T, float out_scale, float act_scale, void* stream) {
    if (!X16 || !w_pw1 || !w_dw1 || !w_pw2 || !w_dw2 || (!Y16 && !Yact16) || B < 1 || C < 1 || T < 1) return fail(WV_EINVAL, "null pointer (X16, a weight, or both Y16 and Yact16) or B, C, T < 1");
    Tmp t;
    wv::RhArgs a{};
    a.X = X16; a.pre_scale = pre_scale;
    { const std::vector<uint16_t> q = wv::pack_rh_pw(w_pw1, C, &a.w1); a.w1.wq = t.upb(q.data(), q.size() * sizeof(uint16_t)); }
    { const std::vector<uint16_t> q = wv::pack_rh_pw(w_pw2, C, &a.w2); a.w2.wq = t.upb(q.data(), q.size() * sizeof(uint16_t)); }
    a.tab1 = t.upv(wv::pack_rh_table(w_dw1, b1, C, wv::RH_LOG2E)); a.tab2 = t.upv(wv::pack_rh_table(w_dw2, b2, C, 1.0));
    a.Y = Y16; a.Yact = Yact16; a.out_scale = out_scale; a.act_scale = act_scale; a.B = B; a.C = C; a.T = T;
    const hipError_t e = wv::launch_resblock16(a, (hipStream_t)stream);
    if (e == hipErrorNotSupported) return unsupported(std::string("C in {32, 64, 96, 128, 192, 256, 384, 512, 768}") + FUSED_GATES);
    return done(t, e, (hipStream_t)stream);
}
int wv_h16_conv(const void* X16, const float* w_pw, const float* w_dw, const float* bias, const void* resid16, void* Y16, void* Yact16, float* Yf32,
                int B, int K, int M, int Tin, int ks, int stride, int pad, float out_scale, float act_scale, void* stream) {
    if (!X16 || !w_pw || B < 1 || K < 1 || M < 1 || Tin < 1 || ks < 1 || stride < 1 || pad < 0) return fail(WV_EINVAL, "null pointer (X16, w_pw), B, K, M, Tin, ks, stride < 1 or pad < 0");
    Tmp t;
    wv::Conv16Args a{};
    a.X = X16; a.w = t.h16(w_pw, w_dw, M, K, ks); a.bias = t.up(bias, M); a.resid = resid16; a.Y = Y16; a.Yact = Yact16; a.Yf32 = Yf32;
    a.out_scale = out_scale; a.act_scale = act_scale; a.B = B; a.M = M; a.Tin = Tin; a.Tout = (Tin + stride - 1) / stride;
    a.ks = ks; a.stride = stride; a.pad = pad;
    return done(t, wv::launch_conv16(a, (hipStream_t)stream), (hipStream_t)stream);
}

int wv_op_dw_pw(const float* X, const float* w_dw, const float* w_pw, const float* bias, float* Y,
                int B, int K, int M, int Tin, int mode, int ks_or_ratio, float pre_scale, int pre_elu,
                int l2norm, int accumulate, float out_scale, float* Yact, float act_scale, void* stream) {
    if (!X || !w_pw || !Y || B < 1 || K < 1 || M < 1 || Tin < 1) return fail(WV_EINVAL, "null pointer (X, w_pw, Y) or B, K, M, Tin < 1");
    if (mode == 2 && !l2norm && !accumulate) {
        if (!w_dw || ks_or_ratio < 1) return fail(WV_EINVAL, "mode 2 (upsample) needs w_dw and a ratio >= 1");
        Tmp t;
        std::vector<float> taps((size_t)M * 5, 0.f);
        for (int m = 0; m < M; ++m) taps[(size_t)m * 5 + 4] = 1.f;
        wv::PwDwArgs a{};
        a.X = X; a.pw = t.pw(w_pw, M, K); a.ct_w = t.up(w_dw, (size_t)K * 2 * ks_or_ratio); a.ratio = ks_or_ratio;
        a.ct_wt = t.upv(wv::pack_ct_wt(w_dw, K, a.pw.Kp, ks_or_ratio));
        a.dw_w = t.upv(taps); a.dw_b = t.up(bias, M); a.Y = Y; a.Yact = Yact; a.act_scale = act_scale;
        a.B = B; a.Tin = Tin; a.Tout = Tin * ks_or_ratio; a.ks = 5; a.stride = 1; a.dil = 1; a.pad = 4;
        a.pre_scale = pre_scale; a.pre_elu = pre_elu; a.out_scale = 1.f; a.bands = 1;
        a.film_stride = 2;
        return done(t, wv::launch_pw_dw(a, (hipStream_t)stream), (hipStream_t)stream);
    }
    Tmp t;
    wv::DwPwArgs a{};
    a.X = X; a.pw = t.pw(w_pw, M, K); a.bias = t.up(bias, M); a.Y = Y;
    a.B = B; a.Tin = Tin; a.mode = mode; a.Tout = Tin;
    if (mode == 2) return fail(WV_EINVAL, "mode 2 (upsample) has neither L2-norm nor accumulate");
    const bool k1_form = mode == 0 && accumulate && !l2norm && !bias && M >= 128;
    if (Yact && !k1_form) return fail(WV_EINVAL, "Yact exists only in mode 2 and in the accumulate form with M >= 128");
    if (mode == 0 && accumulate && !l2norm && !bias && M >= 128) {
        Tmp t;
        std::vector<float> taps((size_t)M * 5, 0.f);
        for (int m = 0; m < M; ++m) taps[(size_t)m * 5 + 4] = 1.f;
        wv::PwDwArgs a{};
        a.X = X; a.pw = t.pw(w_pw, M, K); a.dw_w = t.upv(taps); a.resid = Y; a.Y = Y; a.Yact = Yact; a.act_scale = act_scale;
        a.B = B; a.Tin = Tin; a.Tout = Tin; a.ks = 5; a.stride = 1; a.dil = 1; a.pad = 4;
        a.pre_scale = pre_scale; a.pre_elu = pre_elu; a.out_scale = out_scale; a.bands = 1; a.film_stride = 2;
        a.spec_add = 1;
        return done(t, wv::launch_pw_dw(a, (hipStream_t)stream), (hipStream_t)stream);
    }
    if (mode == 1) { a.ks = ks_or_ratio; a.dw_w = t.up(w_dw, (size_t)K * a.ks); }
    a.pre_scale = pre_scale; a.pre_elu = pre_elu; a.l2norm = l2norm; a.accumulate = accumulate;
    a.out_scale = out_scale;
    return done(t, wv::launch_dw_pw(a, (hipStream_t)stream), (hipStream_t)stream);
}

static std::vector<float> stft_basis_host(const float* basis_or_null, int n_fft) {
    const int F = n_fft / 2 + 1;
    std::vector<float> basis((size_t)2 * F * n_fft);
    if (basis_or_null) {
        std::memcpy(basis.data(), basis_or_null, basis.size() * sizeof(float));
    } else {
        const float c = (float)(-2.0 * M_PI / n_fft), wc = (float)(2.0 * M_PI / n_fft);
        for (int k = 0; k < F; ++k) {
            volatile float ck = c * (float)k;
            for (int n = 0; n < n_fft; ++n) {
                volatile float ang = ck * (float)n;
                volatile float wa = (float)n * wc;
                const float win = 0.5f - 0.5f * (float)std::cos((double)wa);
                basis[(size_t)k * n_fft + n] = (float)std::cos((double)ang) * win;
                basis[(size_t)(F + k) * n_fft + n] = (float)std::sin((double)ang) * win;
            }
        }
    }
    return basis;
}

int wv_op_stft_logmag(const float* wav, const float* basis_or_null, float* P, int B, int T, int n_fft,
                      int hop, float mean, float std, void* stream) {
    if (!wav || !P || B < 1 || T < 1 || hop < 1) return fail(WV_EINVAL, "null pointer (wav, P) or B, T, hop < 1");
    if (n_fft < 4 || (n_fft & 1)) return fail(WV_EINVAL, "n_fft must be even and >= 4");
    const int F = n_fft / 2 + 1;
    const std::vector<float> basis = stft_basis_host(basis_or_null, n_fft);
    std::vector<float> bt, side;
    int Mp = 0;
    wv::pack_stft_basis(basis.data(), n_fft, bt, side, &Mp);
    Tmp t;
    wv::StftArgs a{};
    a.wav = wav; a.basis_t = t.upv(bt); a.basis_q = t.upv(wv::pack_stft_q(bt, n_fft, Mp)); a.side = t.upv(side); a.P = P; a.B = B; a.T = T; a.Tf = (T + hop - 1) / hop;
    a.n_fft = n_fft; a.hop = hop; a.F = F; a.Mp = Mp; a.mean = mean; a.inv_std = 1.f / std;
    return done(t, wv::launch_stft_logmag(a, (hipStream_t)stream), (hipStream_t)stream);
}

int wv_op_spec_block(const float* wav, const float* basis_or_null, const float* w_pw, const float* x, float* Y, float* Yact, int B, int T,
                     int n_fft, int hop, int M, float mean, float std, float out_scale, float act_scale, void* stream) {
    if (!wav || !w_pw || !x || (!Y && !Yact) || B < 1 || T < 1 || hop < 1 || M < 1) return fail(WV_EINVAL, "null pointer (wav, w_pw, x, or both Y and Yact) or B, T, hop, M < 1");
    if (n_fft < 4 || (n_fft & 1)) return fail(WV_EINVAL, "n_fft must be even and >= 4");
    const int F = n_fft / 2 + 1;
    const std::vector<float> basis = stft_basis_host(basis_or_null, n_fft);
    std::vector<float> bt, side;
    int Mp = 0;
    wv::pack_stft_basis(basis.data(), n_fft, bt, side, &Mp);
    Tmp t;
    wv::StftArgs a{};
    a.wav = wav; a.basis_t = t.upv(bt); a.basis_q = t.upv(wv::pack_stft_q(bt, n_fft, Mp)); a.side = t.upv(side); a.P = nullptr; a.B = B; a.T = T;
    a.Tf = (T + hop - 1) / hop; a.n_fft = n_fft; a.hop = hop; a.F = F; a.Mp = Mp; a.mean = mean; a.inv_std = 1.f / std;
    wv::SpecAddArgs q{};
    q.pw = t.pw(w_pw, M, F); q.resid = x; q.Y = Y; q.Yact = Yact; q.out_scale = out_scale; q.act_scale = act_scale;
    const hipError_t e = wv::launch_stft_spec(a, q, (hipStream_t)stream);
    if (e == hipErrorNotSupported) return unsupported(std::string("n_fft = M in {64, 128}, more than 64 frames, ceil(T / hop) % 4 == 0") + FUSED_GATES);
    return done(t, e, (hipStream_t)stream);
}

int wv_h16_upsample(const void* X16, const float* w_ct, const float* w_pw, const float* bias, void* Y16, void* Yact16,
                    int B, int K, int M, int Tin, int ratio, float act_scale, void* stream) {
    if (!X16 || !w_ct || !w_pw || (!Y16 && !Yact16) || B < 1 || K < 1 || M < 1 || Tin < 1 || ratio < 1) return fail(WV_EINVAL, "null pointer (X16, w_ct, w_pw, or both Y16 and Yact16) or B, K, M, Tin, ratio < 1");
    Tmp t;
    wv::Conv16Args a{};
    const int mb = wv::up16_block(M, ratio) ? wv::up16_block(M, ratio) : M;
    { const std::vector<uint16_t> q = wv::pack_up16(w_pw, w_ct, M, K, ratio, mb, &a.w); a.w.wq = t.upb(q.data(), q.size() * sizeof(uint16_t)); }
    a.up_mb = mb;
    a.X = X16; a.bias = t.up(bias, M); a.Y = Y16; a.Yact = Yact16; a.out_scale = 1.f; a.act_scale = act_scale;
    a.B = B; a.M = M * ratio; a.Tin = Tin; a.Tout = Tin; a.ks = 2; a.stride = 1; a.pad = 1; a.up = ratio;
    return done(t, wv::launch_conv16(a, (hipStream_t)stream), (hipStream_t)stream);
}
int wv_h16_tail(const void* A16, const float* w, const float* bias, const float* x, float* out, int B, int C, int Tin, int T, int ks,
                float out_scale, void* stream) {
    if (!A16 || !w || !out || C < 1 || ks < 1) return fail(WV_EINVAL, "null pointer (A16, w, out) or C, ks < 1");
    Tmp t;
    const hipError_t e = wv::launch_tail16(A16, t.up(w, (size_t)C * ks), t.up(bias, 1), x, out, B, C, Tin, T, ks, out_scale, (hipStream_t)stream);
    if (e == hipErrorNotSupported) return unsupported("ks in {3, 5, 7}");
    return done(t, e, (hipStream_t)stream);
}
int wv_h16_l2norm(const float* lat, void* Y16, int B, int D, int Fr, void* stream) {
    Tmp t;
    return done(t, wv::launch_l2norm_c8(lat, Y16, B, D, Fr, (hipStream_t)stream), (hipStream_t)stream);
}
int wv_h16_head(const float* lat, const float* wc, const float* bc, float* mean_prob, int B, int D, int nb, int hop, int Fr, int T,
                const int* keep_lo, const int* keep_hi, float* psum, void* stream) {
    if (!lat || !wc || !bc || B < 1 || D < 1 || nb < 1 || hop < 1 || Fr < 1 || T < 1) return fail(WV_EINVAL, "null pointer (lat, wc, bc) or B, D, nb, hop, Fr, T < 1");
    if ((long long)(Fr - 1) * hop >= T || (long long)Fr * hop < T) return fail(WV_EINVAL, "Fr is not ceil(T / hop)");
    if (D % 16 || D > 128 || nb % 4 || nb > 32 || hop % 32) return fail(WV_EINVAL, "head limits: D % 16 == 0, D <= 128, nb % 4 == 0, nb <= 32, hop % 32 == 0");
    Tmp t;
    wv::H16Weight w;
    const std::vector<uint16_t> q = wv::pack_head16(wc, D, nb, hop, &w);
    w.wq = t.upb(q.data(), q.size() * sizeof(uint16_t));
    const hipError_t e = wv::launch_head16(lat, w, t.up(bc, nb), mean_prob, B, D, nb, hop, Fr, T, (hipStream_t)stream, keep_lo, keep_hi, psum);
    if (e == hipErrorNotSupported) return unsupported("D % 16 == 0, D <= 128, nb % 4 == 0, nb <= 32, hop % 32 == 0, and a weight pack of exactly that shape");
    return done(t, e, (hipStream_t)stream);
}
int wv_h16_conv_film(const void* X16, const float* w_pw, const float* w_dw, const float* bias, const float* film, int bands, void* Y16, void* Yact16,
                     int B, int K, int M, int Tin, int ks, int stride, int pad, float act_scale, void* stream) {
    if (!X16 || !w_pw || !film || bands < 1 || B < 1 || K < 1 || M < 1 || Tin < 1 || ks < 1 || stride < 1 || pad < 0) return fail(WV_EINVAL, "null pointer (X16, w_pw, film), bands, B, K, M, Tin, ks, stride < 1 or pad < 0");
    Tmp t;
    wv::Conv16Args a{};
    a.X = X16; a.w = t.h16(w_pw, w_dw, M, K, ks); a.bias = t.up(bias, M); a.Y = Y16; a.Yact = Yact16;
    a.out_scale = 1.f; a.act_scale = act_scale; a.B = B; a.M = M; a.Tin = Tin; a.Tout = (Tin + stride - 1) / stride; a.ks = ks; a.stride = stride; a.pad = pad;
    a.film = film; a.bands = bands; a.film_stride = 2 * bands;
    return done(t, wv::launch_conv16(a, (hipStream_t)stream), (hipStream_t)stream);
}
int wv_h16_spec_block(const float* wav, const float* basis_or_null, const float* w_pw, const void* x16, void* Y16, void* Yact16, int B, int T,
                      int n_fft, int hop, int M, float mean, float std_, float out_scale, float act_scale, void* stream) {
    if (!wav || !w_pw || !x16 || (!Y16 && !Yact16) || B < 1 || T < 1 || n_fft < 2 || (n_fft & 1) || hop < 1 || (M != n_fft && 2 * M != n_fft) || !(std_ > 0.f)) return fail(WV_EINVAL, "null pointer (wav, w_pw, x16, or both Y16 and Yact16), B, T, hop < 1, n_fft odd or < 2, M not n_fft or n_fft / 2, or std <= 0");
    Tmp t;
    const std::vector<float> basis = stft_basis_host(basis_or_null, n_fft);
    std::vector<uint16_t> q4[4];
    wv::H16Weight w4[4];
    wv::Spec16Args a{};
    wv::pack_stft16(basis.data(), n_fft, q4, w4);
    for (int k = 0; k < 4; ++k) w4[k].wq = t.upb(q4[k].data(), q4[k].size() * sizeof(uint16_t));
    a.cosw = w4[0]; a.sinw = w4[1]; a.cosl = w4[2]; a.sinl = w4[3];
    std::vector<float> bt, side;
    wv::pack_stft_basis(basis.data(), n_fft, bt, side, nullptr);
    a.side = t.up(side.data(), side.size());
    a.pw = t.h16(w_pw, nullptr, M, n_fft / 2 + 1, 1);
    a.wav = wav; a.resid = x16; a.Y = Y16; a.Yact = Yact16; a.out_scale = out_scale; a.act_scale = act_scale;
    a.c1 = 0.5f * 0.69314718055994531f / std_; a.c0 = -mean / std_;
    a.B = B; a.T = T; a.Tf = (T + hop - 1) / hop; a.n_fft = n_fft; a.hop = hop;
    const hipError_t e = wv::launch_spec16(a, (hipStream_t)stream);
    if (e == hipErrorNotSupported) return unsupported(std::string("(n_fft, hop) in {(64,1),(128,2),(256,8),(512,40),(1024,320)} with M = n_fft, {(64,1),(128,4),(256,32)} with M = n_fft / 2") + FUSED_GATES);
    return done(t, e, (hipStream_t)stream);
}

}

struct wv_stft_plan {
    int n_fft = 0, Mp = 0;
    float *basis_t = nullptr, *basis_q = nullptr, *side = nullptr;
    float *wt_fwd = nullptr, *wt_bwd = nullptr;
    ~wv_stft_plan() { (void)hipFree(basis_t); (void)hipFree(basis_q); (void)hipFree(side); (void)hipFree(wt_fwd); (void)hipFree(wt_bwd); }
};

namespace {
__global__ __launch_bounds__(256) void stft_frames_kernel(const float* __restrict__ wav, float* __restrict__ X, int T, int Tf, int n_fft, int hop) {
    const int n = blockIdx.y, b = blockIdx.z;
    const int t = blockIdx.x * 256 + threadIdx.x;
    if (t >= Tf) return;
    const int sidx = t * hop + n - (n_fft - 1);
    X[((size_t)b * n_fft + n) * Tf + t] = (sidx >= 0 && sidx < T) ? wav[(size_t)b * T + sidx] : 0.f;
// ... 187 lines not shown
```

Baseline: 3447 clips/s.

## Add pointwise epilogue to K1 instead of emulating 1x1 with identity k5 taps

Adds an EPI_PW epilogue variant in the fused pointwise/depthwise kernel that applies only bias (plus residual/activation) when there is no depthwise conv. Spectral accumulate and decoder upsample layers previously ran a 5-tap depthwise filter with identity taps, which needed DPP lane shifts, 5 FMAs per output and 4 padding columns per clip. The new path removes those, shrinks the per-row table to a single bias, and changes flat-column geometry so no pad columns are needed. Dispatch, validation and fallbacks are extended to accept a null dw_w, which adds template instances and a new code path whose correctness depends on the modified flat indexing.

```diff
diff --git a/waveverify_amd/csrc/wv_k1.hip b/waveverify_amd/csrc/wv_k1.hip
--- a/waveverify_amd/csrc/wv_k1.hip
+++ b/waveverify_amd/csrc/wv_k1.hip
@@ -98,11 +98,14 @@
     }
 };
 
+constexpr int EPI_PW = 3;
 template <class C, int EPI, int RES>
 struct K1Epi {
     static constexpr int NT = C::NT, HLD = C::HLD;
-    static constexpr int NTAP = EPI == 0 ? 5 : (EPI == 2 ? 4 : (EPI == 4 ? 8 : 16));
-    static constexpr int WLD = EPI == 0 ? 8 : NTAP + 4;
+    static constexpr bool ACC = EPI == 0 || EPI == EPI_PW;
+    static constexpr int NTAP = EPI == 0 ? 5 : (EPI == EPI_PW ? 0 : (EPI == 2 ? 4 : (EPI == 4 ? 8 : 16)));
+    static constexpr int WLD = EPI == 0 ? 8 : (EPI == EPI_PW ? 1 : NTAP + 4);
+    static_assert((C::BM * WLD) % 4 == 0, "the LDR 6 / 7 window buffer behind the table is DMA'd in 16-byte pieces");
     static constexpr int TABLE_FLOATS = C::BM * WLD;
     static constexpr bool HASR = RES == 1 || RES == 2 || RES == 5;
     static constexpr bool RAWH = RES == 4 || RES == 5;
@@ -173,7 +176,7 @@
         vec = act_lane && to + NT - 1 < p.Tout && o + NT - 1 < p.tto && (p.Tout % NT) == 0;
         nrec = M * p.Tout * 4;
         voff0 = act_lane ? ((m0 + 32 * wave + 4 * half) * p.Tout + to) * 4 : 0x7f000000;
-        if (EPI == 0 && p.flat) {
+        if (ACC && p.flat) {
             const long long gc = gflat + p.pad + o;
             const int bo2 = (int)(gc / p.Tv), t = (int)(gc - (long long)bo2 * p.Tv) - p.pad;
             const bool ok = o < p.tto && bo2 < p.B && t >= 0;
@@ -201,8 +204,9 @@
         for (int m = tid; m < C::BM; m += C::NTHREADS) {
             const int gm = m0 + m;
             float* row = Wl + m * WLD;
-#pragma unroll
-            for (int i = 0; i < NTAP; ++i) row[i] = (gm < M && i < p.ks) ? p.dw_w[(size_t)gm * p.ks + i] : 0.f;
+            if constexpr (EPI == EPI_PW) { row[0] = (gm < M && p.dw_b) ? p.dw_b[gm] : 0.f; continue; }
+#pragma unroll
+            for (int i = 0; i < NTAP; ++i) row[i] = (gm < M && i < p.ks) ? (p.dw_w ? p.dw_w[(size_t)gm * p.ks + i] : (i == p.ks - 1 ? 1.f : 0.f)) : 0.f;
             float gam = 1.f, bet = 0.f;
             if (filmb && gm < M) { const int band = gm / bw; gam = filmb[2 * band]; bet = filmb[2 * band + 1]; }
             row[NTAP] = (gm < M && p.dw_b) ? p.dw_b[gm] : 0.f;
@@ -222,7 +226,7 @@
     }
 
     __device__ __forceinline__ void finish(f32x16 (&acc)[NT], const PwDwArgs& p, float* strips) {
-        if constexpr (EPI == 0) {
+        if constexpr (ACC) {
             constexpr int NSH = 4 / NT;
             const int clip_bytes = nrec;
             const __amdgpu_buffer_rsrc_t rY = uniform_rsrc(Yb ? Yb : p.Yact, Yb ? clip_bytes : 0);
@@ -230,7 +234,7 @@
             const __amdgpu_buffer_rsrc_t rR = uniform_rsrc(Rb ? Rb : p.X, Rb ? clip_bytes : 0);
             const int row_bytes = p.Tout * 4;
             const int voff = voff0;
-            const float* Wrow = Wl + (32 * wave + 4 * half) * 8;
+            const float* Wrow = Wl + (32 * wave + 4 * half) * WLD;
             ovec res4[HASR ? 4 : 1];
             ovec add4[RES == 2 ? 4 : 1];
             const __amdgpu_buffer_rsrc_t rR2 = uniform_rsrc(Rb2 ? Rb2 : p.X, Rb2 ? clip_bytes : 0);
@@ -245,32 +249,40 @@
 #pragma unroll
                 for (int r = 0; r < 4; ++r) add4[r] = buf_load(rR2, voff + ((r & 3) + 8 * (r >> 2)) * row_bytes);
             }
-            f32x4 w0n = *reinterpret_cast<const f32x4*>(Wrow), w1n = *reinterpret_cast<const f32x4*>(Wrow + 4);
+            f32x4 w0n = *reinterpret_cast<const f32x4*>(Wrow), w1n = w0n, bq = w0n;
+            if constexpr (EPI == 0) w1n = *reinterpret_cast<const f32x4*>(Wrow + 4);
 #pragma unroll
             for (int r = 0; r < 16; ++r) {
                 const int cr = (r & 3) + 8 * (r >> 2);
-                const f32x4 w0 = w0n, w1 = w1n;
-                if (r + 1 < 16) {
-                    const int cn = ((r + 1) & 3) + 8 * ((r + 1) >> 2);
-                    w0n = *reinterpret_cast<const f32x4*>(Wrow + cn * 8);
-                    w1n = *reinterpret_cast<const f32x4*>(Wrow + cn * 8 + 4);
-                }
-                float hh[NT + 4], cur[NT];
-#pragma unroll
-                for (int e = 0; e < NT; ++e) { cur[e] = acc[e][r]; hh[e] = cur[e]; }
-#pragma unroll
-                for (int s2 = 1; s2 <= NSH; ++s2) {
-#pragma unroll
-                    for (int e = 0; e < NT; ++e) { cur[e] = dpp_next(cur[e]); hh[s2 * NT + e] = cur[e]; }
-                }
                 const int off = voff + cr * row_bytes;
                 ovec y;
-#pragma unroll
-                for (int e = 0; e < NT; ++e) {
-                    float v = fmaf(w0.x, hh[e], w1.y);
-                    v = fmaf(w0.y, hh[e + 1], v); v = fmaf(w0.z, hh[e + 2], v);
-                    v = fmaf(w0.w, hh[e + 3], v); v = fmaf(w1.x, hh[e + 4], v);
-                    y[e] = v;
+                float hc[NT];
+                if constexpr (EPI == 0) {
+                    const f32x4 w0 = w0n, w1 = w1n;
+                    if (r + 1 < 16) {
+                        const int cn = ((r + 1) & 3) + 8 * ((r + 1) >> 2);
+                        w0n = *reinterpret_cast<const f32x4*>(Wrow + cn * 8);
+                        w1n = *reinterpret_cast<const f32x4*>(Wrow + cn * 8 + 4);
+                    }
+                    float hh[NT + 4], cur[NT];
+#pragma unroll
+                    for (int e = 0; e < NT; ++e) { cur[e] = acc[e][r]; hh[e] = cur[e]; }
+#pragma unroll
+                    for (int s2 = 1; s2 <= NSH; ++s2) {
+#pragma unroll
+                        for (int e = 0; e < NT; ++e) { cur[e] = dpp_next(cur[e]); hh[s2 * NT + e] = cur[e]; }
+                    }
+#pragma unroll
+                    for (int e = 0; e < NT; ++e) {
+                        float v = fmaf(w0.x, hh[e], w1.y);
+                        v = fmaf(w0.y, hh[e + 1], v); v = fmaf(w0.z, hh[e + 2], v);
+                        v = fmaf(w0.w, hh[e + 3], v); v = fmaf(w1.x, hh[e + 4], v);
+                        y[e] = v; hc[e] = hh[e + 4];
+                    }
+                } else {
+                    if ((r & 3) == 0) { bq = w0n; if (r + 4 < 16) w0n = *reinterpret_cast<const f32x4*>(Wrow + 8 * ((r + 4) >> 2)); }
+#pragma unroll
+                    for (int e = 0; e < NT; ++e) { hc[e] = acc[e][r]; y[e] = hc[e] + bq[r & 3]; }
                 }
                 if constexpr (HASR) {
                     const ovec rr = res4[r & 3];
@@ -297,7 +309,7 @@
                 if constexpr (RAWH) {
                     ovec hraw;
 #pragma unroll
-                    for (int e = 0; e < NT; ++e) hraw[e] = hh[e + 4];
+                    for (int e = 0; e < NT; ++e) hraw[e] = hc[e];
                     buf_store(rH, off, hraw);
                 }
                 if (Yb) buf_store(rY, off, y);
@@ -438,7 +450,7 @@
     typedef K1Epi<C, EPI, RES> Epi;
     typedef typename LdrSel<LDR>::type LB;
     typedef typename NVec<C::NT>::type bvec;
-    constexpr bool FLAT_OK = EPI == 0 || EPI == 8;
+    constexpr bool FLAT_OK = EPI == 0 || EPI == EPI_PW || EPI == 8;
     TileId tile = decode_tile(p);
     if (FLAT_OK && p.flat) {
         const unsigned L = blockIdx.x, j = L >> 3;
@@ -477,7 +489,7 @@
     else {
         const float* Xt = Xb;
         int c0 = ti0, ncols = p.Tin, tout = p.Tout;
-        if (EPI == 0 && p.flat) {
+        if ((EPI == 0 || EPI == EPI_PW) && p.flat) {
             const long long g = gflat + 4 * cg;
             const int bb = (int)(g / p.Tv), t = (int)(g - (long long)bb * p.Tv) - p.pad;
             const bool inb = bb < p.B;
@@ -596,6 +608,8 @@
     epi.finish(acc, p, smem);
 }
 
+bool k1_pointwise(const PwDwArgs& a) { return a.ks == 1 && a.stride == 1 && a.dil == 1 && a.pad == 0 && !a.dw_w && !a.film; }
+
 static bool aligned16(const void* p) { return (reinterpret_cast<uintptr_t>(p) & 15) == 0; }
 
 bool k1_supported(const PwDwArgs& a) {
@@ -608,6 +622,7 @@
     if (a.resid && !aligned16(a.resid)) return false;
     if ((a.resid2 && !aligned16(a.resid2)) || (a.Yraw && !aligned16(a.Yraw)) || (a.Ysum && !aligned16(a.Ysum))) return false;
     if (a.ks < 1 || a.ks > 16 || (a.ks - 1) * a.dil + 1 + 3 > 64) return false;
+    if (!a.dw_w && !k1_pointwise(a) && !(a.ks == 5 && a.stride == 1 && a.dil == 1 && a.pad == 4 && !a.film)) return false;
     if (a.ct_w && a.ratio == 1) return false;
     return true;
 }
@@ -622,7 +637,7 @@
     a.stagger = 0; a.first_gen = 0;
     long long n_act = (long long)a.num_t * a.B;
     if (a.flat) {
-        if (!(C::NT == 4 && (EPI == 0 || (EPI == 8 && LDR == 0)))) return hipErrorInvalidValue;
+        if (!(C::NT == 4 && (EPI == 0 || EPI == EPI_PW || (EPI == 8 && LDR == 0)))) return hipErrorInvalidValue;
         n_act = EPI == 8 ? ((long long)a.B * (a.Tv / 8) + a.tto - 1) / a.tto : ((long long)a.B * a.Tv - a.pad + a.tto - 1) / a.tto;
         if (n_act > 0x7fffffffLL) return hipErrorInvalidValue;
         a.num_t = (int)n_act;
@@ -645,30 +660,34 @@
 template <class C, int EPI, int RES>
 static hipError_t k1_pick_ldr(const PwDwArgs& a, hipStream_t s) {
     if (a.ct_w) {
-        if constexpr (EPI == 0 && RES == 0) {
+        if constexpr ((EPI == 0 || EPI == EPI_PW) && RES == 0) {
 #ifndef K1_NO_LDS_UPSAMPLE
             if (!a.flat && a.pre_scale == 1.f && !a.pre_elu && a.pw.K % C::BKC == 0 && a.Tin % 4 == 0 && a.Tout == a.Tin * a.ratio && C::BM <= 128) {
-                if (a.ratio % 4 == 0) return k1_run<C, 0, 6, false>(a, s, "convtr_pw_lds");
-                if (a.ratio == 2) return k1_run<C, 0, 7, false>(a, s, "convtr_pw_lds");
+                if (a.ratio % 4 == 0) return k1_run<C, EPI, 6, false>(a, s, "convtr_pw_lds");
+                if (a.ratio == 2) return k1_run<C, EPI, 7, false>(a, s, "convtr_pw_lds");
             }
 #endif
-            if (a.ratio % 4 == 0) return k1_run<C, 0, 2, false>(a, s, "convtr_pw");
-            if (a.ratio == 2) return k1_run<C, 0, 3, false>(a, s, "convtr_pw");
-            return k1_run<C, 0, 5, false>(a, s, "convtr_pw");
+            if (a.ratio % 4 == 0) return k1_run<C, EPI, 2, false>(a, s, "convtr_pw");
+            if (a.ratio == 2) return k1_run<C, EPI, 3, false>(a, s, "convtr_pw");
+            return k1_run<C, EPI, 5, false>(a, s, "convtr_pw");
         }
         return hipErrorInvalidValue;
     }
-    const char* base = a.spec_add ? "spec_add" : (EPI == 0 ? (RES == 2 ? "pw_dw_k5_dact" : RES == 4 ? "pw_dw_k5_h" : RES == 5 ? "pw_dw_k5_hres" : RES ? "pw_dw_k5" : "pw_dw_k5_nr") : (EPI == 1 ? "pw_dw" : "pw_dw_s"));
+    const char* base = a.spec_add ? "spec_add" : (EPI == EPI_PW ? (RES ? "pw_dw_k1" : "pw_dw_k1_nr") : EPI == 0 ? (RES == 2 ? "pw_dw_k5_dact" : RES == 4 ? "pw_dw_k5_h" : RES == 5 ? "pw_dw_k5_hres" : RES ? "pw_dw_k5" : "pw_dw_k5_nr") : (EPI == 1 ? "pw_dw" : "pw_dw_s"));
     if (a.pre_elu || a.pre_scale != 1.f) return k1_run<C, EPI, 1, RES>(a, s, base);
     if constexpr (C::NT == 4 && C::BM == 128) {
-        if (EPI == 0 && a.pw.K >= 256) return k1_run<C, EPI, 0, RES, 3>(a, s, base);
+        if ((EPI == 0 || EPI == EPI_PW) && a.pw.K >= 256) return k1_run<C, EPI, 0, RES, 3>(a, s, base);
     }
     return k1_run<C, EPI, 0, RES>(a, s, base);
 }
 
 template <class C>
-static hipError_t k1_pick_epi(const PwDwArgs& a, hipStream_t s, bool k5) {
+static hipError_t k1_pick_epi(const PwDwArgs& a, hipStream_t s, bool k5, bool pw) {
     const bool res = a.resid != nullptr;
+    if (pw) {
+        if (a.res_mode == 2 || a.Yraw || a.Ysum) return hipErrorInvalidValue;
+        return res ? k1_pick_ldr<C, EPI_PW, true>(a, s) : k1_pick_ldr<C, EPI_PW, false>(a, s);
+    }
     if (a.res_mode == 2) {
         if (!k5 || !res) return hipErrorNotSupported;
         return k1_pick_ldr<C, 0, 2>(a, s);
@@ -692,9 +711,13 @@
 
 hipError_t launch_k1(const PwDwArgs& a0, hipStream_t s) {
     PwDwArgs a = a0;
+#ifdef K1_NO_POINTWISE
+    if (k1_pointwise(a)) { a.ks = 5; a.pad = 4; }
+#endif
     const bool k5 = a.ks == 5 && a.stride == 1 && a.dil == 1 && a.pad == 4 && !a.film;
+    const bool pw = k1_pointwise(a);
     const int need = (a.ks - 1) * a.dil + 1;
-    bool narrow = (a.ct_w ? a.Tout : a.Tin) + a.pad + 3 <= 64;
+    bool narrow = (a.ct_w ? a.Tout : a.Tin) + a.pad + (pw ? 0 : 3) <= 64;
     if (!narrow) {
         PwDwArgs g128 = a, g64 = a;
         if (pw_dw_geometry(g128, 128) && pw_dw_geometry(g64, 64)) {
@@ -705,11 +728,11 @@
     }
     (void)need;
     a.flat = 0;
-    if (k5 && a.B > 1 && (a.Tout & 3) == 0) {
+    if ((k5 || pw) && a.B > 1 && (a.Tout & 3) == 0) {
         int bm = 128, best = (a.pw.M + 127) / 128 * 128;
         for (int cand : {96, 64}) { const int pd = (a.pw.M + cand - 1) / cand * cand; if (pd < best) { best = pd; bm = cand; } }
-        const long long Tv = a.Tout + 4;
-        const long long flat_cols = ((long long)a.B * Tv - 4 + 123) / 124 * 128;
+        const long long Tv = a.Tout + a.pad;
+        const long long flat_cols = pw ? ((long long)a.B * Tv + 127) / 128 * 128 : ((long long)a.B * Tv - 4 + 123) / 124 * 128;
         PwDwArgs g = a;
         const int bn = narrow ? 64 : 128;
         long long clip_cols = -1;
@@ -734,14 +757,15 @@
         if (padded < best) { best = padded; bm = cand; }
     }
     if (narrow) {
-        if (bm == 128) return k1_pick_epi<K1<2, 32, 128>>(a, s, k5);
-        if (bm == 96) return k1_pick_epi<K1<2, 32, 96>>(a, s, k5);
-        return k1_pick_epi<K1<2, 32, 64>>(a, s, k5);
-    }
-    if (a.ct_w && k5 && !narrow && !a.resid && !a.Yraw && a.res_mode != 2 && a.pw.M % 256 == 0) return k1_pick_ldr<K1<4, 16, 256>, 0, false>(a, s);
-    if (bm == 128) return k1_pick_epi<K1<4, 16, 128>>(a, s, k5);
-    if (bm == 96) return k1_pick_epi<K1<4, 16, 96>>(a, s, k5);
-    return k1_pick_epi<K1<4, 16, 64>>(a, s, k5);
+        if (bm == 128) return k1_pick_epi<K1<2, 32, 128>>(a, s, k5, pw);
+        if (bm == 96) return k1_pick_epi<K1<2, 32, 96>>(a, s, k5, pw);
+        return k1_pick_epi<K1<2, 32, 64>>(a, s, k5, pw);
+    }
+    if (a.ct_w && (k5 || pw) && !narrow && !a.resid && !a.Yraw && a.res_mode != 2 && a.pw.M % 256 == 0)
+        return pw ? k1_pick_ldr<K1<4, 16, 256>, EPI_PW, false>(a, s) : k1_pick_ldr<K1<4, 16, 256>, 0, false>(a, s);
+    if (bm == 128) return k1_pick_epi<K1<4, 16, 128>>(a, s, k5, pw);
+    if (bm == 96) return k1_pick_epi<K1<4, 16, 96>>(a, s, k5, pw);
+    return k1_pick_epi<K1<4, 16, 64>>(a, s, k5, pw);
 }
 
 
diff --git a/waveverify_amd/csrc/wv_kernels.h b/waveverify_amd/csrc/wv_kernels.h
--- a/waveverify_amd/csrc/wv_kernels.h
+++ b/waveverify_amd/csrc/wv_kernels.h
@@ -48,6 +48,7 @@
 };
 hipError_t launch_pw_dw(const PwDwArgs& a, hipStream_t s);
 bool k1_supported(const PwDwArgs& a);
+bool k1_pointwise(const PwDwArgs& a);
 hipError_t launch_k1(const PwDwArgs& a, hipStream_t s);
 bool pw_dw_geometry(PwDwArgs& a, int BN);
 struct RbArgs {
diff --git a/waveverify_amd/csrc/wv_kernels.hip b/waveverify_amd/csrc/wv_kernels.hip
--- a/waveverify_amd/csrc/wv_kernels.hip
+++ b/waveverify_amd/csrc/wv_kernels.hip
@@ -279,7 +279,7 @@
                 float v[8] = {0, 0, 0, 0, 0, 0, 1.f, 0};
                 if (gm < M) {
 #pragma unroll
-                    for (int i = 0; i < KS; ++i) v[i] = p.dw_w[(size_t)gm * KS + i];
+                    for (int i = 0; i < KS; ++i) v[i] = p.dw_w ? p.dw_w[(size_t)gm * KS + i] : (i == KS - 1 ? 1.f : 0.f);
                     v[5] = p.dw_b ? p.dw_b[gm] : 0.f;
                     if (filmb) { const int band = gm / bw; v[6] = filmb[2 * band]; v[7] = filmb[2 * band + 1]; }
                 }
@@ -1076,10 +1076,13 @@
     return 128;
 }
 
-hipError_t launch_pw_dw(const PwDwArgs& a, hipStream_t s) {
-    if (a.ct_w && (!a.ct_wt || (reinterpret_cast<uintptr_t>(a.ct_wt) & 7) || a.ratio < 1 || a.Tout != a.Tin * a.ratio || a.ks != 5 || a.stride != 1 || a.dil != 1 || a.pad != 4 ||
+hipError_t launch_pw_dw(const PwDwArgs& a0, hipStream_t s) {
+    PwDwArgs a = a0;
+    const bool k5 = a.ks == 5 && a.stride == 1 && a.dil == 1 && a.pad == 4;
+    if (a.ct_w && (!a.ct_wt || (reinterpret_cast<uintptr_t>(a.ct_wt) & 7) || a.ratio < 1 || a.Tout != a.Tin * a.ratio || !(k5 || k1_pointwise(a)) ||
                    (reinterpret_cast<uintptr_t>(a.ct_w) & 15)))
         return hipErrorInvalidValue;
+    if (!a.dw_w && !k1_pointwise(a) && !(k5 && !a.film)) return hipErrorInvalidValue;
     if (a.ks < 1 || a.ks > 16 || a.stride < 1 || a.dil < 1 || a.pad < 0 || a.pw.Mp % M_ALIGN || a.pw.Kp % BK || !a.pw.wq)
         return hipErrorInvalidValue;
     if (k1_supported(a)) {
@@ -1087,6 +1090,7 @@
         if (e != hipErrorNotSupported) return e;
     }
     if (a.res_mode || a.Yraw || a.Ysum) return hipErrorNotSupported;
+    if (k1_pointwise(a)) { a.ks = 5; a.pad = 4; }
     const int need = (a.ks - 1) * a.dil + 1;
     bool narrow = a.Tin + a.pad + 3 <= 64 && need + 3 <= 64;
     if (!narrow && need + 3 <= 64) {
diff --git a/waveverify_amd/csrc/wv_model.hip b/waveverify_amd/csrc/wv_model.hip
--- a/waveverify_amd/csrc/wv_model.hip
+++ b/waveverify_amd/csrc/wv_model.hip
@@ -38,12 +38,10 @@
 struct SpecLayer {
     const float* basis_t; const float* basis_q; const float* side; int n_fft, hop, F, Mp; float mean, inv_std;
     PwWeight pw; float scale;
-    const float* id_taps;
 };
 struct DownLayer { PwWeight pw; const float *dw_w, *dw_b; int ratio; float pre_scale; };
 struct UpLayer {
     const float* ct_w; int ratio; PwWeight pw; const float* pw_b; float pre_scale;
-    const float* id_taps;
     const float* ct_wt;
     std::vector<ResBlock> res;
 };
@@ -336,11 +334,6 @@
         (void)mi;
         sp.pw = U.pw(pre + ".layer.conv.conv.weight");
         sp.scale = U.scalar_or(pre + ".scale_param", 1.f) * rs;
-        {
-            std::vector<float> taps((size_t)sp.pw.M * 5, 0.f);
-            for (int mm = 0; mm < sp.pw.M; ++mm) taps[(size_t)mm * 5 + 4] = 1.f;
-            sp.id_taps = U.up(taps);
-        }
         m->specs.push_back(sp);
         if (!post) {
             DownLayer d{};
@@ -397,9 +390,6 @@
             u.pw = U.pw("decoder.model." + std::to_string(n + 3) + ".conv.conv.weight");
             u.pw_b = U.plain("decoder.model." + std::to_string(n + 3) + ".conv.conv.bias");
             {
-                std::vector<float> taps((size_t)u.pw.M * 5, 0.f);
-                for (int mm = 0; mm < u.pw.M; ++mm) taps[(size_t)mm * 5 + 4] = 1.f;
-                u.id_taps = U.up(taps);
                 const std::vector<float>& cw = U.host("decoder.model." + std::to_string(n + 2) + ".convtr.convtr.weight");
                 u.ct_wt = U.up(wv::pack_ct_wt(cw.data(), u.pw.K, u.pw.Kp, u.ratio));
             }
@@ -690,10 +680,10 @@
             sm.act = k2.Yact;
         } else {
             wv::PwDwArgs acc{};
-            acc.X = P; acc.pw = sp.pw; acc.dw_w = sp.id_taps; acc.dw_b = nullptr; acc.resid = sm.raw;
+            acc.X = P; acc.pw = sp.pw; acc.dw_w = nullptr; acc.dw_b = nullptr; acc.resid = sm.raw;
             acc.Y = post ? sm.raw : nullptr;
             acc.Yact = post ? nullptr : sm.other_act(); acc.act_scale = down_scale;
-            acc.B = B; acc.Tin = Tl; acc.Tout = Tl; acc.ks = 5; acc.stride = 1; acc.dil = 1; acc.pad = 4;
+            acc.B = B; acc.Tin = Tl; acc.Tout = Tl; acc.ks = 1; acc.stride = 1; acc.dil = 1; acc.pad = 0;
             acc.pre_scale = 1.f; acc.pre_elu = 0; acc.out_scale = sp.scale; acc.bands = 1;
             acc.spec_add = 1;
             WV_HIP_TRY(wv::launch_pw_dw(acc, st));
@@ -923,13 +913,13 @@
         const float stage_next = last_up ? 0.f : m->ups[i + 1].pre_scale;
         wv::prof::set_role("dec.upsample");
         wv::PwDwArgs a{};
-        a.X = sm.act; a.ct_w = u.ct_w; a.ct_wt = u.ct_wt; a.ratio = u.ratio; a.pw = u.pw; a.dw_w = u.id_taps; a.dw_b = u.pw_b;
+        a.X = sm.act; a.ct_w = u.ct_w; a.ct_wt = u.ct_wt; a.ratio = u.ratio; a.pw = u.pw; a.dw_w = nullptr; a.dw_b = u.pw_b;
         const bool has_blocks = !u.res.empty();
         a.Y = (has_blocks || last_up) ? sm.r[0] : nullptr;
         const bool blocks_act = has_blocks && wants_act_copy(c, u.pw.M, Tl * u.ratio);
         a.Yact = has_blocks ? (blocks_act ? sm.other_act() : nullptr) : (last_up ? nullptr : sm.other_act());
         a.act_scale = has_blocks ? u.res[0].pre_scale : stage_next;
-        a.B = B; a.Tin = Tl; a.Tout = Tl * u.ratio; a.ks = 5; a.stride = 1; a.dil = 1; a.pad = 4;
+        a.B = B; a.Tin = Tl; a.Tout = Tl * u.ratio; a.ks = 1; a.stride = 1; a.dil = 1; a.pad = 0;
         a.pre_scale = 1.f; a.pre_elu = 0; a.out_scale = 1.f; a.bands = 1;
         WV_HIP_TRY(wv::launch_pw_dw(a, st));
         sm.raw = a.Y; sm.act = a.Yact;
diff --git a/waveverify_amd/csrc/wv_ops.hip b/waveverify_amd/csrc/wv_ops.hip
--- a/waveverify_amd/csrc/wv_ops.hip
+++ b/waveverify_amd/csrc/wv_ops.hip
@@ -154,13 +154,11 @@
     if (mode == 2 && !l2norm && !accumulate) {
         if (!w_dw || ks_or_ratio < 1) return fail(WV_EINVAL, "mode 2 (upsample) needs w_dw and a ratio >= 1");
         Tmp t;
-        std::vector<float> taps((size_t)M * 5, 0.f);
-        for (int m = 0; m < M; ++m) taps[(size_t)m * 5 + 4] = 1.f;
         wv::PwDwArgs a{};
         a.X = X; a.pw = t.pw(w_pw, M, K); a.ct_w = t.up(w_dw, (size_t)K * 2 * ks_or_ratio); a.ratio = ks_or_ratio;
         a.ct_wt = t.upv(wv::pack_ct_wt(w_dw, K, a.pw.Kp, ks_or_ratio));
-        a.dw_w = t.upv(taps); a.dw_b = t.up(bias, M); a.Y = Y; a.Yact = Yact; a.act_scale = act_scale;
-        a.B = B; a.Tin = Tin; a.Tout = Tin * ks_or_ratio; a.ks = 5; a.stride = 1; a.dil = 1; a.pad = 4;
+        a.dw_w = nullptr; a.dw_b = t.up(bias, M); a.Y = Y; a.Yact = Yact; a.act_scale = act_scale;
+        a.B = B; a.Tin = Tin; a.Tout = Tin * ks_or_ratio; a.ks = 1; a.stride = 1; a.dil = 1; a.pad = 0;
         a.pre_scale = pre_scale; a.pre_elu = pre_elu; a.out_scale = 1.f; a.bands = 1;
         a.film_stride = 2;
         return done(t, wv::launch_pw_dw(a, (hipStream_t)stream), (hipStream_t)stream);
@@ -174,11 +172,9 @@
     if (Yact && !k1_form) return fail(WV_EINVAL, "Yact exists only in mode 2 and in the accumulate form with M >= 128");
     if (mode == 0 && accumulate && !l2norm && !bias && M >= 128) {
         Tmp t;
-        std::vector<float> taps((size_t)M * 5, 0.f);
-        for (int m = 0; m < M; ++m) taps[(size_t)m * 5 + 4] = 1.f;
         wv::PwDwArgs a{};
-        a.X = X; a.pw = t.pw(w_pw, M, K); a.dw_w = t.upv(taps); a.resid = Y; a.Y = Y; a.Yact = Yact; a.act_scale = act_scale;
-        a.B = B; a.Tin = Tin; a.Tout = Tin; a.ks = 5; a.stride = 1; a.dil = 1; a.pad = 4;
+        a.X = X; a.pw = t.pw(w_pw, M, K); a.dw_w = nullptr; a.resid = Y; a.Y = Y; a.Yact = Yact; a.act_scale = act_scale;
+        a.B = B; a.Tin = Tin; a.Tout = Tin; a.ks = 1; a.stride = 1; a.dil = 1; a.pad = 0;
         a.pre_scale = pre_scale; a.pre_elu = pre_elu; a.out_scale = out_scale; a.bands = 1; a.film_stride = 2;
         a.spec_add = 1;
         return done(t, wv::launch_pw_dw(a, (hipStream_t)stream), (hipStream_t)stream);
```

New measurement: 3483 clips/s, median of 6. 1.0% higher.
